# fgcallari/skeres

Hardware: AMD Instinct MI355X
Metric: LM iterations/sec (higher is better)
Workload: dtype f64

## Files before the change

skeres_amd/csrc/bal_kernels.hip:

```cpp
#include <hip/hip_runtime.h>

#include <algorithm>

#include "functors.hpp"
#include "bal_kernels.hpp"

namespace sk {

static constexpr int kBlock = 256;

__device__ __forceinline__ double wave_sum(double v) {
#pragma unroll
  for (int off = 32; off > 0; off >>= 1) v += __shfl_xor(v, off, 64);
  return v;
}

__device__ __forceinline__ int bal_part(const BalDev& d, int i) { return i >= d.cam_b ? 2 : ((i >= d.seg_lo && i < d.cam_a) ? 0 : 1); }
__device__ __forceinline__ int bal_pos(const BalDev& d, int i, int part) { return 9 * (i - (part == 0 ? d.seg_lo : (part == 1 ? d.cam_a : d.cam_b))); }
__device__ __forceinline__ double* bal_block(const BalDev& d, int i, int j, int* ld) {
  const int pj = bal_part(d, j), pi = bal_part(d, i);
  const BalDev::Front& f = d.front[pj];
  const int row = pi == pj ? bal_pos(d, i, pi) : f.border_row[i - d.cam_b];
  *ld = f.ld;
  return f.S + (size_t)row * f.ld + bal_pos(d, j, pj);
// ... 144 lines not shown
    double r0 = 0.0, r1 = 0.0, sqrt_rho1 = 1.0, alpha_sq_norm = 0.0;
    for (int first = 0; first < dim; first += W) {
      J out[2];
      out[1] = J(0.0);
      tape_run<J>(t, c, param, first, regs, out);
      if (first == 0) {
        r0 = out[0].a; r1 = out[1].a;
        if (kLoss) {
          const double sq = r0 * r0 + r1 * r1;
          double rho[3];
          bal_loss_eval(d, o, sq, rho);
          const LossCorrector lc(sq, rho);
          acc[0] += rho[0];
          sqrt_rho1 = lc.sqrt_rho1; alpha_sq_norm = lc.alpha_sq_norm;
          d.r[o] = r0 * lc.residual_scaling;
          d.r[(size_t)d.N + o] = r1 * lc.residual_scaling;
        } else {
          d.r[o] = r0;
          d.r[(size_t)d.N + o] = r1;
          acc[0] += r0 * r0 + r1 * r1;
        }
      }
#pragma unroll
      for (int w = 0; w < W; ++w) {
        const int k = first + w;
        if (k >= dim) continue;
        double j0 = out[0].v[w], j1 = out[1].v[w];
        if (kLoss) {
          const double rtj = alpha_sq_norm * (r0 * j0 + r1 * j1);
          const double a0 = sqrt_rho1 * (j0 - r0 * rtj), a1 = sqrt_rho1 * (j1 - r1 * rtj);
          j0 = a0; j1 = a1;
        }
        if (k < cs) {
          const double s = d.scale_c[9 * (size_t)ci + k];
          d.F[(size_t)k * d.N + o] = j0 * s;
          d.F[(size_t)(9 + k) * d.N + o] = j1 * s;
        } else {
          const double s = d.scale_p[3 * (size_t)pi + (k - cs)];
          d.E[(size_t)(k - cs) * d.N + o] = j0 * s;
          d.E[(size_t)(3 + k - cs) * d.N + o] = j1 * s;
        }
      }
    }
  }
  block_sum<1>(acc, d.partial, d.partial_stride);
}
template <bool kLoss>
__global__ __launch_bounds__(kBlock) void bal_eval_cost_tape_kernel(BalDev d, TapeDev t, int num_obs) {
  extern __shared__ __attribute__((aligned(16))) double tape_lds[];
  const TapeRegs<double> regs{tape_lds, kBlock, (int)threadIdx.x};
  double acc[2] = {0.0, 0.0};
  for (int o = blockIdx.x * kBlock + threadIdx.x; o < d.N; o += gridDim.x * kBlock) {
    if (d.is_host && d.is_host[o]) continue;
    const int ci = d.cam[o], pi = d.pt[o];
    double c[kTapeMaxObs], out[2];
    for (int k = 0; k < num_obs; ++k) c[k] = d.obs[(size_t)k * d.N + o];
    const int cs = d.cam_size;
    auto param = [&](int k) { return k < cs ? d.xc_new[9 * (size_t)ci + k] : d.xp_new[3 * (size_t)pi + (k - cs)]; };
    out[1] = 0.0;
    tape_run<double>(t, c, param, 0, regs, out);
    if (kLoss) {
      double rho[3];
      bal_loss_eval(d, o, out[0] * out[0] + out[1] * out[1], rho);
      acc[0] += rho[0];
    } else {
      acc[0] += out[0] * out[0] + out[1] * out[1];
    }
    double m0 = -d.u[3 * (size_t)d.N + o], m1 = -d.u[4 * (size_t)d.N + o];
#pragma unroll
    for (int k = 0; k < 3; ++k) {
      const double s = d.step_p[3 * (size_t)pi + k];
      m0 += d.E[(size_t)k * d.N + o] * s;
      m1 += d.E[(size_t)(3 + k) * d.N + o] * s;
    }
    acc[1] += m0 * (d.r[o] + m0 / 2.0) + m1 * (d.r[(size_t)d.N + o] + m1 / 2.0);
  }
  block_sum<2>(acc, d.partial, d.partial_stride);
}

template <bool kLoss>
__global__ __launch_bounds__(kBlock) void bal_host_jac_kernel(BalDev d, int partial_off) {
  double acc[1] = {0.0};
  for (int h = blockIdx.x * kBlock + threadIdx.x; h < d.num_host; h += gridDim.x * kBlock) {
    const int o = d.host_obs[h];
    const int ci = d.cam[o], pi = d.pt[o];
    const double* row = d.host_rows + (size_t)h * kHostRow;
    const double r0 = row[0], r1 = row[1];
    double j0[12], j1[12];
#pragma unroll
    for (int k = 0; k < 9; ++k) { j0[k] = row[2 + k]; j1[k] = row[11 + k]; }
#pragma unroll
    for (int k = 0; k < 3; ++k) { j0[9 + k] = row[20 + k]; j1[9 + k] = row[23 + k]; }
    if (kLoss) {
      const double sq = r0 * r0 + r1 * r1;
      double rho[3];
      bal_loss_eval(d, o, sq, rho);
      const LossCorrector lc(sq, rho);
      acc[0] += rho[0];
#pragma unroll
      for (int k = 0; k < 12; ++k) {
        const double a = j0[k], b = j1[k];
        const double rtj = lc.alpha_sq_norm * (r0 * a + r1 * b);
        j0[k] = lc.sqrt_rho1 * (a - r0 * rtj);
        j1[k] = lc.sqrt_rho1 * (b - r1 * rtj);
      }
      d.r[o] = r0 * lc.residual_scaling;
      d.r[(size_t)d.N + o] = r1 * lc.residual_scaling;
    } else {
      d.r[o] = r0;
      d.r[(size_t)d.N + o] = r1;
      acc[0] += r0 * r0 + r1 * r1;
    }
#pragma unroll
    for (int k = 0; k < 9; ++k) {
      const double s = d.scale_c[9 * (size_t)ci + k];
      d.F[(size_t)k * d.N + o] = j0[k] * s;
      d.F[(size_t)(9 + k) * d.N + o] = j1[k] * s;
    }
#pragma unroll
    for (int k = 0; k < 3; ++k) {
      const double s = d.scale_p[3 * (size_t)pi + k];
      d.E[(size_t)k * d.N + o] = j0[9 + k] * s;
      d.E[(size_t)(3 + k) * d.N + o] = j1[9 + k] * s;
    }
  }
  block_sum<1>(acc, d.partial + partial_off, d.partial_stride);
}

template <bool kLoss>
__global__ __launch_bounds__(kBlock) void bal_host_cost_kernel(BalDev d, int partial_off) {
  double acc[2] = {0.0, 0.0};
  for (int h = blockIdx.x * kBlock + threadIdx.x; h < d.num_host; h += gridDim.x * kBlock) {
    const int o = d.host_obs[h];
    const int ci = d.cam[o], pi = d.pt[o];
    const double n0 = d.host_rows[(size_t)h * kHostRow], n1 = d.host_rows[(size_t)h * kHostRow + 1];
    if (kLoss) {
      double rho[3];
      bal_loss_eval(d, o, n0 * n0 + n1 * n1, rho);
      acc[0] += rho[0];
    } else {
      acc[0] += n0 * n0 + n1 * n1;
    }
    double m0 = -d.u[3 * (size_t)d.N + o], m1 = -d.u[4 * (size_t)d.N + o];
#pragma unroll
    for (int k = 0; k < 3; ++k) {
      const double s = d.step_p[3 * (size_t)pi + k];
      m0 += d.E[(size_t)k * d.N + o] * s;
      m1 += d.E[(size_t)(3 + k) * d.N + o] * s;
    }
    acc[1] += m0 * (d.r[o] + m0 / 2.0) + m1 * (d.r[(size_t)d.N + o] + m1 / 2.0);
  }
  block_sum<2>(acc, d.partial + partial_off, d.partial_stride);
}

__global__ __launch_bounds__(kBlock) void bal_scale_jac_kernel(BalDev d) {
  for (int o = blockIdx.x * kBlock + threadIdx.x; o < d.N; o += gridDim.x * kBlock) {
    const int ci = d.cam[o], pi = d.pt[o];
#pragma unroll
    for (int k = 0; k < 9; ++k) {
      const double s = d.scale_c[9 * (size_t)ci + k];
      d.F[(size_t)k * d.N + o] *= s;
      d.F[(size_t)(9 + k) * d.N + o] *= s;
    }
#pragma unroll
    for (int k = 0; k < 3; ++k) {
      const double s = d.scale_p[3 * (size_t)pi + k];
      d.E[(size_t)k * d.N + o] *= s;
      d.E[(size_t)(3 + k) * d.N + o] *= s;
    }
  }
}

__global__ __launch_bounds__(kBlock) void bal_cam_records_kernel(BalDev d) {
  __shared__ __attribute__((aligned(16))) double stage[kBlock / 64][64 * kFcam];
  const int lane = threadIdx.x & 63, w = threadIdx.x >> 6;
  double* st = stage[w];
  const size_t N = d.N;
  for (long o0 = ((long)blockIdx.x * (kBlock / 64) + w) * 64; o0 < d.N; o0 += (long)gridDim.x * kBlock) {
    const long o = o0 + lane;
    const int my_slot = o < d.N ? d.obs_slot[o] : 0;
    if (o < d.N) {
#pragma unroll
      for (int k = 0; k < 18; ++k) st[lane * kFcam + k] = d.F[(size_t)k * N + o];
      st[lane * kFcam + 18] = d.r[o];
      st[lane * kFcam + 19] = d.r[N + o];
    }
    __builtin_amdgcn_wave_barrier();
    __builtin_amdgcn_s_waitcnt(0xC07F);
    __builtin_amdgcn_wave_barrier();
    const int nrec = (int)((d.N - o0) < 64 ? (d.N - o0) : 64);
#pragma unroll
    for (int i = 0; i < kFcam / 2; ++i) {
      const int e2 = i * 64 + lane, rr = e2 / (kFcam / 2), f2 = e2 - rr * (kFcam / 2);
      const int slot = __shfl(my_slot, rr, 64);
      if (rr < nrec) reinterpret_cast<double2*>(d.Fcam + (size_t)slot * kFcam)[f2] = reinterpret_cast<const double2*>(st)[e2];
    }
    __builtin_amdgcn_wave_barrier();
  }
}

__device__ __forceinline__ void bal_cam_reduce_body(const BalDev& d, int block) {
  const int wave = (block * kBlock + threadIdx.x) >> 6, lane = threadIdx.x & 63;
  if (wave >= d.C) return;
  double sq[9], g[9];
#pragma unroll
  for (int k = 0; k < 9; ++k) { sq[k] = 0.0; g[k] = 0.0; }
  for (int e = d.cam_start[wave] + lane; e < d.cam_start[wave + 1]; e += 64) {
    const double2* rec = reinterpret_cast<const double2*>(d.Fcam + (size_t)e * kFcam);
    double v[kFcam];
#pragma unroll
    for (int k = 0; k < kFcam / 2; ++k) { const double2 t = rec[k]; v[2 * k] = t.x; v[2 * k + 1] = t.y; }
    const double r0 = v[18], r1 = v[19];
#pragma unroll
    for (int k = 0; k < 9; ++k) {
      const double f0 = v[k], f1 = v[9 + k];
      sq[k] += f0 * f0 + f1 * f1;
      g[k] += f0 * r0 + f1 * r1;
    }
  }
#pragma unroll
  for (int k = 0; k < 9; ++k) { sq[k] = wave_sum(sq[k]); g[k] = wave_sum(g[k]); }
  if (lane == 0) {
#pragma unroll
    for (int k = 0; k < 9; ++k) { d.colsq_c[9 * (size_t)wave + k] = sq[k]; d.gs_c[9 * (size_t)wave + k] = g[k]; }
  }
}

__device__ __forceinline__ void bal_pt_reduce_body(const BalDev& d, int block) {
  const int gid = block * kBlock + threadIdx.x, sub = gid % kPointLanes;
  const int p = gid / kPointLanes;
  if (p >= d.P) return;
  double sq[3] = {0, 0, 0}, g[3] = {0, 0, 0};
  for (int o = d.pt_start[p] + sub; o < d.pt_start[p + 1]; o += kPointLanes) {
    const double r0 = d.r[o], r1 = d.r[(size_t)d.N + o];
#pragma unroll
    for (int k = 0; k < 3; ++k) {
      const double e0 = d.E[(size_t)k * d.N + o], e1 = d.E[(size_t)(3 + k) * d.N + o];
      sq[k] += e0 * e0 + e1 * e1;
      g[k] += e0 * r0 + e1 * r1;
    }
  }
#pragma unroll
  for (int k = 0; k < 3; ++k) { sq[k] = point_lanes_sum(sq[k]); g[k] = point_lanes_sum(g[k]); }
  if (sub == 0) {
#pragma unroll
    for (int k = 0; k < 3; ++k) { d.colsq_p[3 * (size_t)p + k] = sq[k]; d.gs_p[3 * (size_t)p + k] = g[k]; }
  }
}

__global__ __launch_bounds__(kBlock) void bal_reduce_kernel(BalDev d, int cam_blocks) {
  if ((int)blockIdx.x < cam_blocks) bal_cam_reduce_body(d, (int)blockIdx.x);
  else bal_pt_reduce_body(d, (int)blockIdx.x - cam_blocks);
}

__global__ void jacobi_scale_kernel(const double* colsq, double* scale, int n) {
  const int j = blockIdx.x * blockDim.x + threadIdx.x;
  if (j < n) scale[j] = scale[j] == 0.0 ? 0.0 : 1.0 / (1.0 + sqrt(colsq[j]));
}
__global__ void apply_scale_to_reductions_kernel(double* colsq, double* gs, const double* scale, int n) {
  const int j = blockIdx.x * blockDim.x + threadIdx.x;
  if (j < n) { const double s = scale[j]; colsq[j] = colsq[j] * s * s; gs[j] = gs[j] * s; }
}
__global__ void lm_diagonal_kernel(const double* colsq, double* D, int n, double lo, double hi, double radius) {
  const int j = blockIdx.x * blockDim.x + threadIdx.x;
  if (j < n) D[j] = sqrt(fmin(fmax(colsq[j], lo), hi) / radius);
}
__global__ __launch_bounds__(kBlock) void grad_max_xnorm_kernel(const double* gs, const double* scale, const double* x,
                                                                int n, double* partial, int stride) {
  double m = 0.0, s = 0.0;
  for (int j = blockIdx.x * kBlock + threadIdx.x; j < n; j += gridDim.x * kBlock) {
    if (scale[j] != 0.0 || gs[j] != 0.0) m = max_keep_nan(m, fabs(gs[j] / scale[j]));
    s += x[j] * x[j];
  }
  __shared__ double shm[kBlock / 64], shs[kBlock / 64];
#pragma unroll
  for (int off = 32; off > 0; off >>= 1) { m = max_keep_nan(m, __shfl_xor(m, off, 64)); s += __shfl_xor(s, off, 64); }
  if ((threadIdx.x & 63) == 0) { shm[threadIdx.x >> 6] = m; shs[threadIdx.x >> 6] = s; }
  __syncthreads();
  if (threadIdx.x == 0) {
    for (int i = 1; i < kBlock / 64; ++i) { m = max_keep_nan(m, shm[i]); s += shs[i]; }
    partial[blockIdx.x] = m;
    partial[stride + blockIdx.x] = s;
  }
}

__global__ __launch_bounds__(kBlock) void final_reduce_kernel(const double* partial, int stride, int count, int K, int maxmask, double* out) {
  __shared__ double sh[kBlock];
  const int k = blockIdx.x;
  const bool is_max = ((maxmask >> k) & 1) != 0;
  double a = 0.0;
  for (int i = threadIdx.x; i < count; i += kBlock) {
    const double v = partial[(size_t)k * stride + i];
    a = is_max ? max_keep_nan(a, v) : a + v;
  }
  sh[threadIdx.x] = a;
  __syncthreads();
  for (int w = kBlock / 2; w > 0; w >>= 1) {
    if ((int)threadIdx.x < w) sh[threadIdx.x] = is_max ? max_keep_nan(sh[threadIdx.x], sh[threadIdx.x + w]) : sh[threadIdx.x] + sh[threadIdx.x + w];
    __syncthreads();
  }
  if (threadIdx.x == 0) out[k] = sh[0];
}

__global__ __launch_bounds__(kBlock) void bal_point_block_kernel(BalDev d) {
  const int gid = blockIdx.x * kBlock + threadIdx.x, sub = gid % kPointLanes;
  const int p = gid / kPointLanes;
  if (p >= d.P) return;
  double t00 = 0, t10 = 0, t11 = 0, t20 = 0, t21 = 0, t22 = 0;
  for (int o = d.pt_start[p] + sub; o < d.pt_start[p + 1]; o += kPointLanes) {
    const double a0 = d.E[o], a1 = d.E[(size_t)d.N + o], a2 = d.E[2 * (size_t)d.N + o];
    const double b0 = d.E[3 * (size_t)d.N + o], b1 = d.E[4 * (size_t)d.N + o], b2 = d.E[5 * (size_t)d.N + o];
    t00 += a0 * a0 + b0 * b0; t10 += a1 * a0 + b1 * b0; t11 += a1 * a1 + b1 * b1;
    t20 += a2 * a0 + b2 * b0; t21 += a2 * a1 + b2 * b1; t22 += a2 * a2 + b2 * b2;
  }
  t00 = point_lanes_sum(t00); t10 = point_lanes_sum(t10); t11 = point_lanes_sum(t11);
  t20 = point_lanes_sum(t20); t21 = point_lanes_sum(t21); t22 = point_lanes_sum(t22);
  if (sub != 0) return;
  const double d0 = bal_lm_diag(d, d.colsq_p[3 * (size_t)p]), d1 = bal_lm_diag(d, d.colsq_p[3 * (size_t)p + 1]), d2 = bal_lm_diag(d, d.colsq_p[3 * (size_t)p + 2]);
  t00 += d0 * d0; t11 += d1 * d1; t22 += d2 * d2;
  const double l00 = sqrt(t00);
  const double l10 = t10 / l00, l20 = t20 / l00;
  const double l11 = sqrt(t11 - l10 * l10);
  const double l21 = (t21 - l20 * l10) / l11;
  const double l22 = sqrt(t22 - l20 * l20 - l21 * l21);
  const double m00 = 1.0 / l00, m11 = 1.0 / l11, m22 = 1.0 / l22;
  const double m10 = -(l10 * m00) / l11;
  const double m21 = -(l21 * m11) / l22;
  const double m20 = -(l20 * m00 + l21 * m10) / l22;
  const size_t P = d.P;
  d.M[p] = m00; d.M[P + p] = m10; d.M[2 * P + p] = m11; d.M[3 * P + p] = m20; d.M[4 * P + p] = m21; d.M[5 * P + p] = m22;
  const double g0 = d.gs_p[3 * (size_t)p], g1 = d.gs_p[3 * (size_t)p + 1], g2 = d.gs_p[3 * (size_t)p + 2];
  const double u0 = m00 * g0, u1 = m10 * g0 + m11 * g1, u2 = m20 * g0 + m21 * g1 + m22 * g2;
  d.q[p] = m00 * u0 + m10 * u1 + m20 * u2;
  d.q[P + p] = m11 * u1 + m21 * u2;
  d.q[2 * P + p] = m22 * u2;
  if (!(l00 > 0.0) || !(l11 > 0.0) || !(l22 > 0.0)) *d.fail_flag = 1;
}

__global__ __launch_bounds__(kBlock) void bal_kept_points_kernel(BalDev d, int obs_blocks) {
  const size_t N = d.N, P = d.P;
  if ((int)blockIdx.x < obs_blocks) {
    const int e = blockIdx.x * kBlock + threadIdx.x;
    if (e >= d.num_kept_obs) return;
    const int o = d.kept_obs[e], k = d.kept_obs_slot[e];
    const int ic = d.kept_cam[k] / 3, t3 = 3 * (d.kept_cam[k] % 3);
    const int c = d.cam[o];
    const bool below = ic > c;
    if (!d.front[bal_part(d, below ? c : ic)].S) return;
    double ea[3], eb[3];
#pragma unroll
    for (int a = 0; a < 3; ++a) { ea[a] = d.E[(size_t)a * N + o]; eb[a] = d.E[(size_t)(3 + a) * N + o]; }
    int ld;
    double* blk = below ? bal_block(d, ic, c, &ld) : bal_block(d, c, ic, &ld);
#pragma unroll
    for (int b = 0; b < 9; ++b) {
      const double f0 = d.F[(size_t)b * N + o], f1 = d.F[(size_t)(9 + b) * N + o];
#pragma unroll
      for (int a = 0; a < 3; ++a) {
        const double v = ea[a] * f0 + eb[a] * f1;
        if (below) blk[(size_t)(t3 + a) * ld + b] = v; else blk[(size_t)b * ld + t3 + a] = v;
      }
    }
    return;
  }
  const int k = (((int)blockIdx.x - obs_blocks) * kBlock + threadIdx.x) >> 6, lane = threadIdx.x & 63;
  if (k >= d.num_kept) return;
  const int p = d.kept_pt[k], ic = d.kept_cam[k] / 3, t3 = 3 * (d.kept_cam[k] % 3);
  double t00 = 0, t10 = 0, t11 = 0, t20 = 0, t21 = 0, t22 = 0;
  for (int o = d.pt_start[p] + lane; o < d.pt_start[p + 1]; o += 64) {
    const double a0 = d.E[o], a1 = d.E[N + o], a2 = d.E[2 * N + o];
    const double b0 = d.E[3 * N + o], b1 = d.E[4 * N + o], b2 = d.E[5 * N + o];
    t00 += a0 * a0 + b0 * b0; t10 += a1 * a0 + b1 * b0; t11 += a1 * a1 + b1 * b1;
    t20 += a2 * a0 + b2 * b0; t21 += a2 * a1 + b2 * b1; t22 += a2 * a2 + b2 * b2;
  }
  t00 = wave_sum(t00); t10 = wave_sum(t10); t11 = wave_sum(t11); t20 = wave_sum(t20); t21 = wave_sum(t21); t22 = wave_sum(t22);
  if (lane != 0) return;
  d.M[p] = 0.0; d.M[P + p] = 0.0; d.M[2 * P + p] = 0.0; d.M[3 * P + p] = 0.0; d.M[4 * P + p] = 0.0; d.M[5 * P + p] = 0.0;
  d.q[p] = 0.0; d.q[P + p] = 0.0; d.q[2 * P + p] = 0.0;
  if (!d.front[bal_part(d, ic)].S) return;
  const bool home = !d.kept_home || d.kept_home[k] != 0;
  const double d0 = home ? bal_lm_diag(d, d.colsq_p[3 * (size_t)p]) : 0.0, d1 = home ? bal_lm_diag(d, d.colsq_p[3 * (size_t)p + 1]) : 0.0,
               d2 = home ? bal_lm_diag(d, d.colsq_p[3 * (size_t)p + 2]) : 0.0;
  int ld;
  double* blk = bal_block(d, ic, ic, &ld) + (size_t)t3 * ld + t3;
  blk[0] = t00 + d0 * d0;
  blk[ld] = t10; blk[ld + 1] = t11 + d1 * d1;
  blk[2 * (size_t)ld] = t20; blk[2 * (size_t)ld + 1] = t21; blk[2 * (size_t)ld + 2] = t22 + d2 * d2;
  double* rhs = bal_rhs(d, ic) + t3;
  rhs[0] = home ? d.gs_p[3 * (size_t)p] : 0.0; rhs[1] = home ? d.gs_p[3 * (size_t)p + 1] : 0.0; rhs[2] = home ? d.gs_p[3 * (size_t)p + 2] : 0.0;
}

__global__ __launch_bounds__(kBlock) void bal_kept_sums_kernel(BalDev d, double* buf, int K, int gather) {
  const int t = blockIdx.x * kBlock + threadIdx.x;
  if (t >= 3 * d.num_kept) return;
  const int k = t / 3, a = t - 3 * k;
  const size_t p = (size_t)d.kept_pt[k], g = (size_t)(d.kept_global ? d.kept_global[k] : k);
  if (gather) { buf[3 * g + a] = d.colsq_p[3 * p + a]; buf[3 * (size_t)K + 3 * g + a] = d.gs_p[3 * p + a]; }
  else { d.colsq_p[3 * p + a] = buf[3 * g + a]; d.gs_p[3 * p + a] = buf[3 * (size_t)K + 3 * g + a]; }
}

__global__ __launch_bounds__(kBlock, 4) void bal_obs_precompute_kernel(BalDev d) {
  constexpr int kLs = kWs + 2;
  __shared__ __attribute__((aligned(16))) double stage[kBlock / 64][32 * kLs];
  const size_t N = d.N, P = d.P;
  const int lane = threadIdx.x & 63, wave = threadIdx.x >> 6;
  double* mine = &stage[wave][0];
  for (long base = (long)(blockIdx.x * kBlock + wave * 64); base < (long)d.N; base += (long)gridDim.x * kBlock) {
    const long o = base + lane;
    const int my_slot = o < (long)d.N ? d.obs_slot[o] : 0;
    double w[27], rt[2];
    if (o < (long)d.N) {
      const int p = d.pt[o];
      const double m00 = d.M[p], m10 = d.M[P + p], m11 = d.M[2 * P + p], m20 = d.M[3 * P + p], m21 = d.M[4 * P + p], m22 = d.M[5 * P + p];
      const double q0 = d.q[p], q1 = d.q[P + p], q2 = d.q[2 * P + p];
      double eh[2][3];
#pragma unroll
      for (int r = 0; r < 2; ++r) {
        const double e0 = d.E[(3 * r) * N + o], e1 = d.E[(3 * r + 1) * N + o], e2 = d.E[(3 * r + 2) * N + o];
        eh[r][0] = e0 * m00;
        eh[r][1] = e0 * m10 + e1 * m11;
        eh[r][2] = e0 * m20 + e1 * m21 + e2 * m22;
        rt[r] = d.r[r * N + o] - (e0 * q0 + e1 * q1 + e2 * q2);
      }
#pragma unroll
      for (int c = 0; c < 9; ++c) {
        const double f0 = d.F[c * N + o], f1 = d.F[(9 + c) * N + o];
#pragma unroll
        for (int a = 0; a < 3; ++a) w[3 * c + a] = f0 * eh[0][a] + f1 * eh[1][a];
      }
    }
    const int nrec = (int)(((long)d.N - base) < 64 ? ((long)d.N - base) : 64);
    const int sub = lane >> 4, chunk = lane & 15;
#pragma unroll
    for (int half = 0; half < 2; ++half) {
      if ((lane >> 5) == half && o < (long)d.N) {
        double* rec = mine + (lane & 31) * kLs;
#pragma unroll
        for (int k = 0; k < 27; ++k) rec[k] = w[k];
        rec[27] = rt[0]; rec[28] = rt[1];
        rec[29] = 0.0; rec[30] = 0.0; rec[31] = 0.0;
      }
      __builtin_amdgcn_wave_barrier();
#pragma unroll 4
      for (int it = 0; it < 8; ++it) {
        const int rl = 4 * it + sub, rec = 32 * half + rl;
        const int slot = __shfl(my_slot, rec, 64);
        if (rec < nrec) {
          const double2 v = *reinterpret_cast<const double2*>(&mine[rl * kLs + 2 * chunk]);
          *reinterpret_cast<double2*>(d.What + (size_t)slot * kWs + 2 * chunk) = v;
        }
      }
      __builtin_amdgcn_wave_barrier();
    }
  }
}

__global__ __launch_bounds__(kBlock) void bal_cam_diag_kernel(BalDev d) {
  const int i = (blockIdx.x * kBlock + threadIdx.x) >> 6, lane = threadIdx.x & 63;
  if (i >= d.C) return;
  if (d.pseudo && d.pseudo[i]) return;
  double acc[45], rh[9];
#pragma unroll
  for (int k = 0; k < 45; ++k) acc[k] = 0.0;
#pragma unroll
  for (int k = 0; k < 9; ++k) rh[k] = 0.0;
  for (int e = d.cam_start[i] + lane; e < d.cam_start[i + 1]; e += 64) {
    double f0[9], f1[9], w[28];
    {
      const double2* rec = reinterpret_cast<const double2*>(d.Fcam + (size_t)e * kFcam);
#pragma unroll
      for (int k = 0; k < 9; ++k) {
        const double2 t = rec[k];
        if (2 * k < 9) f0[2 * k] = t.x; else f1[2 * k - 9] = t.x;
        if (2 * k + 1 < 9) f0[2 * k + 1] = t.y; else f1[2 * k + 1 - 9] = t.y;
      }
    }
    const double2* wrec = reinterpret_cast<const double2*>(d.What + (size_t)e * kWs);
#pragma unroll
    for (int k = 0; k < 14; ++k) { const double2 t = wrec[k]; w[2 * k] = t.x; w[2 * k + 1] = t.y; }
    const double r0 = w[27], r1 = wrec[14].x;
    int k = 0;
#pragma unroll
    for (int c = 0; c < 9; ++c) {
      rh[c] += f0[c] * r0 + f1[c] * r1;
#pragma unroll
      for (int e2 = 0; e2 <= c; ++e2, ++k)
        acc[k] += (f0[c] * f0[e2] + f1[c] * f1[e2]) - (w[3 * c] * w[3 * e2] + w[3 * c + 1] * w[3 * e2 + 1] + w[3 * c + 2] * w[3 * e2 + 2]);
    }
  }
#pragma unroll
  for (int k = 0; k < 45; ++k) acc[k] = wave_sum(acc[k]);
#pragma unroll
  for (int k = 0; k < 9; ++k) rh[k] = wave_sum(rh[k]);
  if (lane == 0 && d.front[bal_part(d, i)].S) {
    int k = 0, ld;
    double* blk = bal_block(d, i, i, &ld);
    double* rhs = bal_rhs(d, i);
#pragma unroll
    for (int c = 0; c < 9; ++c) {
      rhs[c] = rh[c];
#pragma unroll
      for (int e2 = 0; e2 <= c; ++e2, ++k) blk[(size_t)c * ld + e2] = acc[k];
    }
  }
}

__global__ __launch_bounds__(64) void bal_dup_diag_kernel(BalDev d) {
  const int first = blockIdx.x;
  const int i = d.dup_cam[first];
  if (first > 0 && d.dup_cam[first - 1] == i) return;
  if (!d.front[bal_part(d, i)].S) return;
  const int t = threadIdx.x;
  if (t >= 45) return;
  int c = 0, rem = t;
  while (rem > c) { rem -= c + 1; ++c; }
  const int e2 = rem;
  double acc = 0.0;
  for (int k = first; k < d.num_dup && d.dup_cam[k] == i; ++k) {
    const double* wa = d.What + (size_t)d.dup_a[k] * kWs;
    const double* wb = d.What + (size_t)d.dup_b[k] * kWs;
    acc += (wa[3 * c] * wb[3 * e2] + wa[3 * c + 1] * wb[3 * e2 + 1] + wa[3 * c + 2] * wb[3 * e2 + 2]) +
           (wb[3 * c] * wa[3 * e2] + wb[3 * c + 1] * wa[3 * e2 + 1] + wb[3 * c + 2] * wa[3 * e2 + 2]);
  }
  int ld;
  double* blk = bal_block(d, i, i, &ld);
  blk[(size_t)c * ld + e2] -= acc;
}

constexpr int kPairSlot = 34;
__device__ __forceinline__ void pair_accumulate(const BalDev& d, int e_begin, int e_end, int stride, int c, double* slot, double (&acc)[9]) {
  if (e_begin >= e_end) return;
  const int last = e_begin + (e_end - 1 - e_begin) / stride * stride;
  const double* wr = d.What + (size_t)d.pair_row_obs[e_begin] * kWs + 3 * c;
  const double* wc = d.What + (size_t)d.pair_col_obs[e_begin] * kWs + 3 * c;
  double y0 = wr[0], y1 = wr[1], y2 = wr[2], v0 = wc[0], v1 = wc[1], v2 = wc[2];
  int e1 = e_begin + stride <= last ? e_begin + stride : last;
  int ob1 = d.pair_row_obs[e1], oa1 = d.pair_col_obs[e1];
  for (int e = e_begin; e < e_end; e += stride) {
    slot[3 * c] = v0; slot[3 * c + 1] = v1; slot[3 * c + 2] = v2;
    __builtin_amdgcn_wave_barrier();
    double w[kWu];
#pragma unroll
    for (int k = 0; k < kWu / 2; ++k) { const double2 t = reinterpret_cast<const double2*>(slot)[k]; w[2 * k] = t.x; w[2 * k + 1] = t.y; }
    __builtin_amdgcn_wave_barrier();
    const double* wrn = d.What + (size_t)ob1 * kWs + 3 * c;
    const double* wcn = d.What + (size_t)oa1 * kWs + 3 * c;
    const double yn0 = wrn[0], yn1 = wrn[1], yn2 = wrn[2], vn0 = wcn[0], vn1 = wcn[1], vn2 = wcn[2];
    const int e2 = e + 2 * stride <= last ? e + 2 * stride : last;
    const int ob2 = d.pair_row_obs[e2], oa2 = d.pair_col_obs[e2];
#pragma unroll
    for (int k = 0; k < 9; ++k) acc[k] += y0 * w[3 * k] + y1 * w[3 * k + 1] + y2 * w[3 * k + 2];
    y0 = yn0; y1 = yn1; y2 = yn2; v0 = vn0; v1 = vn1; v2 = vn2;
    ob1 = ob2; oa1 = oa2;
  }
}

__device__ __forceinline__ int xcd_grouped_block(int w, int group) {
  if (group <= 0) return w;
  const int x = w & 7, q = w >> 3;
  return ((q / group) * 8 + x) * group + q % group;
}

__global__ __launch_bounds__(kBlock) void bal_pair_kernel(BalDev d, int xcd_group) {
  const int lane = threadIdx.x & 63;
  const int wave = (xcd_grouped_block((int)blockIdx.x, xcd_group) * kBlock + threadIdx.x) >> 6;
  __shared__ __attribute__((aligned(16))) double share[kBlock / 64][7][kPairSlot];
  const int sub = lane / 9, c = lane - 9 * sub;
  const int slot = wave * 7 + sub;
  if (sub >= 7 || slot >= d.num_short_segments) return;
  const int seg = d.short_segments[slot];
  double acc[9];
#pragma unroll
  for (int k = 0; k < 9; ++k) acc[k] = 0.0;
  pair_accumulate(d, d.seg_start[seg], d.seg_start[seg + 1], 1, c, share[threadIdx.x >> 6][sub], acc);
  const int i = d.seg_row[seg], j = d.seg_col[seg];
  int ld;
  double* out = bal_block(d, i, j, &ld) + (size_t)c * ld;
#pragma unroll
  for (int k = 0; k < 9; ++k) out[k] = -acc[k];
}

__global__ __launch_bounds__(kBlock) void bal_pair_long_kernel(BalDev d, int xcd_group) {
  __shared__ double red[kBlock / 64][7][81];
  __shared__ __attribute__((aligned(16))) double share[kBlock / 64][7][kPairSlot];
  const int lane = threadIdx.x & 63, w = threadIdx.x >> 6;
  const int slot = (xcd_grouped_block((int)blockIdx.x, xcd_group) * kBlock + threadIdx.x) >> 6;
  if (slot >= d.num_long_segments) return;
  const int seg = d.long_segments[slot];
  const int sub = lane / 9, c = lane - 9 * sub;
  double acc[9];
#pragma unroll
  for (int k = 0; k < 9; ++k) acc[k] = 0.0;
  if (sub < 7) {
    pair_accumulate(d, d.seg_start[seg] + sub, d.seg_start[seg + 1], 7, c, share[w][sub], acc);
#pragma unroll
    for (int k = 0; k < 9; ++k) red[w][sub][9 * c + k] = acc[k];
  }
  __builtin_amdgcn_wave_barrier();
  __builtin_amdgcn_s_waitcnt(0xC07F);
  __builtin_amdgcn_wave_barrier();
  const int i = d.seg_row[seg], j = d.seg_col[seg];
  int ld;
  double* blk = bal_block(d, i, j, &ld);
  for (int e = lane; e < 81; e += 64) {
    double s = 0.0;
#pragma unroll
    for (int g = 0; g < 7; ++g) s += red[w][g][e];
    blk[(size_t)(e / 9) * ld + e % 9] = -s;
  }
}

__global__ void finish_normal_matrix_kernel(double* S, int ld, int n, int npad, int rhs_row, const double* D) {
  const int j = blockIdx.x * blockDim.x + threadIdx.x;
  if (j >= npad) return;
  if (j < n) S[(size_t)j * ld + j] += D[j] * D[j];
  else if (j == rhs_row) S[(size_t)j * ld + j] = 1e300;
  else S[(size_t)j * ld + j] = 1.0;
}
__global__ void bal_finish_S_kernel(BalDev d, int parts) {
  const int j = blockIdx.x * blockDim.x + threadIdx.x;
  if (j >= 9 * d.C) return;
  const int i = j / 9, c = j - 9 * i, part = bal_part(d, i);
  if (!((parts >> part) & 1) || !d.front[part].S) return;
  if (d.pseudo && d.pseudo[i]) return;
  int ld;
  double* blk = bal_block(d, i, i, &ld);
  const double D = bal_lm_diag(d, d.colsq_c[j]);
  blk[(size_t)c * ld + c] += D * D;
}
__global__ void set_diagonal_kernel(double* S, int ld, int from, int to, double value) {
  const int j = from + blockIdx.x * blockDim.x + threadIdx.x;
  if (j < to) S[(size_t)j * ld + j] = value;
}

__global__ __launch_bounds__(kBlock) void bal_obs_backsub_kernel(BalDev d) {
  const size_t N = d.N;
  for (int o = blockIdx.x * kBlock + threadIdx.x; o < d.N; o += gridDim.x * kBlock) {
    const double* yc = d.y_c + 9 * (size_t)d.cam[o];
    double f0 = 0.0, f1 = 0.0;
#pragma unroll
    for (int c = 0; c < 9; ++c) { f0 += d.F[c * N + o] * yc[c]; f1 += d.F[(9 + c) * N + o] * yc[c]; }
    d.u[o] = d.E[o] * f0 + d.E[3 * N + o] * f1;
    d.u[N + o] = d.E[N + o] * f0 + d.E[4 * N + o] * f1;
    d.u[2 * N + o] = d.E[2 * N + o] * f0 + d.E[5 * N + o] * f1;
    d.u[3 * N + o] = f0;
    d.u[4 * N + o] = f1;
  }
}

__global__ __launch_bounds__(kBlock) void bal_point_backsub_kernel(BalDev d) {
  const int gid = blockIdx.x * kBlock + threadIdx.x, sub = gid % kPointLanes;
  const int p = gid / kPointLanes;
  double acc[1] = {0.0};
  double w0 = 0.0, w1 = 0.0, w2 = 0.0;
  if (p < d.P) {
    for (int o = d.pt_start[p] + sub; o < d.pt_start[p + 1]; o += kPointLanes) {
      w0 += d.u[o];
      w1 += d.u[(size_t)d.N + o];
      w2 += d.u[2 * (size_t)d.N + o];
    }
  }
  w0 = point_lanes_sum(w0); w1 = point_lanes_sum(w1); w2 = point_lanes_sum(w2);
  if (p < d.P && sub == 0) {
    const size_t P = d.P;
    const double t0 = d.gs_p[3 * (size_t)p] - w0, t1 = d.gs_p[3 * (size_t)p + 1] - w1, t2 = d.gs_p[3 * (size_t)p + 2] - w2;
    const double m00 = d.M[p], m10 = d.M[P + p], m11 = d.M[2 * P + p], m20 = d.M[3 * P + p], m21 = d.M[4 * P + p], m22 = d.M[5 * P + p];
    const double u0 = m00 * t0, u1 = m10 * t0 + m11 * t1, u2 = m20 * t0 + m21 * t1 + m22 * t2;
    const double y[3] = {m00 * u0 + m10 * u1 + m20 * u2, m11 * u1 + m21 * u2, m22 * u2};
#pragma unroll
    for (int k = 0; k < 3; ++k) {
      const double st = -y[k];
      const double dl = st * d.scale_p[3 * (size_t)p + k];
      d.step_p[3 * (size_t)p + k] = st;
      const double xo = d.xp[3 * (size_t)p + k];
      const double xn = xo + dl;
      d.xp_new[3 * (size_t)p + k] = xn;
      const double df = xo - xn;
      acc[0] += df * df;
    }
  }
  block_sum<1>(acc, d.partial + d.partial_stride, d.partial_stride);
}

__global__ __launch_bounds__(kBlock) void bal_kept_step_kernel(BalDev d, int slot) {
  double acc[1] = {0.0};
  for (int k = threadIdx.x; k < d.num_kept; k += kBlock) {
    const int p = d.kept_pt[k], ic = d.kept_cam[k] / 3, t3 = 3 * (d.kept_cam[k] % 3);
    const bool home = !d.kept_home || d.kept_home[k] != 0;
#pragma unroll
    for (int a = 0; a < 3; ++a) {
      const double st = -d.y_c[9 * (size_t)ic + t3 + a];
      d.step_p[3 * (size_t)p + a] = st;
      const double xo = d.xp[3 * (size_t)p + a];
      const double xn = xo + st * d.scale_p[3 * (size_t)p + a];
      d.xp_new[3 * (size_t)p + a] = xn;
      const double df = xo - xn;
      if (home) acc[0] += df * df;
    }
  }
  block_sum<1>(acc, d.partial + d.partial_stride + slot, d.partial_stride);
}

__global__ __launch_bounds__(kBlock) void bal_cam_step_kernel(BalDev d, int norm_lo, int norm_hi, int norm_lo2, int norm_hi2) {
  double acc[1] = {0.0};
  const int n = 9 * d.C;
  const int j = blockIdx.x * kBlock + threadIdx.x;
  if (j < n) {
    const int i = j / 9, c = j - 9 * i, part = bal_part(d, i);
    const double y = d.front[part].S ? d.y_front[part][bal_pos(d, i, part) + c] : 0.0;
    d.y_c[j] = y;
    const double st = -y;
    d.step_c[j] = st;
    const double xo = d.xc[j];
    const double xn = xo + st * d.scale_c[j];
    d.xc_new[j] = xn;
    const double df = xo - xn;
    if ((j >= norm_lo && j < norm_hi) || (j >= norm_lo2 && j < norm_hi2)) acc[0] += df * df;
  }
  block_sum<1>(acc, d.partial, d.partial_stride);
}
__global__ __launch_bounds__(1024) void final_reduce_rows_kernel(const double* partial, int stride, ReduceRows rows) {
  __shared__ double sh[1024];
  const int k = blockIdx.x, count = rows.count[k];
  const bool is_max = rows.is_max[k] != 0;
  const double* src = partial + (size_t)rows.row[k] * stride;
  double a = 0.0;
  for (int i = threadIdx.x; i < count; i += 1024) a = is_max ? max_keep_nan(a, src[i]) : a + src[i];
  sh[threadIdx.x] = a;
  __syncthreads();
  for (int w = 512; w > 0; w >>= 1) {
    if ((int)threadIdx.x < w) sh[threadIdx.x] = is_max ? max_keep_nan(sh[threadIdx.x], sh[threadIdx.x + w]) : sh[threadIdx.x] + sh[threadIdx.x + w];
    __syncthreads();
  }
  if (threadIdx.x == 0) *rows.out[k] = sh[0];
}
void launch_final_reduce_rows(const double* partial, int stride, const ReduceRows& rows, hipStream_t s) {
  if (rows.n > 0) hipLaunchKernelGGL(final_reduce_rows_kernel, dim3(rows.n), dim3(1024), 0, s, partial, stride, rows);
}

__global__ __launch_bounds__(256) void tri_pack_kernel(double* S, int ld, double* packed, const int* __restrict__ col0, const long long* __restrict__ off,
                                                       int to_packed) {
  const int kb = blockIdx.y;
  const size_t c0 = (size_t)col0[kb] * 128, width = (size_t)(kb + 1) * 128 - c0;
  double* pk = packed + off[kb];
  const size_t n2 = 128 * width / 2;
  for (size_t i = (size_t)blockIdx.x * 256 + threadIdx.x; i < n2; i += (size_t)gridDim.x * 256) {
    const size_t e = 2 * i, r = e / width, c = e % width;
    double2* a = reinterpret_cast<double2*>(S + ((size_t)kb * 128 + r) * ld + c0 + c);
    double2* b = reinterpret_cast<double2*>(pk + e);
    if (to_packed) *b = *a; else *a = *b;
  }
}

static inline int grid_for(int n, int cap = 2048) {
  int g = (n + kBlock - 1) / kBlock;
  return g < 1 ? 1 : (g > cap ? cap : g);
}

__global__ __launch_bounds__(256) void zero_envelope_kernel(double* S, int ld, const int* col0) {
  const int kb = blockIdx.y;
  const size_t c0 = (size_t)col0[kb] * 128, width = (size_t)(kb + 1) * 128 - c0;
  const size_t n2 = 128 * width / 2;
  for (size_t i = (size_t)blockIdx.x * 256 + threadIdx.x; i < n2; i += (size_t)gridDim.x * 256) {
    const size_t e = 2 * i, r = e / width, c = e % width;
    *reinterpret_cast<double2*>(S + ((size_t)kb * 128 + r) * ld + c0 + c) = make_double2(0.0, 0.0);
  }
}
void launch_zero_envelope(double* S, int ld, const int* col0, int nblk, hipStream_t s) {
  if (nblk > 0) hipLaunchKernelGGL(zero_envelope_kernel, dim3(32, nblk), dim3(256), 0, s, S, ld, col0);
}

int bal_partial_blocks(int N) { return grid_for(N); }
size_t tri_packed_elems(int nblk) { return (size_t)128 * 128 * ((size_t)nblk * (nblk + 1) / 2); }
void launch_tri_pack(double* S, int ld, double* packed, int nblk, const int* col0, const long long* off, bool to_packed, hipStream_t s) {
  if (nblk > 0) hipLaunchKernelGGL(tri_pack_kernel, dim3(64, nblk), dim3(256), 0, s, S, ld, packed, col0, off, to_packed ? 1 : 0);
}

void launch_bal_eval_jac(const BalDev& d, hipStream_t s) {
  if (d.loss_root >= 0) hipLaunchKernelGGL(bal_eval_jac_kernel<true>, dim3(grid_for(d.N)), dim3(kBlock), 0, s, d);
  else hipLaunchKernelGGL(bal_eval_jac_kernel<false>, dim3(grid_for(d.N)), dim3(kBlock), 0, s, d);
}
void launch_bal_eval_cost(const BalDev& d, hipStream_t s) {
  if (d.loss_root >= 0) hipLaunchKernelGGL(bal_eval_cost_kernel<true>, dim3(grid_for(d.N)), dim3(kBlock), 0, s, d);
  else hipLaunchKernelGGL(bal_eval_cost_kernel<false>, dim3(grid_for(d.N)), dim3(kBlock), 0, s, d);
}
int bal_tape_width(const Tape& t) { return t.num_obs_consts > kTapeMaxObs ? 0 : tape_pick_width(t, kBlock); }
template <class K> static void bal_tape_allow_lds(K kernel, size_t bytes) {
  if (bytes > 48 * 1024) (void)hipFuncSetAttribute(reinterpret_cast<const void*>(kernel), hipFuncAttributeMaxDynamicSharedMemorySize, (int)bytes);
}
void launch_bal_eval_jac_tape(const BalDev& d, const TapeDevBuffers& tb, hipStream_t s) {
  const int W = bal_tape_width(tb.host), nobs = tb.host.num_obs_consts;
  const size_t lds = tape_lds_bytes(tb.host, W, kBlock);
  const dim3 g(grid_for(d.N)), b(kBlock);
#define SK_TAPE_JAC(LOSS, WW) { bal_tape_allow_lds(bal_eval_jac_tape_kernel<LOSS, WW>, lds); hipLaunchKernelGGL((bal_eval_jac_tape_kernel<LOSS, WW>), g, b, lds, s, d, tb.view, nobs); }
  if (d.loss_root >= 0) { if (W == 3) SK_TAPE_JAC(true, 3) else if (W == 2) SK_TAPE_JAC(true, 2) else SK_TAPE_JAC(true, 1) }
  else { if (W == 3) SK_TAPE_JAC(false, 3) else if (W == 2) SK_TAPE_JAC(false, 2) else SK_TAPE_JAC(false, 1) }
#undef SK_TAPE_JAC
}
void launch_bal_eval_cost_tape(const BalDev& d, const TapeDevBuffers& tb, hipStream_t s) {
  const size_t lds = tape_lds_bytes(tb.host, 0, kBlock);
  const int nobs = tb.host.num_obs_consts;
  if (d.loss_root >= 0) { bal_tape_allow_lds(bal_eval_cost_tape_kernel<true>, lds); hipLaunchKernelGGL(bal_eval_cost_tape_kernel<true>, dim3(grid_for(d.N)), dim3(kBlock), lds, s, d, tb.view, nobs); }
  else { bal_tape_allow_lds(bal_eval_cost_tape_kernel<false>, lds); hipLaunchKernelGGL(bal_eval_cost_tape_kernel<false>, dim3(grid_for(d.N)), dim3(kBlock), lds, s, d, tb.view, nobs); }
}
int launch_bal_host_jac(const BalDev& d, int partial_off, hipStream_t s) {
  if (d.num_host <= 0) return 0;
  const int g = grid_for(d.num_host);
  if (d.loss_root >= 0) hipLaunchKernelGGL(bal_host_jac_kernel<true>, dim3(g), dim3(kBlock), 0, s, d, partial_off);
  else hipLaunchKernelGGL(bal_host_jac_kernel<false>, dim3(g), dim3(kBlock), 0, s, d, partial_off);
  return g;
}
int launch_bal_host_cost(const BalDev& d, int partial_off, hipStream_t s) {
  if (d.num_host <= 0) return 0;
  const int g = grid_for(d.num_host);
  if (d.loss_root >= 0) hipLaunchKernelGGL(bal_host_cost_kernel<true>, dim3(g), dim3(kBlock), 0, s, d, partial_off);
  else hipLaunchKernelGGL(bal_host_cost_kernel<false>, dim3(g), dim3(kBlock), 0, s, d, partial_off);
  return g;
}
void launch_bal_scale_jac(const BalDev& d, hipStream_t s) { hipLaunchKernelGGL(bal_scale_jac_kernel, dim3(grid_for(d.N)), dim3(kBlock), 0, s, d); }
void launch_bal_cam_records(const BalDev& d, hipStream_t s) { hipLaunchKernelGGL(bal_cam_records_kernel, dim3(grid_for((d.N + 63) / 64 * 64)), dim3(kBlock), 0, s, d); }
void launch_bal_reduce(const BalDev& d, hipStream_t s) {
  const int cam_blocks = (d.C * 64 + kBlock - 1) / kBlock, pt_blocks = d.P > 0 ? (int)(((long)d.P * kPointLanes + kBlock - 1) / kBlock) : 0;
  hipLaunchKernelGGL(bal_reduce_kernel, dim3(cam_blocks + pt_blocks), dim3(kBlock), 0, s, d, cam_blocks);
}
static int point_grid(int P) { return (int)(((long)P * kPointLanes + kBlock - 1) / kBlock); }
int bal_point_blocks(int P) { return P > 0 ? point_grid(P) : 1; }
void launch_jacobi_scale(const double* colsq, double* scale, int n, hipStream_t s) { if (n > 0) hipLaunchKernelGGL(jacobi_scale_kernel, dim3((n + 255) / 256), dim3(256), 0, s, colsq, scale, n); }
void launch_apply_scale_to_reductions(double* colsq, double* gs, const double* scale, int n, hipStream_t s) { if (n > 0) hipLaunchKernelGGL(apply_scale_to_reductions_kernel, dim3((n + 255) / 256), dim3(256), 0, s, colsq, gs, scale, n); }
void launch_lm_diagonal(const double* colsq, double* D, int n, double lo, double hi, double radius, hipStream_t s) { if (n > 0) hipLaunchKernelGGL(lm_diagonal_kernel, dim3((n + 255) / 256), dim3(256), 0, s, colsq, D, n, lo, hi, radius); }
int launch_grad_max_xnorm(const double* gs, const double* scale, const double* x, int n, double* partial, int stride, hipStream_t s) {
  const int g = grid_for(n, 256);
  hipLaunchKernelGGL(grad_max_xnorm_kernel, dim3(g), dim3(kBlock), 0, s, gs, scale, x, n, partial, stride);
  return g;
}
__global__ void bal_pack_rank_scalars_kernel(const double* __restrict__ scal, double* __restrict__ table, int rank, int world, int mode, int segmented) {
  const int K = mode == 0 ? 3 : 4;
  for (int i = threadIdx.x; i < world * K; i += blockDim.x) table[i] = 0.0;
  __syncthreads();
  if (threadIdx.x != 0) return;
  double* t = table + (size_t)rank * K;
  if (mode == 0) {
    t[0] = scal[4];
    t[1] = segmented ? fmax(scal[2], scal[0]) : scal[2];
    t[2] = scal[3] + (segmented ? scal[1] : 0.0);
  } else {
    const int fail = *reinterpret_cast<const int*>(scal + 14), info = *reinterpret_cast<const int*>(scal + 15);
    t[0] = scal[0]; t[1] = scal[1];
    t[2] = scal[9] + (segmented ? scal[8] : 0.0);
    t[3] = (double)(fail | info);
  }
}
void launch_bal_pack_rank_scalars(const double* scal, double* table, int rank, int world, int mode, bool segmented, hipStream_t s) {
  hipLaunchKernelGGL(bal_pack_rank_scalars_kernel, dim3(1), dim3(64), 0, s, scal, table, rank, world, mode, segmented ? 1 : 0);
}
void launch_final_reduce(const double* partial, int stride, int count, int K, int maxmask, double* out, hipStream_t s) { hipLaunchKernelGGL(final_reduce_kernel, dim3(K), dim3(kBlock), 0, s, partial, stride, count, K, maxmask, out); }
void launch_bal_point_block(const BalDev& d, hipStream_t s) { if (d.P > 0) hipLaunchKernelGGL(bal_point_block_kernel, dim3(point_grid(d.P)), dim3(kBlock), 0, s, d); }
void launch_bal_kept_points(const BalDev& d, hipStream_t s) {
  if (d.num_kept <= 0) return;
  const int obs_blocks = (d.num_kept_obs + kBlock - 1) / kBlock;
  hipLaunchKernelGGL(bal_kept_points_kernel, dim3(obs_blocks + (d.num_kept * 64 + kBlock - 1) / kBlock), dim3(kBlock), 0, s, d, obs_blocks);
}
void launch_bal_obs_precompute(const BalDev& d, hipStream_t s) { hipLaunchKernelGGL(bal_obs_precompute_kernel, dim3(grid_for(d.N)), dim3(kBlock), 0, s, d); }
void launch_bal_kept_sums(const BalDev& d, double* buf, int K, bool gather, hipStream_t s) {
  if (d.num_kept > 0) hipLaunchKernelGGL(bal_kept_sums_kernel, dim3((3 * d.num_kept + kBlock - 1) / kBlock), dim3(kBlock), 0, s, d, buf, K, gather ? 1 : 0);
}
void launch_bal_cam_diag(const BalDev& d, hipStream_t s) {
  hipLaunchKernelGGL(bal_cam_diag_kernel, dim3((d.C * 64 + kBlock - 1) / kBlock), dim3(kBlock), 0, s, d);
  if (d.num_dup > 0) hipLaunchKernelGGL(bal_dup_diag_kernel, dim3(d.num_dup), dim3(64), 0, s, d);
}
void launch_bal_pair(const BalDev& d, hipStream_t s) {
  const int group_long = dev_knobs().schedule_plain ? 0 : 8, group_short = group_long;
  auto grid = [](int blocks, int group) { return group > 0 ? (blocks + 8 * group - 1) / (8 * group) * (8 * group) : blocks; };
  if (d.num_long_segments > 0)
    hipLaunchKernelGGL(bal_pair_long_kernel, dim3(grid((d.num_long_segments * 64 + kBlock - 1) / kBlock, group_long)), dim3(kBlock), 0, s, d, group_long);
  if (d.num_short_segments > 0) {
    const int waves = (d.num_short_segments + 6) / 7;
    hipLaunchKernelGGL(bal_pair_kernel, dim3(grid((waves * 64 + kBlock - 1) / kBlock, group_short)), dim3(kBlock), 0, s, d, group_short);
  }
}
void launch_finish_normal_matrix(double* S, int ld, int n, int npad, int rhs_row, const double* D, hipStream_t s) { hipLaunchKernelGGL(finish_normal_matrix_kernel, dim3((npad + 255) / 256), dim3(256), 0, s, S, ld, n, npad, rhs_row, D); }
__global__ void bal_finish_all_kernel(BalDev d, BalFinishRanges r, int jmax) {
  const int j = blockIdx.x * blockDim.x + threadIdx.x;
  if (j >= jmax) return;
  if (j < 9 * d.C) {
    const int i = j / 9, c = j - 9 * i, part = bal_part(d, i);
    if (d.front[part].S && !(d.pseudo && d.pseudo[i])) {
      int ld;
      double* blk = bal_block(d, i, i, &ld);
      const double D = bal_lm_diag(d, d.colsq_c[j]);
      blk[(size_t)c * ld + c] += D * D;
    }
  }
#pragma unroll
  for (int k = 0; k < 4; ++k)
    if (r.S[k] && j >= r.from[k] && j < r.to[k]) r.S[k][(size_t)j * r.ld[k] + j] = r.value[k];
}
void launch_bal_finish_all(const BalDev& d, const BalFinishRanges& r, hipStream_t s) {
  int jmax = 9 * d.C;
  for (int k = 0; k < 4; ++k) if (r.S[k] && r.to[k] > jmax) jmax = r.to[k];
  hipLaunchKernelGGL(bal_finish_all_kernel, dim3((jmax + 255) / 256), dim3(256), 0, s, d, r, jmax);
}
void launch_bal_finish_S(const BalDev& d, int parts, hipStream_t s) { hipLaunchKernelGGL(bal_finish_S_kernel, dim3((9 * d.C + 255) / 256), dim3(256), 0, s, d, parts); }
void launch_set_diagonal(double* S, int ld, int from, int to, double value, hipStream_t s) {
  if (to > from) hipLaunchKernelGGL(set_diagonal_kernel, dim3((to - from + 255) / 256), dim3(256), 0, s, S, ld, from, to, value);
}
void launch_bal_backsub(const BalDev& d, double* out, int norm_lo, int norm_hi, int norm_lo2, int norm_hi2, hipStream_t s) {
  const int gc = (9 * d.C + kBlock - 1) / kBlock, gp = bal_point_blocks(d.P);
  hipLaunchKernelGGL(bal_cam_step_kernel, dim3(gc), dim3(kBlock), 0, s, d, norm_lo, norm_hi, norm_lo2, norm_hi2);
  hipLaunchKernelGGL(bal_obs_backsub_kernel, dim3(grid_for(d.N)), dim3(kBlock), 0, s, d);
  hipLaunchKernelGGL(bal_point_backsub_kernel, dim3(gp), dim3(kBlock), 0, s, d);
  if (d.num_kept > 0) hipLaunchKernelGGL(bal_kept_step_kernel, dim3(1), dim3(kBlock), 0, s, d, gp);
  ReduceRows rows;
  rows.n = 2;
  rows.row[0] = 0; rows.count[0] = gc; rows.out[0] = out;
  rows.row[1] = 1; rows.count[1] = d.P > 0 ? gp + (d.num_kept > 0 ? 1 : 0) : 0; rows.out[1] = out + 1;
  launch_final_reduce_rows(d.partial, d.partial_stride, rows, s);
}

__global__ __launch_bounds__(kBlock) void dogleg_vector_norms_kernel(BalDev d, DoglegDev q) {
  double acc[3] = {0.0, 0.0, 0.0};
  const int nc = 9 * d.C, n = nc + 3 * d.P;
  for (int j = blockIdx.x * kBlock + threadIdx.x; j < n; j += gridDim.x * kBlock) {
    double sj = 0.0, gj = 0.0;
    if (!(j < nc && d.pseudo && d.pseudo[j / 9])) {
      const double diag = sqrt(fmin(fmax(d.colsq_c[j], d.lm_lo), d.lm_hi));
      const double gh = d.gs_c[j] / diag;
      gj = d.step_c[j];
      const double p = diag * gj;
      sj = -gh / diag;
      acc[0] += gh * gh; acc[1] += gh * p; acc[2] += p * p;
    }
    q.s[j] = sj; q.g[j] = gj;
  }
  block_sum<3>(acc, q.partial + 5 * (size_t)q.stride, q.stride);
}

__global__ __launch_bounds__(kBlock) void bal_dogleg_products_kernel(BalDev d, DoglegDev q) {
  double acc[5] = {0.0, 0.0, 0.0, 0.0, 0.0};
  const size_t N = d.N;
  const double* sp = q.s + 9 * (size_t)d.C;
  const double* gp = q.g + 9 * (size_t)d.C;
  for (int o = blockIdx.x * kBlock + threadIdx.x; o < d.N; o += gridDim.x * kBlock) {
    const size_t ci = 9 * (size_t)d.cam[o], pi = 3 * (size_t)d.pt[o];
    double w0 = 0.0, w1 = 0.0, m0 = 0.0, m1 = 0.0;
#pragma unroll
    for (int k = 0; k < 9; ++k) {
      const double f0 = d.F[k * N + o], f1 = d.F[(9 + k) * N + o], sk_ = q.s[ci + k], gk = q.g[ci + k];
      w0 += f0 * sk_; w1 += f1 * sk_; m0 += f0 * gk; m1 += f1 * gk;
    }
#pragma unroll
    for (int k = 0; k < 3; ++k) {
      const double e0 = d.E[k * N + o], e1 = d.E[(3 + k) * N + o], sk_ = sp[pi + k], gk = gp[pi + k];
      w0 += e0 * sk_; w1 += e1 * sk_; m0 += e0 * gk; m1 += e1 * gk;
    }
    const double r0 = d.r[o], r1 = d.r[N + o];
    acc[0] += w0 * r0 + w1 * r1; acc[1] += m0 * r0 + m1 * r1;
    acc[2] += w0 * w0 + w1 * w1; acc[3] += w0 * m0 + w1 * m1; acc[4] += m0 * m0 + m1 * m1;
  }
  block_sum<5>(acc, q.partial, q.stride);
}

__global__ __launch_bounds__(kBlock) void bal_dogleg_combine_kernel(BalDev d, DoglegDev q, double a, double b) {
  double acc[1] = {0.0};
  const int n = 9 * d.C + 3 * d.P;
  for (int j = blockIdx.x * kBlock + threadIdx.x; j < n; j += gridDim.x * kBlock) {
    const double st = a * q.s[j] + b * q.g[j];
    d.step_c[j] = st;
    const double xo = d.xc[j];
    const double xn = xo + st * d.scale_c[j];
    d.xc_new[j] = xn;
    const double df = xo - xn;
    acc[0] += df * df;
  }
  block_sum<1>(acc, q.partial + 8 * (size_t)q.stride, q.stride);
}

int dogleg_partial_stride(const BalDev& d) { return std::max(grid_for(d.N), grid_for(9 * d.C + 3 * d.P)); }
void launch_dogleg_vector_norms(const BalDev& d, const DoglegDev& q, hipStream_t s) {
  hipLaunchKernelGGL(dogleg_vector_norms_kernel, dim3(grid_for(9 * d.C + 3 * d.P)), dim3(kBlock), 0, s, d, q);
}
void launch_bal_dogleg_products(const BalDev& d, const DoglegDev& q, hipStream_t s) {
  hipLaunchKernelGGL(bal_dogleg_products_kernel, dim3(grid_for(d.N)), dim3(kBlock), 0, s, d, q);
}
void launch_dogleg_reduce_scalars(const DoglegDev& q, hipStream_t s) { launch_final_reduce(q.partial, q.stride, q.stride, 8, 0, q.scal, s); }
void launch_bal_dogleg_combine(const BalDev& d, const DoglegDev& q, double a, double b, hipStream_t s) {
  const int g = grid_for(9 * d.C + 3 * d.P);
  hipLaunchKernelGGL(bal_dogleg_combine_kernel, dim3(g), dim3(kBlock), 0, s, d, q, a, b);
  launch_final_reduce(q.partial + 8 * (size_t)q.stride, q.stride, g, 1, 0, q.scal + 8, s);
}

__global__ void box_project_kernel(double* x, const double* __restrict__ lo, const double* __restrict__ hi, int n) {
  const int j = blockIdx.x * blockDim.x + threadIdx.x;
  if (j < n) x[j] = fmin(fmax(x[j], lo[j]), hi[j]);
}

__global__ __launch_bounds__(kBlock) void bounded_grad_max_xnorm_kernel(const double* __restrict__ gs, const double* __restrict__ scale, const double* __restrict__ x,
                                                                        int n, BoundsDev q) {
  double m = 0.0;
  double acc[2] = {0.0, 0.0};
  for (int j = blockIdx.x * kBlock + threadIdx.x; j < n; j += gridDim.x * kBlock) {
    const double xj = x[j], lo = q.lo[j], hi = q.hi[j];
    if (scale[j] != 0.0) m = fmax(m, fabs(xj - fmin(fmax(xj - gs[j] / scale[j], lo), hi)));
    acc[0] += xj * xj;
    acc[1] += (xj == lo || xj == hi) ? 1.0 : 0.0;
  }
  __shared__ double shm[kBlock / 64];
#pragma unroll
  for (int off = 32; off > 0; off >>= 1) m = fmax(m, __shfl_xor(m, off, 64));
  if ((threadIdx.x & 63) == 0) shm[threadIdx.x >> 6] = m;
  __syncthreads();
  if (threadIdx.x == 0) {
    for (int i = 1; i < kBlock / 64; ++i) m = fmax(m, shm[i]);
    q.partial[3 * (size_t)q.stride + blockIdx.x] = m;
  }
  block_sum<2>(acc, q.partial + 4 * (size_t)q.stride, q.stride);
}

__global__ __launch_bounds__(kBlock) void bal_directional_derivative_kernel(BalDev d, BoundsDev q) {
  double m = 0.0;
  double acc[1] = {0.0};
  const int nc = 9 * d.C, n = nc + 3 * d.P;
  for (int j = blockIdx.x * kBlock + threadIdx.x; j < n; j += gridDim.x * kBlock) {
    if (j < nc && d.pseudo && d.pseudo[j / 9]) continue;
    const double st = d.step_c[j];
    acc[0] += d.gs_c[j] * st;
    m = fmax(m, fabs(st * d.scale_c[j]));
  }
  __shared__ double shm[kBlock / 64];
#pragma unroll
  for (int off = 32; off > 0; off >>= 1) m = fmax(m, __shfl_xor(m, off, 64));
  if ((threadIdx.x & 63) == 0) shm[threadIdx.x >> 6] = m;
  __syncthreads();
  if (threadIdx.x == 0) {
    for (int i = 1; i < kBlock / 64; ++i) m = fmax(m, shm[i]);
    q.partial[2 * (size_t)q.stride + blockIdx.x] = m;
  }
  block_sum<1>(acc, q.partial + q.stride, q.stride);
}

__global__ __launch_bounds__(kBlock) void bal_bounded_candidate_kernel(BalDev d, BoundsDev q, double alpha) {
  double acc[1] = {0.0};
  const int nc = 9 * d.C, n = nc + 3 * d.P;
  for (int j = blockIdx.x * kBlock + threadIdx.x; j < n; j += gridDim.x * kBlock) {
    const double xo = d.xc[j];
    double xn = xo;
    if (!(j < nc && d.pseudo && d.pseudo[j / 9])) xn = fmin(fmax(xo + (alpha * d.step_c[j]) * d.scale_c[j], q.lo[j]), q.hi[j]);
    d.xc_new[j] = xn;
    const double df = xo - xn;
    acc[0] += df * df;
  }
  block_sum<1>(acc, q.partial, q.stride);
}

int bounds_partial_stride(int n) { return grid_for(n); }
void launch_box_project(double* x, const double* lo, const double* hi, int n, hipStream_t s) {
  if (n > 0) hipLaunchKernelGGL(box_project_kernel, dim3((n + 255) / 256), dim3(256), 0, s, x, lo, hi, n);
}
void launch_bounded_grad_max_xnorm(const double* gs, const double* scale, const double* x, int n, const BoundsDev& q, hipStream_t s) {
  const int g = grid_for(n);
  hipLaunchKernelGGL(bounded_grad_max_xnorm_kernel, dim3(g), dim3(kBlock), 0, s, gs, scale, x, n, q);
  launch_final_reduce(q.partial + 3 * (size_t)q.stride, q.stride, g, 3, 1, q.scal + 3, s);
}
void launch_bal_directional_derivative(const BalDev& d, const BoundsDev& q, hipStream_t s) {
  const int g = grid_for(9 * d.C + 3 * d.P);
  hipLaunchKernelGGL(bal_directional_derivative_kernel, dim3(g), dim3(kBlock), 0, s, d, q);
  launch_final_reduce(q.partial + q.stride, q.stride, g, 2, 2, q.scal + 1, s);
}
void launch_bal_bounded_candidate(const BalDev& d, const BoundsDev& q, double alpha, hipStream_t s) {
  const int g = grid_for(9 * d.C + 3 * d.P);
  hipLaunchKernelGGL(bal_bounded_candidate_kernel, dim3(g), dim3(kBlock), 0, s, d, q, alpha);
  launch_final_reduce(q.partial, q.stride, g, 1, 0, q.scal, s);
}

}
```

skeres_amd/csrc/bal_kernels.hpp:

```cpp
#pragma once
#include <hip/hip_runtime.h>

#include "common.hpp"
#include "loss.hpp"

namespace sk {

constexpr int kLongSegment = 32;
constexpr int kWs = 32;
constexpr int kWu = 28;
struct BalDev {
  int C, P, N;
  int res_size, cam_size, pt_size;
  const int* cam;
  const int* pt;
  const double* obs;
  const int* pt_start;
  const int* cam_start;
  const int* cam_obs;
  int num_segments;
  const int* seg_start;
  const int* seg_row;
  const int* seg_col;
  int num_short_segments, num_long_segments;
  const int* short_segments;
  const int* long_segments;
  const int* pair_row_obs;
  const int* pair_col_obs;
  int num_kept;
  const int* kept_pt;  const int* kept_cam;
  int num_kept_obs;  const int* kept_obs;  const int* kept_obs_slot;
  const unsigned char* pseudo;
  const int* kept_home;  const int* kept_global;
  int num_dup;  const int* dup_a;  const int* dup_b;  const int* dup_cam;
  double* xc;  double* xp;
  double* xc_new;  double* xp_new;
  double* scale_c;  double* scale_p;
  double* colsq_c;  double* colsq_p;
  double* gs_c;  double* gs_p;
  double lm_lo, lm_hi, lm_radius;  const double* lm_radius_dev;
  double* step_c;  double* step_p;
  double* y_c;
  double* r;  double* F;  double* E;  double* What;  double* u;
  double* Fcam;  const int* obs_slot;
  double* M;  double* q;
  struct Front { double* S; int ld; int interior; int rhs_row; const int* border_row; };
  Front front[3];
  int seg_lo, cam_a, cam_b;
  const double* y_front[3];
  double* S;  int ld;  int rhs_row;
  double* partial;  int partial_stride;
  int* fail_flag;
  const LossNode* loss_nodes;  int loss_root;  const int* loss_of_obs;
  const unsigned char* is_host;
  int num_host;
  const int* host_obs;
  const double* host_rows;
};
constexpr int kHostRow = 26;
constexpr int kFcam = 20;

int bal_partial_blocks(int N);
int bal_point_blocks(int P);
void launch_zero_envelope(double* S, int ld, const int* col0, int nblk, hipStream_t s);
size_t tri_packed_elems(int nblk);
void launch_tri_pack(double* S, int ld, double* packed, int nblk, const int* col0, const long long* off, bool to_packed, hipStream_t s);
void launch_bal_eval_jac(const BalDev& d, hipStream_t s);
void launch_bal_eval_cost(const BalDev& d, hipStream_t s);
void launch_bal_eval_jac_tape(const BalDev& d, const TapeDevBuffers& tb, hipStream_t s);
void launch_bal_eval_cost_tape(const BalDev& d, const TapeDevBuffers& tb, hipStream_t s);
int launch_bal_host_jac(const BalDev& d, int partial_off, hipStream_t s);
int launch_bal_host_cost(const BalDev& d, int partial_off, hipStream_t s);
void launch_bal_scale_jac(const BalDev& d, hipStream_t s);
void launch_bal_cam_records(const BalDev& d, hipStream_t s);
void launch_bal_reduce(const BalDev& d, hipStream_t s);
void launch_jacobi_scale(const double* colsq, double* scale, int n, hipStream_t s);
void launch_apply_scale_to_reductions(double* colsq, double* gs, const double* scale, int n, hipStream_t s);
void launch_lm_diagonal(const double* colsq, double* D, int n, double lo, double hi, double radius, hipStream_t s);
int launch_grad_max_xnorm(const double* gs, const double* scale, const double* x, int n, double* partial, int stride, hipStream_t s);
void launch_final_reduce(const double* partial, int stride, int count, int K, int maxmask, double* out, hipStream_t s);
void launch_bal_pack_rank_scalars(const double* scal, double* table, int rank, int world, int mode, bool segmented, hipStream_t s);
struct ReduceRows { int n = 0; int row[4] = {0, 0, 0, 0}, count[4] = {0, 0, 0, 0}, is_max[4] = {0, 0, 0, 0}; double* out[4] = {nullptr, nullptr, nullptr, nullptr}; };
void launch_final_reduce_rows(const double* partial, int stride, const ReduceRows& rows, hipStream_t s);
void launch_bal_point_block(const BalDev& d, hipStream_t s);
void launch_bal_kept_points(const BalDev& d, hipStream_t s);
void launch_bal_kept_sums(const BalDev& d, double* buf, int K, bool gather, hipStream_t s);
void launch_bal_obs_precompute(const BalDev& d, hipStream_t s);
void launch_bal_cam_diag(const BalDev& d, hipStream_t s);
void launch_bal_pair(const BalDev& d, hipStream_t s);
void launch_finish_normal_matrix(double* S, int ld, int n, int npad, int rhs_row, const double* D, hipStream_t s);
void launch_bal_finish_S(const BalDev& d, int parts, hipStream_t s);
struct BalFinishRanges { double* S[4] = {nullptr, nullptr, nullptr, nullptr}; int ld[4] = {0, 0, 0, 0}, from[4] = {0, 0, 0, 0}, to[4] = {0, 0, 0, 0}; double value[4] = {0, 0, 0, 0}; };
void launch_bal_finish_all(const BalDev& d, const BalFinishRanges& r, hipStream_t s);
void launch_set_diagonal(double* S, int ld, int from, int to, double value, hipStream_t s);
void launch_bal_backsub(const BalDev& d, double* out, int norm_lo, int norm_hi, int norm_lo2, int norm_hi2, hipStream_t s);

struct DoglegDev { double* s; double* g; double* partial; int stride; double* scal; };
int dogleg_partial_stride(const BalDev& d);
void launch_dogleg_vector_norms(const BalDev& d, const DoglegDev& q, hipStream_t s);
void launch_bal_dogleg_products(const BalDev& d, const DoglegDev& q, hipStream_t s);
void launch_dogleg_reduce_scalars(const DoglegDev& q, hipStream_t s);
void launch_bal_dogleg_combine(const BalDev& d, const DoglegDev& q, double a, double b, hipStream_t s);

struct BoundsDev { const double* lo; const double* hi; double* partial; int stride; double* scal; };
int bounds_partial_stride(int n);
void launch_box_project(double* x, const double* lo, const double* hi, int n, hipStream_t s);
void launch_bounded_grad_max_xnorm(const double* gs, const double* scale, const double* x, int n, const BoundsDev& q, hipStream_t s);
void launch_bal_directional_derivative(const BalDev& d, const BoundsDev& q, hipStream_t s);
void launch_bal_bounded_candidate(const BalDev& d, const BoundsDev& q, double alpha, hipStream_t s);

}
```

skeres_amd/csrc/bal_solver.hip:

```cpp
#include <algorithm>
#include <cmath>
#include <limits>

#include "bal_kernels.hpp"
#include "bal_plan.hpp"
#include "solver.hpp"

namespace sk {

namespace {

struct CaptureGuard {
  hipStream_t s; bool active; bool* graph_mode;
  CaptureGuard(hipStream_t st, bool on, bool* gm) : s(st), active(on), graph_mode(gm) {}
  void release() { active = false; }
  ~CaptureGuard() {
    if (!active) return;
    hipGraph_t g = nullptr;
    (void)hipStreamEndCapture(s, &g);
    if (g) (void)hipGraphDestroy(g);
    (void)hipGetLastError();
    *graph_mode = false;
  }
};

class BalSolver : public SolverBase {
 public:
  BalSolver(const Options& o, Problem* p) : SolverBase(o, p) {}
  double syrk_flops_per_solve() const override {
    double f = 0.0;
    for (int k = 0; k < 3; ++k) if (fr_[k].nblk > 0) f += cholesky_syrk_flops((int)fr_[k].dim, group_, fr_[k].env(), chain_ok() && (k != 1 || tail_chain()), nullptr, fr_[k].ncols, fr_[k].tail_rows, fr_[k].tl());
    return f;
  }
  double syrk_c_bytes_per_solve() const override {
    double tiles = 0.0;
    for (int k = 0; k < 3; ++k) {
      double t = 0.0;
      if (fr_[k].nblk > 0) (void)cholesky_syrk_flops((int)fr_[k].dim, group_, fr_[k].env(), chain_ok() && (k != 1 || tail_chain()), &t, fr_[k].ncols, fr_[k].tail_rows, fr_[k].tl());
      tiles += t;
    }
    return tiles * 2.0 * 128.0 * 128.0 * sizeof(double);
  }
  void set_kernel_timing(int on) override {
    SolverBase::set_kernel_timing(on);
    kt_b_.only(on == 2 ? "gemm_syrk" : ""); kt_b_.enable(on != 0);
  }
  KernelTimer::Stat kernel_stat(const std::string& name) override {
    KernelTimer::Stat a = kt_.get_stat(name), b = kt_b_.get_stat(name);
    a.seconds += b.seconds; a.launches += b.launches;
    return a;
  }
  bool stat(const std::string& name, double* value) const override {
    const int nblk = npad_ / 128;
    if (name == "envelope_fill") {
      double in = 0.0;
      for (int k = 0; k < 3; ++k) in += fr_[k].envelope().blocks();
      *value = in / (0.5 * nblk * (nblk + 1.0));
      return true;
    }
    if (name == "reduced_system_blocks") { *value = nblk; return true; }
    if (name == "camera_order") { *value = camera_order_; return true; }
    if (name == "cholesky_flops_full") { const double n = 9.0 * C_; *value = n * n * n / 3.0; return true; }
    if (name == "cholesky_flops_plan") {
      double f = 0.0;
      for (int k = 0; k < 3; ++k) if (fr_[k].nblk > 0) f += cholesky_plan_flops(fr_[k].nblk, fr_[k].env(), fr_[k].ncols, fr_[k].tail_rows, fr_[k].tl());
      *value = f;
      return true;
    }
    if (name == "cholesky_columns_resident") {
      int r = 0;
      for (int k = 0; k < 3; ++k) {
        if (fr_[k].nblk == 0) continue;
        const CholeskyPlan plan = cholesky_plan(fr_[k].nblk, group_, fr_[k].env(), chain_live() && (k != 1 || tail_chain()), fr_[k].ncols, fr_[k].tail_rows, fr_[k].tl());
        for (char c : plan.resident) r += c ? 1 : 0;
      }
      *value = r;
      return true;
    }
    if (name == "chain_steps") {
      *value = (dissected_ ? std::max(fr_[0].ncols, fr_[1].ncols) : 0) + fr_[2].ncols;
      return true;
    }
    if (name == "allreduce_bytes") { *value = (double)packed_elems_ * sizeof(double); return true; }
    if (name == "allreduce_bytes_full_triangle") { *value = (double)tri_packed_elems(nblk) * sizeof(double); return true; }
    if (name == "dissected") { *value = dissected_ ? 1.0 : 0.0; return true; }
    if (name == "pair_segments_short") { *value = d_.num_short_segments; return true; }
    if (name == "pair_segments_long") { *value = d_.num_long_segments; return true; }
    if (name == "graph_replay") { *value = graph_mode_ ? 1.0 : 0.0; return true; }
    if (name == "host_callback_blocks" || name == "tape_blocks") {
      const bool host = name == "host_callback_blocks";
      size_t c = 0;
      for (size_t b = 0; b < problem_->rb_functor.size(); ++b)
        c += host ? problem_->rb_functor[b] == SK_FUNCTOR_HOST_CALLBACK : problem_->tape_of_block(b) != nullptr;
      *value = (double)c;
      return true;
    }
    if (name == "tape_width") { *value = tape_mode_ ? bal_tape_width(tape_dev_.host) : 0; return true; }
    if (name == "tape_lds_bytes") { *value = tape_mode_ ? (double)tape_lds_bytes(tape_dev_.host, bal_tape_width(tape_dev_.host), 256) : 0.0; return true; }
    if (name == "retained_points") { *value = (double)retained_pts_.size(); return true; }
    if (name == "retained_model_us") { *value = retained_model_us_; return true; }
    if (name == "retained_model_us_without") { *value = retained_without_us_; return true; }
    if (name == "border_cameras") { *value = border_cams_; return true; }
    if (name == "border_gap") { *value = border_gap_; return true; }
    if (name == "border_model_us") { *value = border_model_us_; return true; }
    if (name == "border_model_us_plain") { *value = border_plain_us_; return true; }
    if (name == "segments") { *value = segmented_ ? segments_ : (dissected_ ? 2 : 1); return true; }
    if (name == "segment_cameras") { *value = segmented_ ? my_hi_ - my_lo_ : C_; return true; }
    if (name.rfind("model_us_segments_", 0) == 0) { const int k = atoi(name.c_str() + 18); if (k < 1 || k > 8) return false; *value = cut_model_.model_us[k]; return true; }
    if (name == "dissection_head_cameras") { *value = cam_a_; return true; }
    if (name == "dissection_tail_cameras") { *value = cam_b_ - cam_a_; return true; }
    if (name == "dissection_separator_cameras") { *value = dissected_ ? C_ - cam_b_ : 0; return true; }
    if (name == "dissection_model_us_plain") { *value = cut_model_.t_plain; return true; }
    if (name == "dissection_model_us") { *value = cut_model_.t_model; return true; }
    if (name == "model_us_two_segments_with_members") { *value = cut_model_.two_segments_members_us; return true; }
    return strategy_stat(name, value);
  }
  bool chain_ok() const { return opt_.cholesky_group == 0 && opt_.lookahead && chol_ctx_.server != nullptr; }
  bool chain_live() const { return chain_ok() && cholesky_chain_enabled(&chol_ctx_); }
  bool tail_chain() const { return chol_ctx_b_.server != nullptr; }
  int distribution(double* allreduce_s, double* saved_s) const override {
    if (allreduce_s) *allreduce_s = est_allreduce_s_;
    if (saved_s) *saved_s = est_saved_s_;
    return distribution_;
  }

 protected:
  int setup() override;
  int evaluate_with_jacobian(bool first) override;
  int linear_solve(double radius, LinearSolve* out) override;
  int dogleg_trial(double a, double b, double* cost, double* step_norm) override;
  int bounded_trial(double alpha, double* cost, double* step_norm) override;
  bool supports_dogleg() const override { return true; }
  int solve_once(double radius, LinearSolve* out, bool* chain_lost);
  struct Backsolve { int resident; bool zero_after; };
  int enqueue_schur_assembly(const Backsolve& bs, bool graph);
  int enqueue_factor_backsolve(const Backsolve& bs, bool graph);
  int enqueue_point_backsub(bool graph);
  int enqueue_candidate_cost(int rows, bool* failed);
  int trial_cost(const double* step_sq_dev, int step_sq_slot, double* cost, double* step_norm);
  const char* refuses_bounds() const override {
    for (int f : problem_->rb_functor)
      if (f == SK_FUNCTOR_HOST_CALLBACK) return "parameter bounds with host-evaluated (director) residual blocks under DENSE_SCHUR are not supported";
    return nullptr;
  }
  int upload_bounds();
  BoundsDev bd_{};
  DevBuf<double> b_bd_box_, b_bd_partial_, b_bd_scal_;
  DoglegDev dl_{};
  DevBuf<double> b_dl_vec_, b_dl_partial_, b_dl_scal_;
  void accept_candidate() override { std::swap(d_.xc, d_.xc_new); std::swap(d_.xp, d_.xp_new); parity_ ^= 1; }
  int write_back() override;
  void describe(Summary* s) override {
    s->num_parameter_blocks = (int)problem_->block_size.size();
    s->num_parameters = problem_->num_parameters();
    s->num_residual_blocks = (int)problem_->rb_functor.size();
    s->num_residuals = problem_->num_residuals;
    s->num_e_blocks = P_total_; s->num_f_blocks = C_ - pseudo_cams_;
  }

 private:
  int gather_rank_scalars(double* vals, int K, const int* ops);
  int host_callbacks(const double* x_dev, bool jac, bool* failed);
  std::vector<int> host_obs_;
  std::vector<const CostFunction*> host_cf_;
  std::vector<double> host_x_, host_rows_h_;
  DevBuf<unsigned char> b_is_host_;
  DevBuf<int> b_host_obs_;
  DevBuf<double> b_host_rows_;
  std::vector<int> h_cam_, h_pt_;
  int gather_rank_scalars_signed(double* vals, int K);
  bool rank_table_on_device(int K) const;
  int enqueue_rank_table(int mode, int K);
  int fold_rank_table(const double* table, double* vals, int K, const int* ops);
  int exchange_rank_table(const double* vals, int K, std::vector<double>* table);

  int C_ = 0, P_total_ = 0, P_ = 0, N_ = 0;
  int res_size_ = 2, cam_size_ = 9, pt_size_ = 3;
  int n_ = 0, npad_ = 0, rhs_row_ = 0;
  std::vector<int> cam_block_, pt_block_;
  std::vector<int> local_pt_;
  BalDev d_{};
  DevBuf<LossNode> b_loss_nodes_;
  DevBuf<int> b_loss_of_obs_;
  DevBuf<int> b_cam_, b_pt_, b_pt_start_, b_cam_start_, b_cam_obs_, b_obs_slot_, b_seg_start_, b_seg_row_, b_seg_col_, b_pair_row_, b_pair_col_, b_short_segs_, b_long_segs_;
  int *fail_p_ = nullptr, *info_p_ = nullptr;
  DevBuf<double> b_obs_, b_xc_, b_xp_, b_xc_new_, b_xp_new_, b_scale_, b_colsq_, b_gs_, b_step_, b_y_,
      b_r_, b_F_, b_Fcam_, b_E_, b_W_, b_rt_, b_M_, b_q_, b_S_, b_Linv_, b_partial_, b_scal_, b_small_;
  std::vector<int> env_last_;
  std::vector<int> env_tail_;
  std::vector<int> retained_pts_, retained_cam_;
  int pseudo_cams_ = 0;
  int border_members_ = 0;
  double retained_model_us_ = 0.0, retained_without_us_ = 0.0;
  std::vector<int> struct_ocam_, struct_opt_;
  int struct_P_ = 0;
  DevBuf<int> b_kept_pt_, b_kept_cam_, b_kept_obs_, b_kept_obs_slot_;
  int P_own_ = 0;
  DevBuf<int> b_kept_home_, b_kept_global_;
  DevBuf<int> b_dup_a_, b_dup_b_, b_dup_cam_;
  int num_dup_ = 0;
  int num_kept_obs_ = 0;
  DevBuf<unsigned char> b_pseudo_;
  int border_cams_ = 0, border_gap_ = 0;
  double border_model_us_ = 0.0, border_plain_us_ = 0.0;
  FrontHost fr_[3];
  bool dissected_ = false;
  bool segmented_ = false;
  int segments_ = 0, role_ = 0, my_lo_ = 0, my_hi_ = 0;
  bool replica_ = false;
  int fold_world_ = 0;
  int cam_a_ = 0, cam_b_ = 0, border_blocks_ = 0;
  std::vector<int> seg_off_;
  std::vector<int> sep_first_;
  std::vector<int> root_last_, root_tail_;
  FrontView leaf_;
  DevBuf<int> b_border_row_[2], b_leaf_map_, b_leaf_gmap_;
  CutModel cut_model_;
  DissectedSystem ds_;
  CholeskyContext chol_ctx_b_;
  KernelTimer kt_b_;
  bool tape_mode_ = false;
  TapeDevBuffers tape_dev_;
  bool graph_mode_ = false;
  int parity_ = 0;
  hipGraphExec_t g_step_[2] = {nullptr, nullptr}, g_eval_[2] = {nullptr, nullptr};
  bool graph_ok() const { return graph_mode_ && !kt_.enabled(); }
  int finish_capture(hipStream_t s, hipGraphExec_t* exec);
  DevBuf<int> b_zero_col0_f_[3], b_mapB_;
  bool mapB_involution_ = false;
  DevBuf<double> b_yf_, b_wf_, b_ybB_;
  double order_hash_ = 0.0;
  int camera_order_ = 0;
  int group_ = 3;
  DevBuf<double> b_pack_;
  size_t packed_elems_ = 0;
  std::vector<int> pack_col0_h_;
  std::vector<long long> pack_off_h_;
  DevBuf<int> b_pack_col0_;
  DevBuf<long long> b_pack_off_;
  int distribution_ = SK_DISTRIBUTION_SHARDED;
  double est_allreduce_s_ = 0.0, est_saved_s_ = 0.0;
  int choose_distribution(const std::vector<int>& opt);
  struct Structure {
    std::vector<int> ocam, opt;
    std::vector<int> band_ocam, band_opt;
    std::vector<int> env_for_model;
    int Creal = 0;
  };
  int init_queues();
  int plan_layout(Structure* st);
  void plan_pack();
  int prepare_pack();
  int shard_or_replicate(const std::vector<int>& opt);
  int cut_camera_sequence(Structure* st);
  void adopt_cuts(const CutPlan& cuts, int Cband, bool multi, Structure* st);
  int upload_structure(const LocalStructure& ls);
  int allocate_fronts(const FrontLayout& lay);
  int bind_device_view(const LocalStructure& ls);
  int agree_with_ranks();
  bool distribution_decided_ = false;
  std::chrono::steady_clock::time_point setup_t0_, stage_last_;
  void stage(const char* what) {
    if (!dev_knobs().debug_setup) return;
    const auto now = std::chrono::steady_clock::now();
    std::fprintf(stderr, "[skeres_amd] set-up: %-40s %8.1f ms (at %.1f ms)\n", what, std::chrono::duration<double, std::milli>(now - stage_last_).count(),
                 std::chrono::duration<double, std::milli>(now - setup_t0_).count());
    stage_last_ = now;
  }
  CholeskyContext chol_ctx_;
  enum Slot {
    kGradMaxCam = 0, kXSqCam, kGradMaxPt, kXSqPt, kSumSq,
    kEvalFirst = kGradMaxCam, kEvalLast = kSumSq,
    kCandSumSq = 0, kModel,
    kStepSqCam = 8, kStepSqPt,
    kRadiusDev = 12,
    kFail = 14, kInfo,
    kStepFirst = kCandSumSq, kStepLast = kInfo,
    kDevSlots = kStepLast + 1,
    kRadius = kDevSlots,
    kDogleg,
    kBounds = kDogleg + kDlScalCount,
    kRankTable = kBounds + kBdScalCount,
    kRankTableSlots = 24,
    kHostSlots = kRankTable + kRankTableSlots
  };
  static_assert(kEvalLast < kStepSqCam && kModel < kStepSqCam && kStepSqPt < kRadiusDev && kRadiusDev < kFail, "b_scal_'s slots are distinct");
  static_assert(kStepLast < kRadius && kRadius < kDogleg && kDogleg + kDlScalCount <= kBounds && kBounds + kBdScalCount <= kRankTable, "h_scal_'s regions do not overlap");
  double* h_scal_ = nullptr;
  int host_flag(int slot) const { int v = 0; std::memcpy(&v, h_scal_ + slot, sizeof(int)); return v; }
  double* rank_table_dev() const { return b_small_.p + 2 * 9 * (size_t)C_ + 6 * retained_pts_.size() + 64; }
  int partial_stride_ = 0;
  bool zero_by_backsolve_ = false;
  bool need_full_zero_ = false;
  DevBuf<int> b_zero_min_f_[3];
  bool pair_claimed_ = false;
 public:
  ~BalSolver() override {
    if (pair_claimed_) cholesky_release_pair_servers(&chol_ctx_);
    for (hipGraphExec_t g : {g_step_[0], g_step_[1], g_eval_[0], g_eval_[1]}) if (g) (void)hipGraphExecDestroy(g);
    if (h_scal_) (void)hipHostFree(h_scal_);
  }
};

int BalSolver::choose_distribution(const std::vector<int>& opt) {
  const int W = opt_.world;
  distribution_ = SK_DISTRIBUTION_SHARDED;
  if (W <= 1 || opt_.distribution_mode == SK_DISTRIBUTION_SHARDED) return SK_OK;
  if (opt_.distribution_mode != SK_DISTRIBUTION_REPLICATED) {
    const double per_iter = chain_model::shardable_work_s(chain_model::pair_entries(opt, P_total_), (double)opt.size());
    est_saved_s_ = per_iter * (1.0 - 1.0 / W);
    int rc = allreduce(b_pack_.p, packed_elems_);
    if (rc) return rc;
    SK_HIP_TRY(hipStreamSynchronize(stream_));
    const auto t0 = std::chrono::steady_clock::now();
    for (int rep = 0; rep < 2; ++rep) { rc = allreduce(b_pack_.p, packed_elems_); if (rc) return rc; }
    SK_HIP_TRY(hipStreamSynchronize(stream_));
    double mine = std::chrono::duration<double>(std::chrono::steady_clock::now() - t0).count() / 2.0;
    double vals[1] = {mine};
    const int ops[1] = {0};
    SK_HIP_TRY(b_small_.alloc(2 * 9 * (size_t)C_ + 6 * retained_pts_.size() + 64 + 16 * (size_t)W));
    rc = gather_rank_scalars(vals, 1, ops);
    if (rc) return rc;
    est_allreduce_s_ = vals[0] / W;
    collect_allreduce_time(true);
    phase_[5] = 0.0;
    if (est_allreduce_s_ <= est_saved_s_) return SK_OK;
  }
  distribution_ = SK_DISTRIBUTION_REPLICATED;
  opt_.allreduce = nullptr; opt_.world = 1; opt_.rank = 0;
  b_pack_.release();
  return SK_OK;
}

int BalSolver::setup() {
  setup_t0_ = stage_last_ = std::chrono::steady_clock::now();
  std::string why;
  if (!problem_is_bal_shaped(*problem_, &why)) { set_error("%s", why.c_str()); return SK_ERR_UNSUPPORTED; }
  const Problem& p = *problem_;
  int rc = SK_OK;
  Structure st;
  (void)bal_block_shape(p, &res_size_, &cam_size_, &pt_size_);
  bal_index_problem(p, &cam_block_, &pt_block_, &st.ocam, &st.opt);
  C_ = (int)cam_block_.size(); P_total_ = (int)pt_block_.size();
  st.Creal = C_;
  n_ = 9 * C_; rhs_row_ = n_; npad_ = ((n_ + 1 + 127) / 128) * 128;
  if ((rc = init_queues())) return rc;
  if ((rc = plan_layout(&st))) return rc;
  stage("camera order applied");
  plan_pack();
  if ((rc = cut_camera_sequence(&st))) return rc;
  if (opt_.allreduce && !distribution_decided_) {
    if ((rc = prepare_pack())) return rc;
    if (!segmented_ && (rc = choose_distribution(st.opt))) return rc;
  }
  const LocalInputs li{&st.ocam, &st.opt, C_, P_total_, opt_.world, opt_.rank, segmented_, segments_, role_, &seg_off_, &retained_pts_, &retained_cam_};
  LocalStructure ls = index_local_structure(p, li);
  if (!ls.error.empty()) { set_error("%s", ls.error.c_str()); return SK_ERR_UNSUPPORTED; }
  local_pt_ = ls.local_pt; P_ = ls.P; P_own_ = ls.P_own; N_ = ls.N;
  host_obs_ = ls.host_obs; host_cf_ = ls.host_cf;
  stage("dissection, local observations, camera lists");
  add_pair_lists(&ls, C_, kLongSegment);
  if (!ls.error.empty()) { set_error("%s", ls.error.c_str()); return SK_ERR_UNSUPPORTED; }
  if ((rc = upload_structure(ls))) return rc;
  stage("pair lists, uploads");
  const bool with_pseudo = !struct_ocam_.empty();
  const FrontInputs fi{with_pseudo ? &struct_ocam_ : &st.ocam, with_pseudo ? &struct_opt_ : &st.opt, with_pseudo ? struct_P_ : P_total_, C_, npad_, rhs_row_,
                       &env_last_, &env_tail_, dissected_, segmented_, segments_, role_, &seg_off_, &sep_first_, cam_b_, border_members_, &root_last_, &root_tail_};
  if ((rc = allocate_fronts(layout_fronts(fi)))) return rc;
  stage("fronts, zero pass, tables");
  if ((rc = bind_device_view(ls))) return rc;
  if (bounded_ && (rc = upload_bounds())) return rc;
  if ((rc = agree_with_ranks())) return rc;
  stage("device view, the ranks' agreement");
  return SK_OK;
}

int BalSolver::init_queues() {
  const Problem& p = *problem_;
  SK_HIP_TRY(cholesky_init());
  {
    bool host_or_tape = false;
    for (size_t b = 0; b < p.rb_functor.size() && !host_or_tape; ++b) host_or_tape = p.rb_functor[b] == SK_FUNCTOR_HOST_CALLBACK || p.tape_of_block(b) != nullptr;
    if (dogleg() && host_or_tape) {
      for (size_t b = 0; b < p.rb_functor.size(); ++b)
        if (p.rb_functor[b] == SK_FUNCTOR_HOST_CALLBACK) { set_error("DOGLEG with host-evaluated (director) residual blocks under DENSE_SCHUR is not supported"); return SK_ERR_UNSUPPORTED; }
    }
    graph_mode_ = npad_ / 128 <= 8 && !opt_.allreduce && !host_or_tape && opt_.dissection != SK_DISSECTION_ON && dev_knobs().dissect_at < 0 && opt_.graph_replay && !dogleg() && !bounded_;
    if (graph_mode_) opt_.lookahead = false;
  }
  chol_ctx_.resident = chol_ctx_b_.resident = opt_.resident_kernels;
  if (opt_.lookahead && chol_ctx_.init() != hipSuccess) {
    (void)hipGetLastError();
    opt_.lookahead = false;
  }
  if (opt_.lookahead) cholesky_prepare(&chol_ctx_, stream_);
  if (opt_.allreduce && opt_.world > 1) {
    SK_HIP_TRY(b_small_.alloc(2 * 9 * ((size_t)C_ + (size_t)(std::max(1536, opt_.retained_max) + 12) / 3) + 6 * (size_t)(std::max(1536, opt_.retained_max) + 12) + 64 + 16 * (size_t)opt_.world));
    double off[1] = {opt_.lookahead ? 0.0 : 1.0};
    int rc = gather_rank_scalars_signed(off, 1);
    if (rc) return rc;
    if (off[0] > 0.0) opt_.lookahead = false;
  }
  return SK_OK;
}

int BalSolver::plan_layout(Structure* st) {
  const Problem& p = *problem_;
  const int Creal = st->Creal;
  RetainedGraphs rgraphs;
  const bool many_segments = opt_.allreduce && opt_.world > 1 && opt_.distribution_mode == SK_DISTRIBUTION_SEGMENTED && opt_.max_segments != 2;
  const bool border_ok = opt_.envelope && opt_.border != SK_BORDER_OFF && opt_.dissection != SK_DISSECTION_ON && dev_knobs().dissect_at < 0 && !many_segments;
  const bool retained_ok = opt_.retained != SK_RETAINED_OFF && opt_.dissection != SK_DISSECTION_ON && dev_knobs().dissect_at < 0 && !graph_mode_;
  CameraOrderPlan plan;
  auto pick = [&](bool with_memory_order) {
    ReducedSystemPlan rp = plan_reduced_system(p, cam_block_, st->ocam, st->opt, Creal, P_total_, with_memory_order, border_ok, opt_.border,
                                               retained_ok ? opt_.retained : SK_RETAINED_OFF, opt_.retained_max);
    plan = std::move(rp.order);
    retained_pts_ = rp.retained; rgraphs = std::move(rp.graphs);
    retained_without_us_ = rp.without_us; retained_model_us_ = retained_pts_.empty() ? 0.0 : plan.model_us;
    unsigned long long h = 1469598103934665603ull;
    for (int v : retained_pts_) { h ^= (unsigned)v; h *= 1099511628211ull; }
    for (int v : plan.id) { h ^= (unsigned)v; h *= 1099511628211ull; }
    for (int v : plan.last) { h ^= (unsigned)v; h *= 1099511628211ull; }
    for (int v : plan.tail) { h ^= (unsigned)v; h *= 1099511628211ull; }
    order_hash_ = (double)(h >> 12);
  };
  stage("structure, queue trial");
  pick(true);
  stage("plan of the reduced system");
  if (opt_.allreduce && opt_.world > 1) {
    double v[2] = {order_hash_, -order_hash_};
    int rc = gather_rank_scalars_signed(v, 2);
    if (rc) return rc;
    if (v[0] != order_hash_ || v[1] != -order_hash_) pick(false);
  }
  const std::vector<int>& id = plan.id;
  camera_order_ = plan.candidate;
  if (!retained_pts_.empty()) {
    pseudo_cams_ = rgraphs.Cx - Creal;
    C_ = rgraphs.Cx;
    n_ = 9 * C_; rhs_row_ = n_; npad_ = ((n_ + 1 + 127) / 128) * 128;
    struct_ocam_ = rgraphs.ocam_x; struct_opt_ = rgraphs.opt_x; struct_P_ = rgraphs.Px;
    for (int& c : struct_ocam_) c = id[c];
    st->band_ocam = rgraphs.ocam_g; st->band_opt = rgraphs.opt_g;
    for (int& c : st->band_ocam) c = id[c];
    retained_cam_.resize(retained_pts_.size());
    for (size_t k = 0; k < retained_pts_.size(); ++k) retained_cam_[k] = id[Creal + (int)k / 3];
  }
  std::vector<int> cb(C_, -1);
  for (int c = 0; c < Creal; ++c) cb[id[c]] = cam_block_[c];
  cam_block_.swap(cb);
  for (int& c : st->ocam) c = id[c];
  const int nblk = npad_ / 128;
  const double best = plan.flops, full = cholesky_syrk_flops(npad_, 1, nullptr);
  border_plain_us_ = plan.border.plain_us;
  if (plan.bordered) {
    env_tail_ = plan.tail;
    border_cams_ = plan.border.border_cams; border_gap_ = plan.border.gap;
    border_model_us_ = plan.border.model_us;
  }
  group_ = opt_.group_or(opt_.envelope && best < 0.5 * full ? 1 : 3);
  st->env_for_model = plan.last;
  if (opt_.envelope) env_last_ = plan.last;
  else env_tail_.clear();
  if (dev_knobs().debug_envelope && opt_.envelope) {
    long h = 0;
    for (int c = 0; c < nblk; ++c) h += env_last_[c] - c;
    std::fprintf(stderr, "[skeres_amd] camera order %d (0 first appearance, 1 memory, 2 RCM); envelope: %d block columns, mean height %.1f; "
                 "trailing-update flops %.3e (full %.3e)\n", camera_order_, nblk, (double)h / nblk, best, full);
    if (border_cams_ > 0)
      std::fprintf(stderr, "[skeres_amd] loop closures: %d cameras in a trailing border (visits split at jumps of more than %d cameras): chain model %.0f us against %.0f\n",
                   border_cams_, border_gap_, border_model_us_, border_plain_us_);
  }
  return SK_OK;
}

static void pack_rows(int nblk, const std::vector<int>& last, const std::vector<int>& tail, std::vector<int>* col0, std::vector<long long>* off) {
  col0->assign(nblk, 0);
  off->assign(nblk + 1, 0);
  if (!last.empty()) *col0 = cholesky_row_first_cols(nblk, last.data(), tail.empty() ? nullptr : tail.data());
  for (int kb = 0; kb < nblk; ++kb) (*off)[kb + 1] = (*off)[kb] + (long long)128 * 128 * (kb + 1 - (*col0)[kb]);
}
void BalSolver::plan_pack() {
  pack_rows(npad_ / 128, env_last_, env_tail_, &pack_col0_h_, &pack_off_h_);
  packed_elems_ = (size_t)pack_off_h_.back();
}
int BalSolver::prepare_pack() {
  if (opt_.reduce_buffer) {
    if (opt_.reduce_buffer_bytes < packed_elems_ * sizeof(double)) { set_error("reduce buffer too small: need %zu bytes", packed_elems_ * sizeof(double)); return SK_ERR_INVALID_ARGUMENT; }
    b_pack_.adopt(static_cast<double*>(opt_.reduce_buffer), packed_elems_);
  } else {
    SK_HIP_TRY(b_pack_.alloc(packed_elems_));
  }
  SK_HIP_TRY(b_pack_.zero(stream_));
  return SK_OK;
}
int BalSolver::shard_or_replicate(const std::vector<int>& opt) {
  int rc = prepare_pack();
  if (rc) return rc;
  rc = choose_distribution(opt);
  if (rc) return rc;
  distribution_decided_ = true;
  return SK_OK;
}

int BalSolver::cut_camera_sequence(Structure* st) {
  const bool seg_modes = opt_.distribution_mode == SK_DISTRIBUTION_AUTO || opt_.distribution_mode == SK_DISTRIBUTION_SEGMENTED;
  if (opt_.allreduce && opt_.world > 1 && pseudo_cams_ > 0 && !seg_modes) {
    int rc = shard_or_replicate(st->opt);
    if (rc) return rc;
  }
  for (int pass = 0; pass < 2; ++pass) {
    const bool multi = opt_.allreduce != nullptr && opt_.world >= 2;
    border_members_ = env_tail_.empty() ? 0 : border_cams_ + pseudo_cams_;
    const BandStructure band{&st->ocam, &st->opt, C_, P_total_, &st->band_ocam, &st->band_opt, &struct_ocam_, &struct_opt_, struct_P_,
                             &st->env_for_model, &env_tail_, npad_ / 128, pseudo_cams_, border_members_};
    const bool band_chain_bound = band_is_chain_bound(band);
    const bool two_seg_try = multi && pseudo_cams_ > 0 && seg_modes && !distribution_decided_;
    const bool pseudo_border = border_members_ > 0 && (!multi || two_seg_try) && (pseudo_cams_ > 0 || band_chain_bound);
    const int Cband = C_ - (pseudo_border ? border_members_ : 0);
    const bool plan_ok = opt_.dissection != SK_DISSECTION_OFF && opt_.envelope && opt_.lookahead && opt_.cholesky_group == 0 && (env_tail_.empty() || pseudo_border);
    bool may_dissect = plan_ok && (multi ? ((pseudo_cams_ == 0 || two_seg_try) && seg_modes)
                                         : (!opt_.allreduce && chol_ctx_b_.init_secondary(chol_ctx_) == hipSuccess));
    if (!may_dissect) (void)hipGetLastError();
    if (!plan_ok && opt_.distribution_mode == SK_DISTRIBUTION_SEGMENTED) {
      set_error("the segmented distribution needs the library's own factorisation plan (envelope, look-ahead, no explicit group); not supported with these options");
      return SK_ERR_UNSUPPORTED;
    }
    CutPlan cuts;
    if (may_dissect) {
      const bool lockstep_cut = !multi && opt_.dissection == SK_DISSECTION_AUTO && opt_.resident_kernels && cholesky_chain_enabled(&chol_ctx_);
      const CutFlags flags{multi, two_seg_try, lockstep_cut, pseudo_border, opt_.dissection, opt_.distribution_mode, opt_.max_segments, opt_.world, dev_knobs().dissect_at};
      cuts = plan_cuts(band, flags, &cut_model_);
      if (cuts.needs_pair_claim) {
        if (!pair_claimed_) pair_claimed_ = cholesky_claim_pair_servers(&chol_ctx_);
        if (!pair_claimed_ && cuts.drop_without_claim) { cuts.a.clear(); cuts.b.clear(); }
      }
    }
    if (two_seg_try && cuts.a.empty() && opt_.distribution_mode != SK_DISTRIBUTION_SEGMENTED) {
      int rc = shard_or_replicate(st->opt);
      if (rc) return rc;
      continue;
    }
    if (multi && opt_.distribution_mode == SK_DISTRIBUTION_SEGMENTED && cuts.a.empty()) {
      set_error("the segmented distribution needs a separator in the camera sequence (no point seen from both ends); not supported for this problem");
      return SK_ERR_UNSUPPORTED;
    }
    if (!cuts.a.empty()) adopt_cuts(cuts, Cband, multi, st);
    break;
  }
  return SK_OK;
}

void BalSolver::adopt_cuts(const CutPlan& cuts, int Cband, bool multi, Structure* st) {
  dissected_ = true;
  segmented_ = multi;
  const CutNumbering num = apply_cuts(cuts, Cband, C_);
  seg_off_ = num.seg_off; sep_first_ = num.sep_first;
  const std::vector<int>& fin = num.fin;
  segments_ = (int)cuts.a.size() + 1;
  cam_b_ = seg_off_[segments_];
  std::vector<int> cb2(C_);
  for (int c = 0; c < C_; ++c) cb2[fin[c]] = cam_block_[c];
  cam_block_.swap(cb2);
  for (int& c : st->ocam) c = fin[c];
  for (int& c : struct_ocam_) c = fin[c];
  for (int& c : retained_cam_) c = fin[c];
  env_tail_.clear();
  cam_a_ = seg_off_[1];
  if (!segmented_) return;
  distribution_ = SK_DISTRIBUTION_SEGMENTED;
  role_ = opt_.rank % segments_;
  replica_ = opt_.rank >= segments_;
  fold_world_ = segments_;
  my_lo_ = seg_off_[role_]; my_hi_ = seg_off_[role_ + 1];
  std::vector<int> sep_off;
  for (int f : sep_first_) sep_off.push_back(9 * (std::min(f, C_ - border_members_) - cam_b_));
  root_tail_.clear();
  root_last_ = root_envelope(sep_off, 9 * border_members_, &root_tail_);
  pack_rows((9 * (C_ - cam_b_) + 1 + 127) / 128, root_last_, root_tail_, &pack_col0_h_, &pack_off_h_);
  packed_elems_ = (size_t)pack_off_h_.back();
}

int BalSolver::upload_structure(const LocalStructure& ls) {
  const Problem& p = *problem_;
  hipStream_t s = stream_;
  SK_HIP_TRY(b_cam_.upload(ls.cam, s)); SK_HIP_TRY(b_pt_.upload(ls.pt, s)); SK_HIP_TRY(b_obs_.upload(ls.obs, s));
  if (ls.tape) { tape_mode_ = true; SK_HIP_TRY(tape_dev_.upload(*ls.tape, s)); }
  SK_HIP_TRY(b_pt_start_.upload(ls.pt_start, s)); SK_HIP_TRY(b_cam_start_.upload(ls.cam_start, s)); SK_HIP_TRY(b_cam_obs_.upload(ls.cam_obs, s));
  SK_HIP_TRY(b_obs_slot_.upload(ls.slot, s));
  if (!ls.dup_cam.empty()) { SK_HIP_TRY(b_dup_a_.upload(ls.dup_a, s)); SK_HIP_TRY(b_dup_b_.upload(ls.dup_b, s)); SK_HIP_TRY(b_dup_cam_.upload(ls.dup_cam, s)); }
  num_dup_ = (int)ls.dup_cam.size();
  SK_HIP_TRY(b_seg_start_.upload(ls.seg_start, s)); SK_HIP_TRY(b_seg_row_.upload(ls.seg_row, s)); SK_HIP_TRY(b_seg_col_.upload(ls.seg_col, s));
  SK_HIP_TRY(b_pair_row_.upload(ls.pair_row, s)); SK_HIP_TRY(b_pair_col_.upload(ls.pair_col, s));
  SK_HIP_TRY(b_short_segs_.upload(ls.short_segs, s)); SK_HIP_TRY(b_long_segs_.upload(ls.long_segs, s));
  d_.num_short_segments = (int)ls.short_segs.size(); d_.num_long_segments = (int)ls.long_segs.size();
  const size_t nc = 9 * (size_t)C_, np = 3 * (size_t)P_, nx = nc + np;
  std::vector<double> x(nx, 0.0);
  for (int i = 0; i < C_; ++i) if (cam_block_[i] >= 0) std::memcpy(&x[9 * (size_t)i], p.block_ptr[cam_block_[i]], cam_size_ * sizeof(double));
  for (int q = 0; q < P_; ++q) std::memcpy(&x[nc + 3 * (size_t)q], p.block_ptr[pt_block_[local_pt_[q]]], pt_size_ * sizeof(double));
  SK_HIP_TRY(b_xc_.upload(x, s)); SK_HIP_TRY(b_xc_new_.alloc(nx));
  SK_HIP_TRY(b_scale_.alloc(nx)); SK_HIP_TRY(b_colsq_.alloc(nx)); SK_HIP_TRY(b_gs_.alloc(nx)); SK_HIP_TRY(b_step_.alloc(nx));
  {
    std::vector<double> free_mask(nx, 1.0);
    auto mask_block = [&](int block, size_t off, int size, int padded) {
      for (int k = size; k < padded; ++k) free_mask[off + k] = 0.0;
      if ((size_t)block < p.block_constant.size() && p.block_constant[block]) { for (int k = 0; k < size; ++k) free_mask[off + k] = 0.0; return; }
      const int pi = (size_t)block < p.block_param.size() ? p.block_param[block] : -1;
      if (pi < 0) return;
      const LocalParameterization& lp = p.params[pi];
      if (lp.type == kParamSubset) for (int k = 0; k < size; ++k) if ((lp.constant_mask >> k) & 1u) free_mask[off + k] = 0.0;
    };
    for (int i = 0; i < C_; ++i) {
      if (cam_block_[i] >= 0) mask_block(cam_block_[i], 9 * (size_t)i, cam_size_, 9);
      else for (int k = 0; k < 9; ++k) free_mask[9 * (size_t)i + k] = 0.0;
    }
    for (int q = 0; q < P_; ++q) mask_block(pt_block_[local_pt_[q]], nc + 3 * (size_t)q, pt_size_, 3);
    SK_HIP_TRY(hipMemcpyAsync(b_scale_.p, free_mask.data(), nx * sizeof(double), hipMemcpyHostToDevice, s));
    SK_HIP_TRY(hipStreamSynchronize(s));
  }
  SK_HIP_TRY(b_y_.alloc(npad_ + 128));
  SK_HIP_TRY(b_r_.alloc(2 * (size_t)N_)); SK_HIP_TRY(b_F_.alloc(18 * (size_t)N_)); SK_HIP_TRY(b_Fcam_.alloc(kFcam * (size_t)N_)); SK_HIP_TRY(b_E_.alloc(6 * (size_t)N_));
  SK_HIP_TRY(b_W_.alloc(kWs * (size_t)N_)); SK_HIP_TRY(b_rt_.alloc(5 * (size_t)N_));
  if (res_size_ < 2 || cam_size_ < 9 || pt_size_ < 3) {
    SK_HIP_TRY(b_r_.zero(s)); SK_HIP_TRY(b_F_.zero(s)); SK_HIP_TRY(b_E_.zero(s));
  }
  SK_HIP_TRY(b_M_.alloc(6 * (size_t)P_)); SK_HIP_TRY(b_q_.alloc(3 * (size_t)P_));
  if (pseudo_cams_ > 0) {
    std::vector<unsigned char> pseudo(C_, 0);
    for (int i = 0; i < C_; ++i) pseudo[i] = cam_block_[i] < 0 ? 1 : 0;
    SK_HIP_TRY(b_pseudo_.upload(pseudo, s));
    SK_HIP_TRY(b_kept_pt_.upload(ls.kept_pt, s)); SK_HIP_TRY(b_kept_cam_.upload(ls.kept_cam, s));
    if (segmented_) { SK_HIP_TRY(b_kept_home_.upload(ls.kept_home, s)); SK_HIP_TRY(b_kept_global_.upload(ls.kept_global, s)); }
    SK_HIP_TRY(b_kept_obs_.upload(ls.kept_obs, s)); SK_HIP_TRY(b_kept_obs_slot_.upload(ls.kept_obs_slot, s));
    num_kept_obs_ = (int)ls.kept_obs.size();
  }
  return SK_OK;
}

int BalSolver::allocate_fronts(const FrontLayout& lay) {
  hipStream_t s = stream_;
  for (int f = 0; f < 3; ++f) fr_[f] = lay.fr[f];
  border_blocks_ = lay.border_blocks;
  {
    const FrontHost& e = fr_[2];
    SK_HIP_TRY(b_S_.alloc(e.s_off + e.dim * e.dim));
    SK_HIP_TRY(b_Linv_.alloc(e.linv_off + (size_t)e.ncols * 128 * 128)); SK_HIP_TRY(b_Linv_.zero(s));
    const size_t y_end = e.y_off + e.dim;
    SK_HIP_TRY(b_yf_.alloc(y_end)); SK_HIP_TRY(b_yf_.zero(s)); SK_HIP_TRY(b_wf_.alloc(y_end)); SK_HIP_TRY(b_ybB_.alloc((size_t)std::max(1, border_blocks_) * 128));
  }
  if (opt_.allreduce) { SK_HIP_TRY(b_pack_col0_.upload(pack_col0_h_, s)); SK_HIP_TRY(b_pack_off_.upload(pack_off_h_, s)); }
  cholesky_prepare(&chol_ctx_, s);
  if (dissected_ && !segmented_) SK_HIP_TRY(chol_ctx_b_.init_secondary(chol_ctx_));
  SK_HIP_TRY(b_S_.zero(s));
  for (int f = 0; f < 3; ++f) {
    const FrontHost& F = fr_[f];
    if (F.nblk == 0) continue;
    std::vector<int> col0(F.nblk, 0);
    const bool chain_here = chain_ok() && (f != 1 || tail_chain());
    const int widen = F.last.empty() ? 1 : std::max(group_, cholesky_plan_max_group(cholesky_plan(F.nblk, group_, F.last.data(), chain_here, F.ncols, F.tail_rows, F.tl())));
    if (!F.last.empty()) {
      const std::vector<int> first = cholesky_row_first_cols(F.nblk, F.last.data(), F.tl(), F.tail_rows);
      for (int i = 0; i < F.nblk; ++i) col0[i] = std::max(0, first[i] - (widen - 1));
    }
    SK_HIP_TRY(b_zero_col0_f_[f].upload(col0, s));
    std::vector<int> col_min(F.nblk);
    for (int i = 0; i < F.nblk; ++i) col_min[i] = i < F.ncols ? i : F.ncols;
    SK_HIP_TRY(b_zero_min_f_[f].upload(col_min, s));
  }
  for (int f = 0; f < 2; ++f) if (!lay.border_row_h[f].empty()) SK_HIP_TRY(b_border_row_[f].upload(lay.border_row_h[f], s));
  if (segmented_) { SK_HIP_TRY(b_leaf_map_.upload(lay.leaf_map_h, s)); SK_HIP_TRY(b_leaf_gmap_.upload(lay.leaf_gmap_h, s)); }
  if (dissected_ && !segmented_) { SK_HIP_TRY(b_mapB_.upload(lay.mapB, s)); mapB_involution_ = lay.mapB_involution; }
  partial_stride_ = std::max(std::max(std::max(bal_partial_blocks(N_), bal_point_blocks(P_) + 1), (9 * C_ + 255) / 256), 256) + bal_partial_blocks((int)host_obs_.size());
  SK_HIP_TRY(b_partial_.alloc(4 * (size_t)partial_stride_));
  SK_HIP_TRY(b_scal_.alloc(kDevSlots)); SK_HIP_TRY(b_scal_.zero(s)); SK_HIP_TRY(b_small_.alloc(2 * 9 * (size_t)C_ + 6 * retained_pts_.size() + 64 + 16 * (size_t)opt_.world));
  fail_p_ = reinterpret_cast<int*>(b_scal_.p + kFail); info_p_ = reinterpret_cast<int*>(b_scal_.p + kInfo);
  SK_HIP_TRY(hipHostMalloc(reinterpret_cast<void**>(&h_scal_), kHostSlots * sizeof(double), hipHostMallocDefault));
  if (dogleg()) {
    BalDev shape{}; shape.C = C_; shape.P = P_; shape.N = N_;
    const size_t nx = 9 * (size_t)C_ + 3 * (size_t)P_;
    dl_.stride = dogleg_partial_stride(shape);
    SK_HIP_TRY(b_dl_vec_.alloc(2 * nx)); SK_HIP_TRY(b_dl_vec_.zero(s));
    SK_HIP_TRY(b_dl_partial_.alloc(9 * (size_t)dl_.stride)); SK_HIP_TRY(b_dl_partial_.zero(s));
    SK_HIP_TRY(b_dl_scal_.alloc(16)); SK_HIP_TRY(b_dl_scal_.zero(s));
    dl_.s = b_dl_vec_.p; dl_.g = b_dl_vec_.p + nx; dl_.partial = b_dl_partial_.p; dl_.scal = b_dl_scal_.p;
  }
  return SK_OK;
}

int BalSolver::bind_device_view(const LocalStructure& ls) {
  const Problem& p = *problem_;
  hipStream_t s = stream_;
  const size_t nc = 9 * (size_t)C_, nx = nc + 3 * (size_t)P_;
  d_.C = C_; d_.P = P_; d_.N = N_;
  d_.pseudo = pseudo_cams_ > 0 ? b_pseudo_.p : nullptr; d_.num_kept = pseudo_cams_ > 0 ? (int)ls.kept_pt.size() : 0; d_.kept_pt = b_kept_pt_.p; d_.kept_cam = b_kept_cam_.p;
  d_.num_kept_obs = pseudo_cams_ > 0 ? num_kept_obs_ : 0; d_.kept_obs = b_kept_obs_.p; d_.kept_obs_slot = b_kept_obs_slot_.p;
  d_.kept_home = segmented_ && pseudo_cams_ > 0 ? b_kept_home_.p : nullptr; d_.kept_global = segmented_ && pseudo_cams_ > 0 ? b_kept_global_.p : nullptr;
  d_.num_dup = num_dup_; d_.dup_a = b_dup_a_.p; d_.dup_b = b_dup_b_.p; d_.dup_cam = b_dup_cam_.p;
  d_.res_size = res_size_; d_.cam_size = cam_size_; d_.pt_size = pt_size_;
  d_.cam = b_cam_.p; d_.pt = b_pt_.p; d_.obs = b_obs_.p; d_.pt_start = b_pt_start_.p; d_.cam_start = b_cam_start_.p; d_.cam_obs = b_cam_obs_.p; d_.obs_slot = b_obs_slot_.p;
  d_.num_segments = (int)ls.seg_row.size(); d_.seg_start = b_seg_start_.p; d_.seg_row = b_seg_row_.p; d_.seg_col = b_seg_col_.p;
  d_.short_segments = b_short_segs_.p; d_.long_segments = b_long_segs_.p;
  d_.pair_row_obs = b_pair_row_.p; d_.pair_col_obs = b_pair_col_.p;
  d_.xc = b_xc_.p; d_.xp = b_xc_.p + nc; d_.xc_new = b_xc_new_.p; d_.xp_new = b_xc_new_.p + nc;
  d_.scale_c = b_scale_.p; d_.scale_p = b_scale_.p + nc; d_.colsq_c = b_colsq_.p; d_.colsq_p = b_colsq_.p + nc;
  d_.gs_c = b_gs_.p; d_.gs_p = b_gs_.p + nc; d_.step_c = b_step_.p; d_.step_p = b_step_.p + nc;
  d_.y_c = b_y_.p; d_.r = b_r_.p; d_.F = b_F_.p; d_.Fcam = b_Fcam_.p; d_.E = b_E_.p; d_.What = b_W_.p; d_.u = b_rt_.p; d_.M = b_M_.p; d_.q = b_q_.p;
  for (int f = 0; f < 3; ++f) {
    d_.front[f].S = fr_[f].nblk > 0 ? b_S_.p + fr_[f].s_off : nullptr; d_.front[f].ld = (int)fr_[f].dim; d_.front[f].interior = fr_[f].ncols * 128;
    d_.front[f].rhs_row = fr_[f].rhs_row; d_.front[f].border_row = f < 2 ? b_border_row_[f].p : nullptr;
    d_.y_front[f] = b_yf_.p + fr_[f].y_off;
  }
  d_.seg_lo = segmented_ ? my_lo_ : 0; d_.cam_a = segmented_ ? my_hi_ : cam_a_; d_.cam_b = cam_b_;
  d_.S = d_.front[2].S; d_.ld = d_.front[2].ld; d_.rhs_row = fr_[2].rhs_row;
  if (segmented_) {
    const FrontHost& F = fr_[0];
    leaf_.S = d_.front[0].S; leaf_.ld = (long)F.dim; leaf_.nblk = F.nblk; leaf_.ncols = F.ncols; leaf_.last = F.env();
    leaf_.Linv = b_Linv_.p + F.linv_off; leaf_.rhs_row = F.rhs_row; leaf_.tail_rows = F.tail_rows; leaf_.spike = role_ > 0 && role_ + 1 < segments_;
    leaf_.tail = F.tl();
  }
  if (dissected_ && !segmented_) {
    auto view = [&](int f) {
      FrontView v;
      v.S = d_.front[f].S; v.ld = (long)fr_[f].dim; v.nblk = fr_[f].nblk; v.ncols = fr_[f].ncols; v.last = fr_[f].env();
      v.Linv = b_Linv_.p + fr_[f].linv_off; v.rhs_row = fr_[f].rhs_row; v.tail = fr_[f].tl();
      return v;
    };
    ds_.A = view(0); ds_.B = view(1); ds_.R = view(2); ds_.border_blocks = border_blocks_; ds_.mapB = b_mapB_.p; ds_.mapB_involution = mapB_involution_;
  }
  d_.partial = b_partial_.p; d_.partial_stride = partial_stride_; d_.fail_flag = fail_p_;
  d_.loss_nodes = nullptr; d_.loss_root = p.rb_loss.empty() ? -1 : p.rb_loss[0]; d_.loss_of_obs = nullptr;
  {
    bool mixed = false;
    int any_root = -1;
    for (size_t b = 0; b < p.rb_loss.size(); ++b) { mixed = mixed || p.rb_loss[b] != p.rb_loss[0]; any_root = std::max(any_root, p.rb_loss[b]); }
    if (mixed) {
      std::vector<int> roots(N_);
      for (int o = 0; o < N_; ++o) roots[o] = p.rb_loss[ls.order[o]];
      SK_HIP_TRY(b_loss_of_obs_.upload(roots, s));
      d_.loss_of_obs = b_loss_of_obs_.p; d_.loss_root = any_root;
    }
  }
  if (d_.loss_root >= 0) { SK_HIP_TRY(b_loss_nodes_.upload(p.loss_nodes, s)); d_.loss_nodes = b_loss_nodes_.p; }
  d_.is_host = nullptr; d_.num_host = (int)host_obs_.size(); d_.host_obs = nullptr; d_.host_rows = nullptr;
  if (!host_obs_.empty()) {
    std::vector<unsigned char> flag(N_, 0);
    for (int o : host_obs_) flag[o] = 1;
    SK_HIP_TRY(b_is_host_.upload(flag, s)); SK_HIP_TRY(b_host_obs_.upload(host_obs_, s));
    SK_HIP_TRY(b_host_rows_.alloc(host_obs_.size() * (size_t)kHostRow));
    d_.is_host = b_is_host_.p; d_.host_obs = b_host_obs_.p; d_.host_rows = b_host_rows_.p;
    h_cam_ = ls.cam; h_pt_ = ls.pt;
    host_x_.resize(nx); host_rows_h_.resize(host_obs_.size() * (size_t)kHostRow);
  }
  graph_mode_ = graph_mode_ && host_obs_.empty() && !dissected_ && !tape_mode_;
  zero_by_backsolve_ = !graph_mode_ && !dev_knobs().schedule_plain && opt_.resident_kernels;
  for (int f = 0; f < 3; ++f) if (fr_[f].nblk > 0 && !cholesky_backsolve_resident(fr_[f].nblk)) zero_by_backsolve_ = false;
  SK_HIP_TRY(hipStreamSynchronize(s));
  return SK_OK;
}

int BalSolver::upload_bounds() {
  const Problem& p = *problem_;
  hipStream_t s = stream_;
  const size_t nc = 9 * (size_t)C_, nx = nc + 3 * (size_t)P_;
  const double inf = std::numeric_limits<double>::infinity();
  std::vector<double> box(2 * nx);
  std::fill(box.begin(), box.begin() + (long)nx, -inf); std::fill(box.begin() + (long)nx, box.end(), inf);
  auto fill = [&](int block, size_t off, int size) {
    for (int k = 0; k < size; ++k) { box[off + k] = p.lower_bound((size_t)block, k); box[nx + off + k] = p.upper_bound((size_t)block, k); }
  };
  for (int i = 0; i < C_; ++i) if (cam_block_[i] >= 0) fill(cam_block_[i], 9 * (size_t)i, cam_size_);
  for (int q = 0; q < P_; ++q) fill(pt_block_[local_pt_[q]], nc + 3 * (size_t)q, pt_size_);
  SK_HIP_TRY(b_bd_box_.upload(box, s));
  bd_.stride = bounds_partial_stride((int)nx);
  SK_HIP_TRY(b_bd_partial_.alloc(6 * (size_t)bd_.stride)); SK_HIP_TRY(b_bd_partial_.zero(s));
  SK_HIP_TRY(b_bd_scal_.alloc(8)); SK_HIP_TRY(b_bd_scal_.zero(s));
  bd_.lo = b_bd_box_.p; bd_.hi = b_bd_box_.p + nx; bd_.partial = b_bd_partial_.p; bd_.scal = b_bd_scal_.p;
  launch_box_project(d_.xc, bd_.lo, bd_.hi, (int)nx, s);
  SK_HIP_TRY(hipStreamSynchronize(s));
  return SK_OK;
}

int BalSolver::agree_with_ranks() {
  if (!opt_.allreduce) return SK_OK;
  double v[2] = {order_hash_, -order_hash_};
  int rc = gather_rank_scalars_signed(v, 2);
  if (rc) return rc;
  if (v[0] != order_hash_ || v[1] != -order_hash_) {
    set_error("the ranks derived different camera orders for the reduced system (are the residual blocks added in the same order on every rank?)");
    return SK_ERR_COMM;
  }
  double off[1] = {chain_ok() && !chain_live() ? 1.0 : 0.0};
  rc = gather_rank_scalars_signed(off, 1);
  if (rc) return rc;
  if (off[0] > 0.0) cholesky_disable_chain(&chol_ctx_);
  return SK_OK;
}
bool BalSolver::rank_table_on_device(int K) const { return opt_.allreduce != nullptr && opt_.world > 1 && opt_.world * K <= kRankTableSlots; }
int BalSolver::enqueue_rank_table(int mode, int K) {
  double* dev = rank_table_dev();
  launch_bal_pack_rank_scalars(b_scal_.p, dev, opt_.rank, opt_.world, mode, segmented_, stream_);
  int rc = allreduce(dev, (size_t)opt_.world * K);
  if (rc) return rc;
  SK_HIP_TRY(hipMemcpyAsync(h_scal_ + kRankTable, dev, (size_t)opt_.world * K * sizeof(double), hipMemcpyDeviceToHost, stream_));
  return SK_OK;
}
int BalSolver::fold_rank_table(const double* table, double* vals, int K, const int* ops) {
  const int W = opt_.world;
  const int fold = fold_world_ > 0 ? std::min(fold_world_, W) : W;
  for (int k = 0; k < K; ++k) {
    double a = 0.0;
    for (int r = 0; r < fold; ++r) a = ops[k] ? std::max(a, table[(size_t)r * K + k]) : a + table[(size_t)r * K + k];
    vals[k] = a;
  }
  return SK_OK;
}
int BalSolver::exchange_rank_table(const double* vals, int K, std::vector<double>* table) {
  table->assign((size_t)opt_.world * K, 0.0);
  for (int k = 0; k < K; ++k) (*table)[(size_t)opt_.rank * K + k] = vals[k];
  double* dev = rank_table_dev();
  SK_HIP_TRY(hipMemcpyAsync(dev, table->data(), table->size() * sizeof(double), hipMemcpyHostToDevice, stream_));
  int rc = allreduce(dev, table->size());
  if (rc) return rc;
  SK_HIP_TRY(hipMemcpyAsync(table->data(), dev, table->size() * sizeof(double), hipMemcpyDeviceToHost, stream_));
  SK_HIP_TRY(hipStreamSynchronize(stream_));
  return SK_OK;
}
int BalSolver::gather_rank_scalars_signed(double* vals, int K) {
  std::vector<double> table;
  int rc = exchange_rank_table(vals, K, &table);
  if (rc) return rc;
  for (int k = 0; k < K; ++k) {
    double a = table[k];
    for (int r = 1; r < opt_.world; ++r) a = std::max(a, table[(size_t)r * K + k]);
    vals[k] = a;
  }
  return SK_OK;
}
int BalSolver::gather_rank_scalars(double* vals, int K, const int* ops) {
  if (!opt_.allreduce) return SK_OK;
  std::vector<double> table;
  int rc = exchange_rank_table(vals, K, &table);
  return rc ? rc : fold_rank_table(table.data(), vals, K, ops);
}

int BalSolver::evaluate_with_jacobian(bool first) {
  hipStream_t s = stream_;
  const size_t nc = 9 * (size_t)C_, np = 3 * (size_t)P_;
  SK_HIP_TRY(hipEventRecord(ev_[kEvBegin], s));
  const bool graph = graph_ok() && !first;
  const bool replay = graph && g_eval_[parity_] != nullptr;
  if (graph && !replay && hipStreamBeginCapture(s, hipStreamCaptureModeThreadLocal) != hipSuccess) { (void)hipGetLastError(); graph_mode_ = false; return evaluate_with_jacobian(first); }
  CaptureGuard capture(s, graph && !replay, &graph_mode_);
  if (!replay) {
  kt_.begin("bal_eval_jac", s);
  if (tape_mode_) launch_bal_eval_jac_tape(d_, tape_dev_, s); else launch_bal_eval_jac(d_, s);
  kt_.end("bal_eval_jac", s);
  int nb = bal_partial_blocks(N_);
  if (d_.num_host > 0) {
    bool failed = false;
    int rc = host_callbacks(d_.xc, true, &failed);
    if (rc) return rc;
    if (failed) return SK_ERR_EVALUATION_FAILED;
    nb += launch_bal_host_jac(d_, nb, s);
  }
  kt_.begin("bal_cam_records", s); launch_bal_cam_records(d_, s); kt_.end("bal_cam_records", s);
  kt_.begin("bal_reduce", s); launch_bal_reduce(d_, s); kt_.end("bal_reduce", s);
  if (opt_.allreduce) {
    double* buf = b_small_.p;
    const size_t nk = segmented_ && pseudo_cams_ > 0 ? 6 * retained_pts_.size() : 0;
    if (nk) SK_HIP_TRY(hipMemsetAsync(buf + 2 * nc, 0, nk * sizeof(double), s));
    if (replica_) {
      SK_HIP_TRY(hipMemsetAsync(buf, 0, 2 * nc * sizeof(double), s));
    } else {
      SK_HIP_TRY(hipMemcpyAsync(buf, d_.colsq_c, nc * sizeof(double), hipMemcpyDeviceToDevice, s));
      SK_HIP_TRY(hipMemcpyAsync(buf + nc, d_.gs_c, nc * sizeof(double), hipMemcpyDeviceToDevice, s));
      if (nk) launch_bal_kept_sums(d_, buf + 2 * nc, (int)retained_pts_.size(), true, s);
    }
    int rc = allreduce(buf, 2 * nc + nk);
    if (rc) return rc;
    SK_HIP_TRY(hipMemcpyAsync(d_.colsq_c, buf, nc * sizeof(double), hipMemcpyDeviceToDevice, s));
    SK_HIP_TRY(hipMemcpyAsync(d_.gs_c, buf + nc, nc * sizeof(double), hipMemcpyDeviceToDevice, s));
    if (nk) launch_bal_kept_sums(d_, buf + 2 * nc, (int)retained_pts_.size(), false, s);
  }
  if (first && opt_.jacobi_scaling) {
    launch_jacobi_scale(b_colsq_.p, b_scale_.p, (int)(nc + np), s);
    launch_bal_scale_jac(d_, s);
    launch_bal_cam_records(d_, s);
    launch_apply_scale_to_reductions(b_colsq_.p, b_gs_.p, b_scale_.p, (int)(nc + np), s);
  }
  if (!opt_.allreduce) {
    const int g = launch_grad_max_xnorm(b_gs_.p, b_scale_.p, d_.xc, (int)(nc + np), b_partial_.p + (size_t)partial_stride_, partial_stride_, s);
    ReduceRows rows;
    rows.n = 3;
    rows.row[0] = 0; rows.count[0] = nb; rows.out[0] = b_scal_.p + kSumSq;
    rows.row[1] = 1; rows.count[1] = g; rows.is_max[1] = 1; rows.out[1] = b_scal_.p + kGradMaxCam;
    rows.row[2] = 2; rows.count[2] = g; rows.out[2] = b_scal_.p + kXSqCam;
    launch_final_reduce_rows(b_partial_.p, partial_stride_, rows, s);
  } else {
  launch_final_reduce(b_partial_.p, partial_stride_, nb, 1, 0, b_scal_.p + kSumSq, s);
  int c_lo = 0, c_n = (int)nc;
  if (segmented_) { c_lo = 9 * my_lo_; c_n = 9 * (my_hi_ - my_lo_); }
  int gc = launch_grad_max_xnorm(d_.gs_c + c_lo, d_.scale_c + c_lo, d_.xc + c_lo, c_n, b_partial_.p, partial_stride_, s);
  if (segmented_ && role_ == 0) {
    const int lo2 = 9 * cam_b_, n2 = (int)nc - lo2;
    gc += launch_grad_max_xnorm(d_.gs_c + lo2, d_.scale_c + lo2, d_.xc + lo2, n2, b_partial_.p + gc, partial_stride_, s);
  }
  launch_final_reduce(b_partial_.p, partial_stride_, gc, 2, 1, b_scal_.p + kGradMaxCam, s);
  const int np_own = 3 * P_own_;
  const int gp = launch_grad_max_xnorm(d_.gs_p, d_.scale_p, d_.xp, np_own, b_partial_.p + 2 * (size_t)partial_stride_, partial_stride_, s);
  launch_final_reduce(b_partial_.p + 2 * (size_t)partial_stride_, partial_stride_, np_own ? gp : 0, 2, 1, b_scal_.p + kGradMaxPt, s);
  }
  SK_HIP_TRY(hipMemcpyAsync(h_scal_ + kEvalFirst, b_scal_.p + kEvalFirst, (kEvalLast + 1 - kEvalFirst) * sizeof(double), hipMemcpyDeviceToHost, s));
  if (bounded_) {
    kt_.begin("bounded_grad_max_xnorm", s); launch_bounded_grad_max_xnorm(b_gs_.p, b_scale_.p, d_.xc, (int)(nc + np), bd_, s); kt_.end("bounded_grad_max_xnorm", s);
    SK_HIP_TRY(hipMemcpyAsync(h_scal_ + kBounds + kBdGradMax, bd_.scal + kBdGradMax, (kBdActive + 1 - kBdGradMax) * sizeof(double), hipMemcpyDeviceToHost, s));
  }
  }
  if (graph) {
    if (!replay) { capture.release(); int rc = finish_capture(s, &g_eval_[parity_]); if (rc) return rc; if (!graph_mode_) return evaluate_with_jacobian(first); }
    SK_HIP_TRY(hipGraphLaunch(g_eval_[parity_], s));
  }
  SK_HIP_TRY(hipEventRecord(ev_[kEvJac], s));
  const bool dev_gather = rank_table_on_device(3) && !graph;
  if (dev_gather) { int rc = enqueue_rank_table(0, 3); if (rc) return rc; }
  SK_HIP_TRY(hipStreamSynchronize(s));
  const double sumsq = h_scal_[kSumSq];
  const double gmax_c = h_scal_[kGradMaxCam], x2_c = h_scal_[kXSqCam];
  double loc[3] = {sumsq, segmented_ ? std::max(h_scal_[kGradMaxPt], gmax_c) : h_scal_[kGradMaxPt], h_scal_[kXSqPt] + (segmented_ ? x2_c : 0.0)};
  const int ops3[3] = {0, 1, 0};
  int rc = dev_gather ? fold_rank_table(h_scal_ + kRankTable, loc, 3, ops3) : gather_rank_scalars(loc, 3, ops3);
  if (rc) return rc;
  add_phases(0, 0);
  cost_ = 0.5 * loc[0];
  gmax_ = segmented_ ? loc[1] : std::max(gmax_c, loc[1]);
  xnorm_ = std::sqrt((segmented_ ? 0.0 : x2_c) + loc[2]);
  if (bounded_) { gmax_ = h_scal_[kBounds + kBdGradMax]; active_bounds_ = (long)h_scal_[kBounds + kBdActive]; }
  if (!std::isfinite(cost_) || (!opt_.allreduce && (!std::isfinite(gmax_c) || !std::isfinite(loc[1])))) return SK_ERR_EVALUATION_FAILED;
  return SK_OK;
}

int BalSolver::linear_solve(double radius, LinearSolve* out) {
  bool chain_lost = false;
  int rc = solve_once(radius, out, &chain_lost);
  if (rc == SK_OK && chain_lost) rc = solve_once(radius, out, &chain_lost);
  return rc;
}

int BalSolver::solve_once(double radius, LinearSolve* out, bool* chain_lost) {
  hipStream_t s = stream_;
  *chain_lost = false;
  *out = LinearSolve();
  ++n_linear_solves_;
  SK_HIP_TRY(hipEventRecord(ev_[kEvBegin], s));
  const bool graph = graph_ok();
  const bool replay = graph && g_step_[parity_] != nullptr;
  bool candidate_failed = false;
  if (graph) {
    h_scal_[kRadius] = radius;
    if (!replay && hipStreamBeginCapture(s, hipStreamCaptureModeThreadLocal) != hipSuccess) { (void)hipGetLastError(); graph_mode_ = false; return solve_once(radius, out, chain_lost); }
  }
  CaptureGuard capture(s, graph && !replay, &graph_mode_);
  if (!replay) {
    d_.lm_lo = opt_.min_lm_diagonal; d_.lm_hi = opt_.max_lm_diagonal; d_.lm_radius = radius; d_.lm_radius_dev = nullptr;
    if (graph) {
      SK_HIP_TRY(hipMemcpyAsync(b_scal_.p + kRadiusDev, h_scal_ + kRadius, sizeof(double), hipMemcpyHostToDevice, s));
      d_.lm_radius_dev = b_scal_.p + kRadiusDev;
    }
    Backsolve bs;
    bs.resident = opt_.resident_kernels && cholesky_backsolve_resident(npad_ / 128) ? 1 : 0;
    bs.zero_after = zero_by_backsolve_ && bs.resident;
    int rc = enqueue_schur_assembly(bs, graph);
    if (rc == SK_OK) rc = enqueue_factor_backsolve(bs, graph);
    if (rc == SK_OK) rc = enqueue_point_backsub(graph);
    if (rc == SK_OK && !dogleg()) rc = enqueue_candidate_cost(2, &candidate_failed);
    if (rc) return rc;
    if (!graph) SK_HIP_TRY(hipEventRecord(ev_[kEvCost], s));
    SK_HIP_TRY(hipMemcpyAsync(h_scal_ + kStepFirst, b_scal_.p + kStepFirst, (kStepLast + 1 - kStepFirst) * sizeof(double), hipMemcpyDeviceToHost, s));
  }
  const bool dev_gather = rank_table_on_device(4) && !graph;
  if (dev_gather) { int rc = enqueue_rank_table(1, 4); if (rc) return rc; }
  if (graph) {
    if (!replay) { capture.release(); int rc = finish_capture(s, &g_step_[parity_]); if (rc) return rc; if (!graph_mode_) return solve_once(radius, out, chain_lost); }
    SK_HIP_TRY(hipGraphLaunch(g_step_[parity_], s));
    SK_HIP_TRY(hipEventRecord(ev_[kEvCost], s));
  }
  SK_HIP_TRY(hipStreamSynchronize(s));
  if (graph) {
    add_phase(2, ev_[kEvBegin], ev_[kEvCost]);
  } else {
    add_phases(1, 4);
  }
  const int fail = host_flag(kFail), info = host_flag(kInfo);
  if (info != 0) need_full_zero_ = true;
  if (cholesky_note_info(opt_.lookahead ? &chol_ctx_ : nullptr, info) && !opt_.allreduce) {
    if (graph_mode_) {
      for (hipGraphExec_t* g : {&g_step_[0], &g_step_[1], &g_eval_[0], &g_eval_[1]}) if (*g) { (void)hipGraphExecDestroy(*g); *g = nullptr; }
      graph_mode_ = false;
    }
    *chain_lost = true;
    return SK_OK;
  }
  if (dogleg()) {
    out->valid = (fail | info) == 0;
    out->dl = dogleg::Scalars::from(h_scal_ + kDogleg + kDlScalars);
    return SK_OK;
  }
  double loc[4] = {h_scal_[kCandSumSq], h_scal_[kModel], h_scal_[kStepSqPt] + (segmented_ ? h_scal_[kStepSqCam] : 0.0), (double)(fail | info)};
  const int ops4[4] = {0, 0, 0, 1};
  int rc = dev_gather ? fold_rank_table(h_scal_ + kRankTable, loc, 4, ops4) : gather_rank_scalars(loc, 4, ops4);
  if (rc) return rc;
  if (opt_.allreduce && loc[3] >= 2.0) cholesky_disable_chain(&chol_ctx_);
  const double step_sq = (segmented_ ? 0.0 : h_scal_[kStepSqCam]) + loc[2];
  if (loc[3] != 0.0 || !std::isfinite(step_sq) || !std::isfinite(loc[1])) return SK_OK;
  out->valid = true;
  out->model_cost_change = -loc[1];
  out->cost = candidate_failed ? std::numeric_limits<double>::max() : 0.5 * loc[0];
  out->step_norm = std::sqrt(bounded_ ? h_scal_[kBounds + kBdStepSq] : step_sq);
  out->g_delta = h_scal_[kBounds + kBdGDelta]; out->max_delta = h_scal_[kBounds + kBdMaxDelta];
  return SK_OK;
}

int BalSolver::enqueue_schur_assembly(const Backsolve& bs, bool graph) {
  hipStream_t s = stream_;
  kt_.begin("memset_S", s);
  for (int f = 0; f < 3; ++f)
    if (fr_[f].nblk > 0) launch_zero_envelope(d_.front[f].S, (int)fr_[f].dim, (zero_by_backsolve_ && !need_full_zero_) ? b_zero_min_f_[f].p : b_zero_col0_f_[f].p, fr_[f].nblk, s);
  kt_.end("memset_S", s);
  need_full_zero_ = !bs.zero_after;
  SK_HIP_TRY(hipMemsetAsync(b_scal_.p + kFail, 0, (kInfo + 1 - kFail) * sizeof(double), s));
  launch_bal_point_block(d_, s);
  launch_bal_kept_points(d_, s);
  launch_bal_obs_precompute(d_, s);
  kt_.begin("bal_cam_diag", s); launch_bal_cam_diag(d_, s); kt_.end("bal_cam_diag", s);
  kt_.begin("bal_pair", s); launch_bal_pair(d_, s); kt_.end("bal_pair", s);
  if (opt_.allreduce && !segmented_) {
    launch_tri_pack(d_.S, npad_, b_pack_.p, npad_ / 128, b_pack_col0_.p, b_pack_off_.p, true, s);
    int rc = allreduce(b_pack_.p, packed_elems_);
    if (rc) return rc;
    launch_tri_pack(d_.S, npad_, b_pack_.p, npad_ / 128, b_pack_col0_.p, b_pack_off_.p, false, s);
  }
  if (!segmented_) {
    BalFinishRanges r;
    int k = 0;
    for (int f = 0; f < 2; ++f)
      if (fr_[f].nblk > 0 && fr_[f].ncols * 128 > 9 * fr_[f].cams) { r.S[k] = d_.front[f].S; r.ld[k] = (int)fr_[f].dim; r.from[k] = 9 * fr_[f].cams; r.to[k] = fr_[f].ncols * 128; r.value[k] = 1.0; ++k; }
    r.S[k] = d_.front[2].S; r.ld[k] = (int)fr_[2].dim; r.from[k] = fr_[2].rhs_row; r.to[k] = fr_[2].rhs_row + 1; r.value[k] = 1e300; ++k;
    if ((int)fr_[2].dim > fr_[2].rhs_row + 1) { r.S[k] = d_.front[2].S; r.ld[k] = (int)fr_[2].dim; r.from[k] = fr_[2].rhs_row + 1; r.to[k] = (int)fr_[2].dim; r.value[k] = 1.0; ++k; }
    launch_bal_finish_all(d_, r, s);
  } else {
    launch_bal_finish_S(d_, 3, s);
    for (int f = 0; f < 2; ++f)
      if (fr_[f].nblk > 0) launch_set_diagonal(d_.front[f].S, (int)fr_[f].dim, 9 * fr_[f].cams, fr_[f].ncols * 128, 1.0, s);
  }
  if (!graph) SK_HIP_TRY(hipEventRecord(ev_[kEvAssemble], s));
  return SK_OK;
}

int BalSolver::enqueue_factor_backsolve(const Backsolve& bs, bool graph) {
  hipStream_t s = stream_;
  CholeskyContext* ctx = opt_.lookahead ? &chol_ctx_ : nullptr;
  int* bs_info = bs.resident ? info_p_ : nullptr;
  double* yf[3] = {b_yf_.p + fr_[0].y_off, b_yf_.p + fr_[1].y_off, b_yf_.p + fr_[2].y_off};
  double* wf[3] = {b_wf_.p + fr_[0].y_off, b_wf_.p + fr_[1].y_off, b_wf_.p + fr_[2].y_off};
  const bool prefilled = bs.resident != 0;
  if (prefilled) SK_HIP_TRY(hipMemsetAsync(b_yf_.p, 0xff, (fr_[0].dim + fr_[1].dim + fr_[2].dim) * sizeof(double), s));
  if (segmented_) {
    const FrontView& L = leaf_;
    const FrontHost& R = fr_[2];
    double* Rs = d_.front[2].S;
    double* RLinv = b_Linv_.p + R.linv_off;
    if (L.ncols > 0) {
      cholesky_factor(L.S, L.ld, L.nblk * 128, L.Linv, info_p_, group_, s, ctx, &kt_, L.last, chain_ok(), L.ncols, L.tail_rows, nullptr, L.tail);
      cholesky_border_add(Rs, (long)R.dim, L.S, L.ld, L.ncols, L.nblk - L.ncols, b_leaf_map_.p, s);
    }
    if (replica_) SK_HIP_TRY(hipMemsetAsync(b_pack_.p, 0, packed_elems_ * sizeof(double), s));
    else launch_tri_pack(Rs, (int)R.dim, b_pack_.p, R.nblk, b_pack_col0_.p, b_pack_off_.p, true, s);
    int rc = allreduce(b_pack_.p, packed_elems_);
    if (rc) return rc;
    launch_tri_pack(Rs, (int)R.dim, b_pack_.p, R.nblk, b_pack_col0_.p, b_pack_off_.p, false, s);
    launch_bal_finish_S(d_, 4, s);
    launch_set_diagonal(Rs, (int)R.dim, R.rhs_row, R.rhs_row + 1, 1e300, s);
    launch_set_diagonal(Rs, (int)R.dim, R.rhs_row + 1, (int)R.dim, 1.0, s);
    cholesky_factor(Rs, (long)R.dim, (int)R.dim, RLinv, info_p_, group_, s, ctx, &kt_, R.env(), chain_ok(), -1, 1, nullptr, R.tl());
    cholesky_backsolve(Rs, (long)R.dim, 9 * R.cams, (int)R.dim, R.rhs_row, RLinv, wf[2], yf[2], s, &kt_, R.env(), bs_info, R.tl(), bs.zero_after, bs.resident, prefilled);
    if (L.ncols > 0) {
      cholesky_gather_map(yf[2], b_leaf_gmap_.p, b_ybB_.p, (L.nblk - L.ncols) * 128, s);
      cholesky_backsolve_front(L.S, L.ld, L.nblk, L.ncols, L.rhs_row, L.Linv, b_ybB_.p, wf[0], yf[0], s, L.last, L.spike, L.tail_rows, bs_info, bs.zero_after, L.tail, nullptr, bs.resident, prefilled);
    }
  } else if (dissected_) {
    cholesky_dissected_factor(ds_, info_p_, group_, s, ctx, &chol_ctx_b_, &kt_, &kt_b_, chain_ok());
    cholesky_dissected_backsolve(ds_, 9 * fr_[2].cams, wf[2], yf[2], wf[0], yf[0], wf[1], yf[1], b_ybB_.p, s, &chol_ctx_b_, &kt_, bs_info, bs.zero_after, bs.resident, prefilled);
  } else {
    const FrontHost& R = fr_[2];
    cholesky_factor(d_.front[2].S, (long)R.dim, (int)R.dim, b_Linv_.p, info_p_, group_, s, ctx, &kt_, R.env(), chain_ok(), -1, 1, nullptr, R.tl());
    cholesky_backsolve(d_.front[2].S, (long)R.dim, n_, (int)R.dim, R.rhs_row, b_Linv_.p, wf[2], yf[2], s, &kt_, R.env(), bs_info, R.tl(), bs.zero_after, bs.resident, prefilled);
  }
  if (!graph) SK_HIP_TRY(hipEventRecord(ev_[kEvChol], s));
  return SK_OK;
}

int BalSolver::enqueue_point_backsub(bool graph) {
  hipStream_t s = stream_;
  int lo = 0, hi = 9 * C_, lo2 = 0, hi2 = 0;
  if (segmented_) {
    lo = 9 * my_lo_; hi = 9 * my_hi_;
    if (role_ == 0) { lo2 = 9 * cam_b_; hi2 = 9 * C_; }
  }
  launch_bal_backsub(d_, b_scal_.p + kStepSqCam, lo, hi, lo2, hi2, s);
  if (dogleg()) {
    kt_.begin("dogleg_vector_norms", s); launch_dogleg_vector_norms(d_, dl_, s); kt_.end("dogleg_vector_norms", s);
    kt_.begin("bal_dogleg_products", s); launch_bal_dogleg_products(d_, dl_, s); kt_.end("bal_dogleg_products", s);
    launch_dogleg_reduce_scalars(dl_, s);
    SK_HIP_TRY(hipMemcpyAsync(h_scal_ + kDogleg + kDlScalars, dl_.scal + kDlScalars, (kDlStepSq - kDlScalars) * sizeof(double), hipMemcpyDeviceToHost, s));
  }
  if (bounded_) {
    kt_.begin("bal_directional_derivative", s); launch_bal_directional_derivative(d_, bd_, s); kt_.end("bal_directional_derivative", s);
    kt_.begin("bal_bounded_candidate", s); launch_bal_bounded_candidate(d_, bd_, 1.0, s); kt_.end("bal_bounded_candidate", s);
    SK_HIP_TRY(hipMemcpyAsync(h_scal_ + kBounds + kBdStepSq, bd_.scal + kBdStepSq, (kBdMaxDelta + 1 - kBdStepSq) * sizeof(double), hipMemcpyDeviceToHost, s));
  }
  if (!graph) SK_HIP_TRY(hipEventRecord(ev_[kEvBacksub], s));
  return SK_OK;
}

int BalSolver::enqueue_candidate_cost(int rows, bool* failed) {
  hipStream_t s = stream_;
  kt_.begin("bal_eval_cost", s);
  if (tape_mode_) launch_bal_eval_cost_tape(d_, tape_dev_, s); else launch_bal_eval_cost(d_, s);
  kt_.end("bal_eval_cost", s);
  int nb_cost = bal_partial_blocks(N_);
  if (d_.num_host > 0) {
    int rc = host_callbacks(d_.xc_new, false, failed);
    if (rc) return rc;
    nb_cost += launch_bal_host_cost(d_, nb_cost, s);
  }
  launch_final_reduce(b_partial_.p, partial_stride_, nb_cost, rows, 0, b_scal_.p + kCandSumSq, s);
  return SK_OK;
}

int BalSolver::trial_cost(const double* step_sq_dev, int step_sq_slot, double* cost, double* step_norm) {
  hipStream_t s = stream_;
  SK_HIP_TRY(hipEventRecord(ev_[kEvBacksub], s));
  bool failed = false;
  int rc = enqueue_candidate_cost(1, &failed);
  if (rc) return rc;
  SK_HIP_TRY(hipEventRecord(ev_[kEvCost], s));
  SK_HIP_TRY(hipMemcpyAsync(h_scal_ + kCandSumSq, b_scal_.p + kCandSumSq, sizeof(double), hipMemcpyDeviceToHost, s));
  SK_HIP_TRY(hipMemcpyAsync(h_scal_ + step_sq_slot, step_sq_dev, sizeof(double), hipMemcpyDeviceToHost, s));
  SK_HIP_TRY(hipStreamSynchronize(s));
  add_phases(3, 4);
  *cost = failed ? std::numeric_limits<double>::max() : 0.5 * h_scal_[kCandSumSq];
  *step_norm = std::sqrt(h_scal_[step_sq_slot]);
  return SK_OK;
}

int BalSolver::bounded_trial(double alpha, double* cost, double* step_norm) {
  SK_HIP_TRY(hipEventRecord(ev_[kEvBegin], stream_));
  kt_.begin("bal_bounded_candidate", stream_); launch_bal_bounded_candidate(d_, bd_, alpha, stream_); kt_.end("bal_bounded_candidate", stream_);
  return trial_cost(bd_.scal + kBdStepSq, kBounds + kBdStepSq, cost, step_norm);
}

int BalSolver::dogleg_trial(double a, double b, double* cost, double* step_norm) {
  SK_HIP_TRY(hipEventRecord(ev_[kEvBegin], stream_));
  kt_.begin("bal_dogleg_combine", stream_); launch_bal_dogleg_combine(d_, dl_, a, b, stream_); kt_.end("bal_dogleg_combine", stream_);
  return trial_cost(dl_.scal + kDlStepSq, kDogleg + kDlStepSq, cost, step_norm);
}

int BalSolver::finish_capture(hipStream_t s, hipGraphExec_t* exec) {
  hipGraph_t g = nullptr;
  hipError_t e = hipStreamEndCapture(s, &g);
  if (e == hipSuccess && g) e = hipGraphInstantiate(exec, g, nullptr, nullptr, 0);
  if (g) (void)hipGraphDestroy(g);
  if (e != hipSuccess || !*exec) {
    (void)hipGetLastError();
    *exec = nullptr;
    graph_mode_ = false;
    std::fprintf(stderr, "[skeres_amd] hipGraph capture of the iteration failed (%s): launches are enqueued one by one\n", hipGetErrorString(e));
  }
  return SK_OK;
}

int BalSolver::host_callbacks(const double* x_dev, bool jac, bool* failed) {
  *failed = false;
  const size_t nc = 9 * (size_t)C_, np = 3 * (size_t)P_;
  SK_HIP_TRY(hipMemcpyAsync(host_x_.data(), x_dev, (nc + np) * sizeof(double), hipMemcpyDeviceToHost, stream_));
  SK_HIP_TRY(hipStreamSynchronize(stream_));
  for (size_t h = 0; h < host_obs_.size(); ++h) {
    const int o = host_obs_[h];
    const CostFunction* cf = host_cf_[h];
    const double* params[2] = {&host_x_[9 * (size_t)h_cam_[o]], &host_x_[nc + 3 * (size_t)h_pt_[o]]};
    double* row = &host_rows_h_[h * (size_t)kHostRow];
    for (int k = 0; k < kHostRow; ++k) row[k] = 0.0;
    if (res_size_ == 2 && cam_size_ == 9 && pt_size_ == 3) {
      double* jptr[2] = {row + 2, row + 20};
      if (!cf->callback(cf->user, params, row, jac ? jptr : nullptr)) { *failed = true; return SK_OK; }
    } else {
      double res[2] = {0.0, 0.0}, jc[2 * 9], jq[2 * 3];
      double* jptr[2] = {jc, jq};
      if (!cf->callback(cf->user, params, res, jac ? jptr : nullptr)) { *failed = true; return SK_OK; }
      for (int r = 0; r < res_size_; ++r) {
        row[r] = res[r];
        if (jac) {
          for (int k = 0; k < cam_size_; ++k) row[2 + 9 * r + k] = jc[r * cam_size_ + k];
          for (int k = 0; k < pt_size_; ++k) row[20 + 3 * r + k] = jq[r * pt_size_ + k];
        }
      }
    }
  }
  SK_HIP_TRY(hipMemcpyAsync(b_host_rows_.p, host_rows_h_.data(), host_rows_h_.size() * sizeof(double), hipMemcpyHostToDevice, stream_));
  SK_HIP_TRY(hipStreamSynchronize(stream_));
  return SK_OK;
}

int BalSolver::write_back() {
  const size_t nc = 9 * (size_t)C_, np = 3 * (size_t)P_;
  std::vector<double> x(nc + np);
  SK_HIP_TRY(hipMemcpyAsync(x.data(), d_.xc, (nc + np) * sizeof(double), hipMemcpyDeviceToHost, stream_));
  SK_HIP_TRY(hipStreamSynchronize(stream_));
  if (segmented_) {
    std::vector<double> cams(nc, 0.0);
    if (!replica_) {
      const size_t lo = 9 * (size_t)my_lo_, hi = 9 * (size_t)my_hi_;
      std::memcpy(&cams[lo], &x[lo], (hi - lo) * sizeof(double));
      if (role_ == 0) std::memcpy(&cams[9 * (size_t)cam_b_], &x[9 * (size_t)cam_b_], (nc - 9 * (size_t)cam_b_) * sizeof(double));
    }
    DevBuf<double> tmpc;
    SK_HIP_TRY(tmpc.upload(cams, stream_));
    int rc = allreduce(tmpc.p, cams.size());
    if (rc) return rc;
    SK_HIP_TRY(hipMemcpyAsync(x.data(), tmpc.p, nc * sizeof(double), hipMemcpyDeviceToHost, stream_));
    SK_HIP_TRY(hipStreamSynchronize(stream_));
  }
  for (int i = 0; i < C_; ++i) if (cam_block_[i] >= 0) std::memcpy(problem_->block_ptr[cam_block_[i]], &x[9 * (size_t)i], cam_size_ * sizeof(double));
  if (!opt_.allreduce) {
    for (int q = 0; q < P_; ++q) std::memcpy(problem_->block_ptr[pt_block_[local_pt_[q]]], &x[nc + 3 * (size_t)q], pt_size_ * sizeof(double));
    return SK_OK;
  }
  std::vector<double> all(3 * (size_t)P_total_, 0.0);
  if (!replica_)
    for (int q = 0; q < P_own_; ++q) std::memcpy(&all[3 * (size_t)local_pt_[q]], &x[nc + 3 * (size_t)q], 3 * sizeof(double));
  DevBuf<double> tmp;
  SK_HIP_TRY(tmp.upload(all, stream_));
  int rc = allreduce(tmp.p, all.size());
  if (rc) return rc;
  SK_HIP_TRY(hipMemcpyAsync(all.data(), tmp.p, all.size() * sizeof(double), hipMemcpyDeviceToHost, stream_));
  SK_HIP_TRY(hipStreamSynchronize(stream_));
  for (int q = 0; q < P_total_; ++q) std::memcpy(problem_->block_ptr[pt_block_[q]], &all[3 * (size_t)q], pt_size_ * sizeof(double));
  return SK_OK;
}

}

std::unique_ptr<SolverBase> make_bal_solver(const Options& o, Problem* p) { return std::unique_ptr<SolverBase>(new BalSolver(o, p)); }

}
```

skeres_amd/csrc/capi.hip:

```cpp
#include <cmath>
#include <cstdlib>
#include <new>

#include "bal_kernels.hpp"
#include "chol_solve.hpp"
#include "dense_kernels.hpp"
#include "dense_rows_kernels.hpp"
#include "evaluate_kernels.hpp"
#include "cgnr_plan.hpp"
#include "inner_plan.hpp"
#include "covariance.hpp"
#include "covariance_plan.hpp"
#include "evaluate_plan.hpp"
#include "solver.hpp"

using namespace sk;

struct sk_ptrvec { std::vector<double*> v; };
struct sk_loss_function { LossFunction l; };
struct sk_cost_function { CostFunction c; };
struct sk_problem { Problem p; };
struct sk_local_parameterization { LocalParameterization p; };
struct sk_options { Options o; };
struct sk_summary { Summary s; };
struct sk_solver { std::unique_ptr<SolverBase> impl; };
struct sk_covariance_options { CovarianceOptions o; };
struct sk_covariance { Covariance c; explicit sk_covariance(const CovarianceOptions& o) : c(o) {} };
struct sk_evaluate_options { EvaluateOptions o; bool launch_timing = false; double launch_seconds[kEvaluatePhases] = {0, 0, 0, 0, 0, 0}; };

static std::string g_program_name;

#define SK_GUARD_BEGIN try {
#define SK_GUARD_END(ret)                                                   \
  } catch (const std::bad_alloc&) { set_error("out of host memory"); return ret; } \
  catch (const std::exception& e) { set_error("internal error: %s", e.what()); return ret; } \
  catch (...) { set_error("internal error"); return ret; }

namespace sk {
int Problem::intern_loss(const LossFunction* l) {
  if (!l || l->nodes.empty()) return -1;
  std::string key(reinterpret_cast<const char*>(l->nodes.data()), l->nodes.size() * sizeof(LossNode));
  auto it = loss_root_of.find(key);
  if (it != loss_root_of.end()) return it->second;
  const int base = (int)loss_nodes.size();
  for (LossNode n : l->nodes) {
    if (n.f >= 0) n.f += base;
    if (n.g >= 0) n.g += base;
    loss_nodes.push_back(n);
  }
  const int root = (int)loss_nodes.size() - 1;
  loss_root_of.emplace(std::move(key), root);
  has_loss = true;
  return root;
}
}

namespace sk { int rotation_apply(int op, int row_major, int jet_dim, const double* in, int n, double* out); }

namespace sk {
const DevKnobs& dev_knobs() {
  static const DevKnobs knobs = [] {
    DevKnobs k;
    auto num = [](const char* name, int def) { const char* e = getenv(name); return e ? atoi(e) : def; };
    k.chain_server = num("SK_CHOL_CHAIN_SERVER", 1);
    k.bs_resident = num("SK_BS_RESIDENT", 1);
    k.chain_stamps = getenv("SK_CHAIN_STAMPS");
    k.bs_stamps = getenv("SK_BS_STAMPS");
    if (const char* e = getenv("SK_DEBUG")) {
      const std::string topics = std::string(",") + e + ",";
      k.debug_queues = topics.find(",queues,") != std::string::npos;
      k.debug_envelope = topics.find(",envelope,") != std::string::npos;
      k.debug_segments = topics.find(",segments,") != std::string::npos;
      k.debug_setup = topics.find(",setup,") != std::string::npos;
      k.debug_chain_abort = topics.find(",chain_abort,") != std::string::npos;
    }
    k.queue_shift = num("SK_QUEUE_SHIFT", 0);
    k.chain_queues = num("SK_CHAIN_QUEUES", -1);
    k.pair_max_trailing = num("SK_CHAIN_PAIR_MAX_TRAILING", 0);
    k.dissect_at = num("SK_DISSECT_AT", -1);
    k.schedule_plain = num("SK_SCHEDULE_PLAIN", 0);
    k.cgnr_batch = num("SK_CGNR_BATCH", 0);
    k.inner_batch = num("SK_INNER_BATCH", 0);
    k.chain_xcd_local = num("SK_CHAIN_XCD_LOCAL", 0);
    if (const char* e = getenv("SK_BS_PAIR")) k.bs_pair = atoi(e);
    if (const char* e = getenv("SK_BS_SPREAD")) k.bs_spread = atoi(e);
    if (const char* e = getenv("SK_CHAIN_EARLY_SERVER")) k.chain_early_server = atoi(e);
    if (const char* e = getenv("SK_BULK_RESERVE")) {
      k.bulk_reserve = atoi(e);
      const char* c = strchr(e, ',');
      k.bulk_reserve_early = c ? atoi(c + 1) : k.bulk_reserve;
    }
    return k;
  }();
  return knobs;
}
}

extern "C" {

const char* sk_version(void) { return "skeres_amd 0.1 (gfx950)"; }
const char* sk_last_error(void) { return get_error(); }
void sk_init_logging(const char* name) { g_program_name = name ? name : ""; }
int sk_device_count(void) { int n = 0; if (hipGetDeviceCount(&n) != hipSuccess) return 0; return n; }

double* sk_array_new(int n) { if (n < 0) return nullptr; return static_cast<double*>(std::calloc((size_t)(n > 0 ? n : 1), sizeof(double))); }
void sk_array_free(double* a) { std::free(a); }
double sk_array_getitem(const double* a, int i) { return a[i]; }
void sk_array_setitem(double* a, int i, double v) { a[i] = v; }
double* sk_array_slice(double* buffer, int start) { return &buffer[start]; }
void sk_array_copy_in(double* dst, const double* src, int n) { if (n > 0) std::memcpy(dst, src, (size_t)n * sizeof(double)); }
void sk_array_copy_out(const double* src, double* dst, int n) { if (n > 0) std::memcpy(dst, src, (size_t)n * sizeof(double)); }

int sk_matrix_is_null(double* const* m) { return m == nullptr; }
double* sk_matrix_row(double* const* m, int i) { return m[i]; }

sk_ptrvec* sk_ptrvec_new(void) { return new (std::nothrow) sk_ptrvec(); }
void sk_ptrvec_free(sk_ptrvec* v) { delete v; }
void sk_ptrvec_add(sk_ptrvec* v, double* p) { v->v.push_back(p); }
int sk_ptrvec_size(const sk_ptrvec* v) { return (int)v->v.size(); }
double* sk_ptrvec_get(const sk_ptrvec* v, int i) { return v->v[i]; }
void sk_ptrvec_set(sk_ptrvec* v, int i, double* p) { v->v[i] = p; }
double** sk_ptrvec_to_pointer_pointer(sk_ptrvec* v) { return v->v.empty() ? nullptr : v->v.data(); }

int sk_rotation_apply(int op, int row_major, int jet_dim, const double* in, int n, double* out) {
  SK_GUARD_BEGIN
  return sk::rotation_apply(op, row_major, jet_dim, in, n, out);
  SK_GUARD_END(SK_ERR_INVALID_ARGUMENT)
}

sk_loss_function* sk_loss_trivial(void) { return new (std::nothrow) sk_loss_function(); }
void sk_loss_free(sk_loss_function* l) { delete l; }

static sk_loss_function* loss_leaf_new(int type, double a, double b) {
  if (!(a > 0.0) || (type == kLossTolerant && !(b > 0.0))) { set_error("loss function parameters must be positive"); return nullptr; }
  sk_loss_function* l = new (std::nothrow) sk_loss_function();
  if (!l) { set_error("out of host memory"); return nullptr; }
  LossNode n; n.type = type; n.f = n.g = -1; n.depth = 0; n.a = a; n.b = b;
  l->l.nodes.push_back(n);
  return l;
}
sk_loss_function* sk_loss_huber(double a) { return loss_leaf_new(kLossHuber, a, 0.0); }
sk_loss_function* sk_loss_soft_l_one(double a) { return loss_leaf_new(kLossSoftLOne, a, 0.0); }
sk_loss_function* sk_loss_cauchy(double a) { return loss_leaf_new(kLossCauchy, a, 0.0); }
sk_loss_function* sk_loss_tukey(double a) { return loss_leaf_new(kLossTukey, a, 0.0); }
sk_loss_function* sk_loss_tolerant(double a, double b) { return loss_leaf_new(kLossTolerant, a, b); }

static int loss_append(std::vector<LossNode>* dst, const sk_loss_function* child, int* depth) {
  *depth = -1;
  if (!child || child->l.nodes.empty()) return -1;
  const int base = (int)dst->size();
  for (LossNode n : child->l.nodes) {
    if (n.f >= 0) n.f += base;
    if (n.g >= 0) n.g += base;
    dst->push_back(n);
  }
  *depth = dst->back().depth;
  return (int)dst->size() - 1;
}
sk_loss_function* sk_loss_composed(const sk_loss_function* f, const sk_loss_function* g) {
  SK_GUARD_BEGIN
  sk_loss_function* l = new sk_loss_function();
  int df = -1, dg = -1;
  LossNode n; n.type = kLossComposed; n.a = n.b = 0.0;
  n.g = loss_append(&l->l.nodes, g, &dg);
  n.f = loss_append(&l->l.nodes, f, &df);
  n.depth = 1 + (df > dg ? df : dg);
  if (n.depth < 1) n.depth = 1;
  if (n.depth > kLossMaxDepth) { delete l; set_error("loss functions nested deeper than %d", kLossMaxDepth); return nullptr; }
  l->l.nodes.push_back(n);
  return l;
  SK_GUARD_END(nullptr)
}
sk_loss_function* sk_loss_scaled(const sk_loss_function* rho, double a) {
  SK_GUARD_BEGIN
  sk_loss_function* l = new sk_loss_function();
  int d = -1;
  LossNode n; n.type = kLossScaled; n.a = a; n.b = 0.0; n.g = -1;
  n.f = loss_append(&l->l.nodes, rho, &d);
  n.depth = 1 + (d > 0 ? d : 0);
  if (n.depth > kLossMaxDepth) { delete l; set_error("loss functions nested deeper than %d", kLossMaxDepth); return nullptr; }
  l->l.nodes.push_back(n);
  return l;
  SK_GUARD_END(nullptr)
}

__global__ void loss_evaluate_kernel(const LossNode* nodes, int root, const double* s, int n, double* rho) {
  const int i = blockIdx.x * blockDim.x + threadIdx.x;
  if (i >= n) return;
  double r[3];
  loss_evaluate(nodes, root, s[i], r);
  rho[3 * i] = r[0]; rho[3 * i + 1] = r[1]; rho[3 * i + 2] = r[2];
}
int sk_loss_evaluate(const sk_loss_function* loss, const double* sq_norm, int n, double* rho) {
  SK_GUARD_BEGIN
  if (n < 0 || (n > 0 && (!sq_norm || !rho))) { set_error("sk_loss_evaluate: bad arguments"); return SK_ERR_INVALID_ARGUMENT; }
  if (n == 0) return SK_OK;
  if (sk_device_count() <= 0) { set_error("no HIP device available: libskeres_amd has no CPU fallback"); return SK_ERR_NO_DEVICE; }
  DevBuf<LossNode> dn; DevBuf<double> ds, dr;
  std::vector<LossNode> nodes;
  if (loss) nodes = loss->l.nodes;
  const int root = nodes.empty() ? -1 : (int)nodes.size() - 1;
  nodes = loss_nodes_or_trivial(std::move(nodes));
  SK_HIP_TRY(dn.upload(nodes, nullptr));
  SK_HIP_TRY(ds.upload(std::vector<double>(sq_norm, sq_norm + n), nullptr));
  SK_HIP_TRY(dr.alloc(3 * (size_t)n));
  hipLaunchKernelGGL(loss_evaluate_kernel, dim3((n + 127) / 128), dim3(128), 0, nullptr, dn.p, root, ds.p, n, dr.p);
  SK_HIP_TRY(hipGetLastError());
  SK_HIP_TRY(hipMemcpy(rho, dr.p, 3 * (size_t)n * sizeof(double), hipMemcpyDeviceToHost));
  return SK_OK;
  SK_GUARD_END(SK_ERR_INVALID_ARGUMENT)
}

static sk_local_parameterization* param_new(int type, int global_size, int local_size, unsigned mask) {
  if (global_size < 1 || global_size > kParamMaxSize) { set_error("local parameterization: size %d outside 1..%d", global_size, kParamMaxSize); return nullptr; }
  sk_local_parameterization* h = new (std::nothrow) sk_local_parameterization();
  if (!h) { set_error("out of host memory"); return nullptr; }
  h->p.type = type; h->p.global_size = global_size; h->p.local_size = local_size; h->p.constant_mask = mask;
  return h;
}
sk_local_parameterization* sk_local_parameterization_identity(int size) { return param_new(kParamIdentity, size, size, 0u); }
sk_local_parameterization* sk_local_parameterization_subset(int size, const int* constant_parameters, int num_constant) {
  if (num_constant < 0 || (num_constant > 0 && !constant_parameters)) { set_error("subset parameterization: bad arguments"); return nullptr; }
  unsigned mask = 0;
  for (int i = 0; i < num_constant; ++i) {
    const int c = constant_parameters[i];
    if (c < 0 || c >= size) { set_error("subset parameterization: constant index %d outside [0, %d)", c, size); return nullptr; }
    if ((mask >> c) & 1u) { set_error("subset parameterization: the set of constant parameters cannot contain duplicates"); return nullptr; }
    mask |= 1u << c;
  }
  return param_new(kParamSubset, size, size - num_constant, mask);
}
sk_local_parameterization* sk_local_parameterization_quaternion(void) { return param_new(kParamQuaternion, 4, 3, 0u); }
sk_local_parameterization* sk_local_parameterization_homogeneous_vector(int size) {
  if (size < 2) { set_error("homogeneous vector parameterization: the size of the homogeneous vector needs to be greater than 1"); return nullptr; }
  return param_new(kParamHomogeneousVector, size, size - 1, 0u);
}
void sk_local_parameterization_free(sk_local_parameterization* p) { delete p; }
int sk_local_parameterization_global_size(const sk_local_parameterization* p) { return p ? p->p.global_size : -1; }
int sk_local_parameterization_local_size(const sk_local_parameterization* p) { return p ? p->p.local_size : -1; }

__global__ void param_apply_kernel(ParamBlock pb, const double* x, const double* delta, int n, double* x_plus, double* jac) {
  const int i = blockIdx.x * blockDim.x + threadIdx.x;
  if (i >= n) return;
  if (x_plus) param_plus(pb, x + (size_t)i * pb.global_size, delta + (size_t)i * (pb.local_size > 0 ? pb.local_size : 1), x_plus + (size_t)i * pb.global_size);
  if (jac) param_jacobian(pb, x + (size_t)i * pb.global_size, jac + (size_t)i * pb.global_size * pb.local_size);
}
static ParamBlock param_block_of(const LocalParameterization& lp) {
  ParamBlock pb; pb.type = lp.type; pb.global_size = lp.global_size; pb.local_size = lp.local_size; pb.constant_mask = lp.constant_mask;
  pb.global_off = pb.local_off = 0;
  return pb;
}
int sk_local_parameterization_plus(const sk_local_parameterization* p, const double* x, const double* delta, int n, double* x_plus) {
  SK_GUARD_BEGIN
  if (!p || n < 0 || (n > 0 && (!x || !delta || !x_plus))) { set_error("sk_local_parameterization_plus: bad arguments"); return SK_ERR_INVALID_ARGUMENT; }
  if (n == 0) return SK_OK;
  if (sk_device_count() <= 0) { set_error("no HIP device available: libskeres_amd has no CPU fallback"); return SK_ERR_NO_DEVICE; }
  const int gs = p->p.global_size, ls = std::max(p->p.local_size, 1);
  DevBuf<double> dx, dd, dout;
  SK_HIP_TRY(dx.upload(std::vector<double>(x, x + (size_t)n * gs), nullptr));
  SK_HIP_TRY(dd.upload(std::vector<double>(delta, delta + (size_t)n * ls), nullptr));
  SK_HIP_TRY(dout.alloc((size_t)n * gs));
  hipLaunchKernelGGL(param_apply_kernel, dim3((n + 127) / 128), dim3(128), 0, nullptr, param_block_of(p->p), (const double*)dx.p, (const double*)dd.p, n, dout.p, (double*)nullptr);
  SK_HIP_TRY(hipGetLastError());
  SK_HIP_TRY(hipMemcpy(x_plus, dout.p, (size_t)n * gs * sizeof(double), hipMemcpyDeviceToHost));
  return SK_OK;
  SK_GUARD_END(SK_ERR_INVALID_ARGUMENT)
}
int sk_local_parameterization_compute_jacobian(const sk_local_parameterization* p, const double* x, int n, double* jacobian) {
  SK_GUARD_BEGIN
  if (!p || n < 0 || (n > 0 && (!x || !jacobian))) { set_error("sk_local_parameterization_compute_jacobian: bad arguments"); return SK_ERR_INVALID_ARGUMENT; }
  if (n == 0 || p->p.local_size == 0) return SK_OK;
  if (sk_device_count() <= 0) { set_error("no HIP device available: libskeres_amd has no CPU fallback"); return SK_ERR_NO_DEVICE; }
  const int gs = p->p.global_size, ls = p->p.local_size;
  DevBuf<double> dx, dj;
  SK_HIP_TRY(dx.upload(std::vector<double>(x, x + (size_t)n * gs), nullptr));
  SK_HIP_TRY(dj.alloc((size_t)n * gs * ls));
  hipLaunchKernelGGL(param_apply_kernel, dim3((n + 127) / 128), dim3(128), 0, nullptr, param_block_of(p->p), (const double*)dx.p, (const double*)nullptr, n, (double*)nullptr, dj.p);
  SK_HIP_TRY(hipGetLastError());
  SK_HIP_TRY(hipMemcpy(jacobian, dj.p, (size_t)n * gs * ls * sizeof(double), hipMemcpyDeviceToHost));
  return SK_OK;
  SK_GUARD_END(SK_ERR_INVALID_ARGUMENT)
}

sk_cost_function* sk_cost_function_new_autodiff(int functor_id, const double* consts, int num_consts) {
  FunctorDesc d;
  if (!functor_desc(functor_id, &d)) { set_error("unknown device functor id %d", functor_id); return nullptr; }
  if (num_consts != d.num_consts || (num_consts > 0 && !consts)) { set_error("functor %d captures %d constants, %d given", functor_id, d.num_consts, num_consts); return nullptr; }
  sk_cost_function* cf = new (std::nothrow) sk_cost_function();
  if (!cf) { set_error("out of host memory"); return nullptr; }
  cf->c.functor_id = functor_id;
  cf->c.consts.assign(consts, consts + num_consts);
  cf->c.num_residuals = d.num_residuals;
  cf->c.block_sizes.assign(d.block_sizes, d.block_sizes + d.num_blocks);
  return cf;
}

sk_cost_function* sk_cost_function_new_callback(sk_evaluate_fn fn, void* user, int num_residuals, const int* block_sizes, int num_blocks) {
  if (!fn) { set_error("null evaluate callback"); return nullptr; }
  if (num_residuals <= 0) { set_error("Nonpositive number of residuals specified: %d", num_residuals); return nullptr; }
  if (num_blocks <= 0 || !block_sizes) { set_error("a cost function needs at least one parameter block"); return nullptr; }
  for (int i = 0; i < num_blocks; ++i) if (block_sizes[i] <= 0) { set_error("Nonpositive parameter block sizes specified"); return nullptr; }
  sk_cost_function* cf = new (std::nothrow) sk_cost_function();
  if (!cf) { set_error("out of host memory"); return nullptr; }
  cf->c.functor_id = SK_FUNCTOR_HOST_CALLBACK; cf->c.callback = fn; cf->c.user = user; cf->c.num_residuals = num_residuals;
  cf->c.block_sizes.assign(block_sizes, block_sizes + num_blocks);
  return cf;
}
sk_cost_function* sk_cost_function_new_tape(int num_residuals, const int* block_sizes, int num_blocks, const int* instructions, int num_instructions,
                                            const double* tape_constants, int num_tape_constants, int num_registers, const int* output_operands,
                                            const double* captured, int num_captured) {
  SK_GUARD_BEGIN
  if (num_residuals <= 0) { set_error("Nonpositive number of residuals specified: %d", num_residuals); return nullptr; }
  if (num_blocks <= 0 || !block_sizes) { set_error("a cost function needs at least one parameter block"); return nullptr; }
  if (num_instructions < 0 || (num_instructions > 0 && !instructions) || num_tape_constants < 0 || (num_tape_constants > 0 && !tape_constants) ||
      !output_operands || num_captured < 0 || (num_captured > 0 && !captured)) { set_error("invalid argument"); return nullptr; }
  auto t = std::make_shared<Tape>();
  t->num_residuals = num_residuals; t->num_registers = num_registers; t->num_obs_consts = num_captured;
  t->block_sizes.assign(block_sizes, block_sizes + num_blocks);
  t->ins.resize((size_t)num_instructions);
  for (int i = 0; i < num_instructions; ++i) t->ins[i] = TapeIns{instructions[5 * i], instructions[5 * i + 1], instructions[5 * i + 2], instructions[5 * i + 3], instructions[5 * i + 4]};
  t->consts.assign(tape_constants, tape_constants + num_tape_constants);
  t->out.assign(output_operands, output_operands + num_residuals);
  const std::string why = tape_validate(*t);
  if (!why.empty()) { set_error("%s", why.c_str()); return nullptr; }
  sk_cost_function* cf = new (std::nothrow) sk_cost_function();
  if (!cf) { set_error("out of host memory"); return nullptr; }
  cf->c.functor_id = SK_FUNCTOR_TAPE; cf->c.num_residuals = num_residuals;
  cf->c.block_sizes = t->block_sizes;
  cf->c.consts.assign(captured, captured + num_captured);
  cf->c.tape = t;
  return cf;
  SK_GUARD_END(nullptr)
}
void sk_cost_function_free(sk_cost_function* cf) { delete cf; }
int sk_cost_function_num_residuals(const sk_cost_function* cf) { return cf->c.num_residuals; }
int sk_cost_function_num_parameter_blocks(const sk_cost_function* cf) { return (int)cf->c.block_sizes.size(); }
int sk_cost_function_parameter_block_size(const sk_cost_function* cf, int i) { return cf->c.block_sizes[i]; }

int sk_cost_function_evaluate(const sk_cost_function* cf, double const* const* parameters, double* residuals, double** jacobians) {
  SK_GUARD_BEGIN
  const CostFunction& c = cf->c;
  if (c.functor_id == SK_FUNCTOR_HOST_CALLBACK) return c.callback(c.user, parameters, residuals, jacobians) ? 1 : 0;
  if (sk_device_count() <= 0) { set_error("no HIP device available: libskeres_amd has no CPU fallback"); return -SK_ERR_NO_DEVICE; }
  const int nb = (int)c.block_sizes.size(), nres = c.num_residuals;
  std::vector<int> x_off(nb), j_off(nb);
  int nx = 0, nj = 0; unsigned long long mask = 0;
  for (int q = 0; q < nb; ++q) { x_off[q] = nx; nx += c.block_sizes[q]; j_off[q] = nj; nj += nres * c.block_sizes[q]; if (jacobians && jacobians[q]) mask |= 1ull << q; }
  std::vector<double> x(nx);
  for (int q = 0; q < nb; ++q) std::memcpy(&x[x_off[q]], parameters[q], c.block_sizes[q] * sizeof(double));
  DevBuf<double> dx, dc, dr, dj; DevBuf<int> dxo, djo, dok;
  std::vector<double> consts = c.consts; if (consts.empty()) consts.push_back(0.0);
  hipStream_t s = nullptr;
#define SK_TRYN(e) do { if ((e) != hipSuccess) { set_error("HIP error in sk_cost_function_evaluate"); return -SK_ERR_HIP; } } while (0)
  SK_TRYN(dx.upload(x, s)); SK_TRYN(dc.upload(consts, s)); SK_TRYN(dxo.upload(x_off, s)); SK_TRYN(djo.upload(j_off, s));
  SK_TRYN(dr.alloc(nres)); SK_TRYN(dj.alloc(nj)); SK_TRYN(dok.alloc(1));
  if (c.functor_id == SK_FUNCTOR_TAPE) {
    TapeDevBuffers tb;
    SK_TRYN(tb.upload(*c.tape, s));
    if (!launch_single_eval_tape(tb, dc.p, dx.p, dxo.p, dr.p, dj.p, djo.p, jacobians ? 1 : 0, mask, dok.p, s)) {
      set_error("the recorded functor needs %d registers: more than the device interpreter holds", c.tape->num_registers);
      return -SK_ERR_UNSUPPORTED;
    }
  } else {
    launch_single_eval(c.functor_id, dc.p, dx.p, dxo.p, dr.p, dj.p, djo.p, jacobians ? 1 : 0, mask, dok.p, s);
  }
  int ok = 0;
  std::vector<double> r(nres), j(nj);
  SK_TRYN(hipMemcpy(&ok, dok.p, sizeof(int), hipMemcpyDeviceToHost));
  SK_TRYN(hipMemcpy(r.data(), dr.p, nres * sizeof(double), hipMemcpyDeviceToHost));
  SK_TRYN(hipMemcpy(j.data(), dj.p, nj * sizeof(double), hipMemcpyDeviceToHost));
#undef SK_TRYN
  if (!ok) return 0;
  std::memcpy(residuals, r.data(), nres * sizeof(double));
  for (int q = 0; q < nb; ++q) if ((mask >> q) & 1ull) std::memcpy(jacobians[q], &j[j_off[q]], (size_t)nres * c.block_sizes[q] * sizeof(double));
  return 1;
  SK_GUARD_END(-SK_ERR_INVALID_ARGUMENT)
}

sk_problem* sk_problem_new(void) { return new (std::nothrow) sk_problem(); }
void sk_problem_free(sk_problem* p) { delete p; }

static int register_block(Problem& P, double* ptr, int size) {
  if (!ptr) { set_error("null parameter block pointer"); return -1; }
// ... 768 lines not shown
```

skeres_amd/csrc/dev_knobs.hpp:

```cpp
#pragma once

namespace sk {

struct DevKnobs {
  int chain_server = 1;
  int bs_resident = 1;
  const char* chain_stamps = nullptr;
  const char* bs_stamps = nullptr;
  bool debug_queues = false, debug_envelope = false, debug_segments = false, debug_chain_abort = false, debug_setup = false;
  int queue_shift = 0;
  int chain_queues = -1;
  int pair_max_trailing = 0;
  int dissect_at = -1;
  int chain_early_server = 1;
  int bs_spread = 1;
  int bs_pair = 1;
  int bulk_reserve = -1, bulk_reserve_early = -1;
  int chain_xcd_local = 0;
  int cgnr_batch = 0;
  int inner_batch = 0;
  int schedule_plain = 0;
};
const DevKnobs& dev_knobs();

}
```

Measured before the change: 260.0.

## Fuse Schur assembly launches: prologue memsets, point+kept, pair long+short, backsub

Merges several small kernel launches and memsets in the Schur assembly and back-substitution path into combined kernels. Envelope zeroing, flag clearing and the yf 0xff fill become one prologue kernel. Point-block plus kept-points, long plus short pair, and point backsub plus kept step each become one launch, partitioned by block index. Kept points are skipped in the generic point kernels via a new per-point flag. The intent is to cut launch overhead and inter-kernel gaps. The cost is some extra branching, and the fused pair kernel carries the larger shared-memory footprint for both halves.

Result: no change. 260.9 (median of 5 runs) (+0.3%).

```diff
diff --git a/skeres_amd/csrc/bal_kernels.hip b/skeres_amd/csrc/bal_kernels.hip
--- a/skeres_amd/csrc/bal_kernels.hip
+++ b/skeres_amd/csrc/bal_kernels.hip
@@ -470,8 +470,9 @@
   if (threadIdx.x == 0) out[k] = sh[0];
 }
 
-__global__ __launch_bounds__(kBlock) void bal_point_block_kernel(BalDev d) {
-  const int gid = blockIdx.x * kBlock + threadIdx.x, sub = gid % kPointLanes;
+template <bool kSkipKept>
+__device__ __forceinline__ void bal_point_block_body(const BalDev& d, int block) {
+  const int gid = block * kBlock + threadIdx.x, sub = gid % kPointLanes;
   const int p = gid / kPointLanes;
   if (p >= d.P) return;
   double t00 = 0, t10 = 0, t11 = 0, t20 = 0, t21 = 0, t22 = 0;
@@ -496,19 +497,24 @@
   const double m21 = -(l21 * m11) / l22;
   const double m20 = -(l20 * m00 + l21 * m10) / l22;
   const size_t P = d.P;
-  d.M[p] = m00; d.M[P + p] = m10; d.M[2 * P + p] = m11; d.M[3 * P + p] = m20; d.M[4 * P + p] = m21; d.M[5 * P + p] = m22;
-  const double g0 = d.gs_p[3 * (size_t)p], g1 = d.gs_p[3 * (size_t)p + 1], g2 = d.gs_p[3 * (size_t)p + 2];
-  const double u0 = m00 * g0, u1 = m10 * g0 + m11 * g1, u2 = m20 * g0 + m21 * g1 + m22 * g2;
-  d.q[p] = m00 * u0 + m10 * u1 + m20 * u2;
-  d.q[P + p] = m11 * u1 + m21 * u2;
-  d.q[2 * P + p] = m22 * u2;
+  if (!(kSkipKept && d.pt_kept && d.pt_kept[p])) {
+    d.M[p] = m00; d.M[P + p] = m10; d.M[2 * P + p] = m11; d.M[3 * P + p] = m20; d.M[4 * P + p] = m21; d.M[5 * P + p] = m22;
+    const double g0 = d.gs_p[3 * (size_t)p], g1 = d.gs_p[3 * (size_t)p + 1], g2 = d.gs_p[3 * (size_t)p + 2];
+    const double u0 = m00 * g0, u1 = m10 * g0 + m11 * g1, u2 = m20 * g0 + m21 * g1 + m22 * g2;
+    d.q[p] = m00 * u0 + m10 * u1 + m20 * u2;
+    d.q[P + p] = m11 * u1 + m21 * u2;
+    d.q[2 * P + p] = m22 * u2;
+  }
   if (!(l00 > 0.0) || !(l11 > 0.0) || !(l22 > 0.0)) *d.fail_flag = 1;
 }
-
-__global__ __launch_bounds__(kBlock) void bal_kept_points_kernel(BalDev d, int obs_blocks) {
+__global__ __launch_bounds__(kBlock) void bal_point_block_kernel(BalDev d) { bal_point_block_body<false>(d, (int)blockIdx.x); }
+
+__global__ __launch_bounds__(kBlock) void bal_kept_points_kernel(BalDev d, int point_blocks, int obs_blocks) {
+  if ((int)blockIdx.x < point_blocks) { bal_point_block_body<true>(d, (int)blockIdx.x); return; }
+  const int block = (int)blockIdx.x - point_blocks;
   const size_t N = d.N, P = d.P;
-  if ((int)blockIdx.x < obs_blocks) {
-    const int e = blockIdx.x * kBlock + threadIdx.x;
+  if (block < obs_blocks) {
+    const int e = block * kBlock + threadIdx.x;
     if (e >= d.num_kept_obs) return;
     const int o = d.kept_obs[e], k = d.kept_obs_slot[e];
     const int ic = d.kept_cam[k] / 3, t3 = 3 * (d.kept_cam[k] % 3);
@@ -531,7 +537,7 @@
     }
     return;
   }
-  const int k = (((int)blockIdx.x - obs_blocks) * kBlock + threadIdx.x) >> 6, lane = threadIdx.x & 63;
+  const int k = ((block - obs_blocks) * kBlock + threadIdx.x) >> 6, lane = threadIdx.x & 63;
   if (k >= d.num_kept) return;
   const int p = d.kept_pt[k], ic = d.kept_cam[k] / 3, t3 = 3 * (d.kept_cam[k] % 3);
   double t00 = 0, t10 = 0, t11 = 0, t20 = 0, t21 = 0, t22 = 0;
@@ -729,10 +735,11 @@
   return ((q / group) * 8 + x) * group + q % group;
 }
 
-__global__ __launch_bounds__(kBlock) void bal_pair_kernel(BalDev d, int xcd_group) {
+typedef double PairShare[7][kPairSlot];
+typedef double PairRed[7][81];
+__device__ __forceinline__ void bal_pair_short_body(const BalDev& d, int block, int xcd_group, PairShare* share) {
   const int lane = threadIdx.x & 63;
-  const int wave = (xcd_grouped_block((int)blockIdx.x, xcd_group) * kBlock + threadIdx.x) >> 6;
-  __shared__ __attribute__((aligned(16))) double share[kBlock / 64][7][kPairSlot];
+  const int wave = (xcd_grouped_block(block, xcd_group) * kBlock + threadIdx.x) >> 6;
   const int sub = lane / 9, c = lane - 9 * sub;
   const int slot = wave * 7 + sub;
   if (sub >= 7 || slot >= d.num_short_segments) return;
@@ -747,12 +754,14 @@
 #pragma unroll
   for (int k = 0; k < 9; ++k) out[k] = -acc[k];
 }
-
-__global__ __launch_bounds__(kBlock) void bal_pair_long_kernel(BalDev d, int xcd_group) {
-  __shared__ double red[kBlock / 64][7][81];
-  __shared__ __attribute__((aligned(16))) double share[kBlock / 64][7][kPairSlot];
+__global__ __launch_bounds__(kBlock, 6) void bal_pair_kernel(BalDev d, int xcd_group) {
+  __shared__ __attribute__((aligned(16))) PairShare share[kBlock / 64];
+  bal_pair_short_body(d, (int)blockIdx.x, xcd_group, share);
+}
+
+__device__ __forceinline__ void bal_pair_long_body(const BalDev& d, int block, int xcd_group, PairRed* red, PairShare* share) {
   const int lane = threadIdx.x & 63, w = threadIdx.x >> 6;
-  const int slot = (xcd_grouped_block((int)blockIdx.x, xcd_group) * kBlock + threadIdx.x) >> 6;
+  const int slot = (xcd_grouped_block(block, xcd_group) * kBlock + threadIdx.x) >> 6;
   if (slot >= d.num_long_segments) return;
   const int seg = d.long_segments[slot];
   const int sub = lane / 9, c = lane - 9 * sub;
@@ -776,6 +785,17 @@
     for (int g = 0; g < 7; ++g) s += red[w][g][e];
     blk[(size_t)(e / 9) * ld + e % 9] = -s;
   }
+}
+__global__ __launch_bounds__(kBlock) void bal_pair_long_kernel(BalDev d, int xcd_group) {
+  __shared__ PairRed red[kBlock / 64];
+  __shared__ __attribute__((aligned(16))) PairShare share[kBlock / 64];
+  bal_pair_long_body(d, (int)blockIdx.x, xcd_group, red, share);
+}
+__global__ __launch_bounds__(kBlock, 6) void bal_pair_all_kernel(BalDev d, int long_blocks, int xcd_group) {
+  __shared__ PairRed red[kBlock / 64];
+  __shared__ __attribute__((aligned(16))) PairShare share[kBlock / 64];
+  if ((int)blockIdx.x < long_blocks) bal_pair_long_body(d, (int)blockIdx.x, xcd_group, red, share);
+  else bal_pair_short_body(d, (int)blockIdx.x - long_blocks, xcd_group, share);
 }
 
 __global__ void finish_normal_matrix_kernel(double* S, int ld, int n, int npad, int rhs_row, const double* D) {
@@ -816,7 +836,8 @@
   }
 }
 
-__global__ __launch_bounds__(kBlock) void bal_point_backsub_kernel(BalDev d) {
+template <bool kSkipKept>
+__device__ __forceinline__ void bal_point_backsub_body(const BalDev& d) {
   const int gid = blockIdx.x * kBlock + threadIdx.x, sub = gid % kPointLanes;
   const int p = gid / kPointLanes;
   double acc[1] = {0.0};
@@ -829,7 +850,7 @@
     }
   }
   w0 = point_lanes_sum(w0); w1 = point_lanes_sum(w1); w2 = point_lanes_sum(w2);
-  if (p < d.P && sub == 0) {
+  if (p < d.P && sub == 0 && !(kSkipKept && d.pt_kept && d.pt_kept[p])) {
     const size_t P = d.P;
     const double t0 = d.gs_p[3 * (size_t)p] - w0, t1 = d.gs_p[3 * (size_t)p + 1] - w1, t2 = d.gs_p[3 * (size_t)p + 2] - w2;
     const double m00 = d.M[p], m10 = d.M[P + p], m11 = d.M[2 * P + p], m20 = d.M[3 * P + p], m21 = d.M[4 * P + p], m22 = d.M[5 * P + p];
@@ -849,8 +870,9 @@
   }
   block_sum<1>(acc, d.partial + d.partial_stride, d.partial_stride);
 }
-
-__global__ __launch_bounds__(kBlock) void bal_kept_step_kernel(BalDev d, int slot) {
+__global__ __launch_bounds__(kBlock) void bal_point_backsub_kernel(BalDev d) { bal_point_backsub_body<false>(d); }
+
+__device__ __forceinline__ void bal_kept_step_body(const BalDev& d, double* out) {
   double acc[1] = {0.0};
   for (int k = threadIdx.x; k < d.num_kept; k += kBlock) {
     const int p = d.kept_pt[k], ic = d.kept_cam[k] / 3, t3 = 3 * (d.kept_cam[k] % 3);
@@ -866,7 +888,12 @@
       if (home) acc[0] += df * df;
     }
   }
-  block_sum<1>(acc, d.partial + d.partial_stride + slot, d.partial_stride);
+  block_sum<1>(acc, out, d.partial_stride);
+}
+__global__ __launch_bounds__(kBlock) void bal_kept_step_kernel(BalDev d, int slot) { bal_kept_step_body(d, d.partial + d.partial_stride + slot); }
+__global__ __launch_bounds__(kBlock) void bal_point_and_kept_backsub_kernel(BalDev d, int point_blocks) {
+  if ((int)blockIdx.x < point_blocks) bal_point_backsub_body<true>(d);
+  else bal_kept_step_body(d, d.partial + d.partial_stride);
 }
 
 __global__ __launch_bounds__(kBlock) void bal_cam_step_kernel(BalDev d, int norm_lo, int norm_hi, int norm_lo2, int norm_hi2) {
@@ -925,8 +952,7 @@
   return g < 1 ? 1 : (g > cap ? cap : g);
 }
 
-__global__ __launch_bounds__(256) void zero_envelope_kernel(double* S, int ld, const int* col0) {
-  const int kb = blockIdx.y;
+__device__ __forceinline__ void zero_envelope_row(double* S, int ld, const int* col0, int kb) {
   const size_t c0 = (size_t)col0[kb] * 128, width = (size_t)(kb + 1) * 128 - c0;
   const size_t n2 = 128 * width / 2;
   for (size_t i = (size_t)blockIdx.x * 256 + threadIdx.x; i < n2; i += (size_t)gridDim.x * 256) {
@@ -934,8 +960,24 @@
     *reinterpret_cast<double2*>(S + ((size_t)kb * 128 + r) * ld + c0 + c) = make_double2(0.0, 0.0);
   }
 }
+__global__ __launch_bounds__(256) void zero_envelope_kernel(double* S, int ld, const int* col0) { zero_envelope_row(S, ld, col0, (int)blockIdx.y); }
 void launch_zero_envelope(double* S, int ld, const int* col0, int nblk, hipStream_t s) {
   if (nblk > 0) hipLaunchKernelGGL(zero_envelope_kernel, dim3(32, nblk), dim3(256), 0, s, S, ld, col0);
+}
+__global__ __launch_bounds__(256) void bal_assembly_prologue_kernel(BalPrologue p) {
+  int kb = blockIdx.y;
+#pragma unroll
+  for (int f = 0; f < 3; ++f) {
+    if (kb < p.nblk[f]) { zero_envelope_row(p.S[f], p.ld[f], p.col0[f], kb); return; }
+    kb -= p.nblk[f];
+  }
+  const long i0 = (long)blockIdx.x * 256 + threadIdx.x;
+  if (i0 < p.nflags) p.flags[i0] = 0.0;
+  unsigned long long* y = reinterpret_cast<unsigned long long*>(p.y);
+  for (long i = i0; i < p.ny; i += (long)gridDim.x * 256) y[i] = ~0ull;
+}
+void launch_bal_assembly_prologue(const BalPrologue& p, hipStream_t s) {
+  hipLaunchKernelGGL(bal_assembly_prologue_kernel, dim3(32, p.nblk[0] + p.nblk[1] + p.nblk[2] + 1), dim3(256), 0, s, p);
 }
 
 int bal_partial_blocks(int N) { return grid_for(N); }
@@ -1026,7 +1068,12 @@
 void launch_bal_kept_points(const BalDev& d, hipStream_t s) {
   if (d.num_kept <= 0) return;
   const int obs_blocks = (d.num_kept_obs + kBlock - 1) / kBlock;
-  hipLaunchKernelGGL(bal_kept_points_kernel, dim3(obs_blocks + (d.num_kept * 64 + kBlock - 1) / kBlock), dim3(kBlock), 0, s, d, obs_blocks);
+  hipLaunchKernelGGL(bal_kept_points_kernel, dim3(obs_blocks + (d.num_kept * 64 + kBlock - 1) / kBlock), dim3(kBlock), 0, s, d, 0, obs_blocks);
+}
+void launch_bal_point_and_kept(const BalDev& d, hipStream_t s) {
+  if (d.num_kept <= 0 || d.P <= 0 || !d.pt_kept) { launch_bal_point_block(d, s); launch_bal_kept_points(d, s); return; }
+  const int obs_blocks = (d.num_kept_obs + kBlock - 1) / kBlock;
+  hipLaunchKernelGGL(bal_kept_points_kernel, dim3(point_grid(d.P) + obs_blocks + (d.num_kept * 64 + kBlock - 1) / kBlock), dim3(kBlock), 0, s, d, point_grid(d.P), obs_blocks);
 }
 void launch_bal_obs_precompute(const BalDev& d, hipStream_t s) { hipLaunchKernelGGL(bal_obs_precompute_kernel, dim3(grid_for(d.N)), dim3(kBlock), 0, s, d); }
 void launch_bal_kept_sums(const BalDev& d, double* buf, int K, bool gather, hipStream_t s) {
@@ -1039,6 +1086,11 @@
 void launch_bal_pair(const BalDev& d, hipStream_t s) {
   const int group_long = dev_knobs().schedule_plain ? 0 : 8, group_short = group_long;
   auto grid = [](int blocks, int group) { return group > 0 ? (blocks + 8 * group - 1) / (8 * group) * (8 * group) : blocks; };
+  if ((dev_knobs().fused_launches & 4) && d.num_long_segments > 0 && d.num_short_segments > 0) {
+    const int gl = grid((d.num_long_segments * 64 + kBlock - 1) / kBlock, group_long), gs = grid((((d.num_short_segments + 6) / 7) * 64 + kBlock - 1) / kBlock, group_short);
+    hipLaunchKernelGGL(bal_pair_all_kernel, dim3(gl + gs), dim3(kBlock), 0, s, d, gl, group_long);
+    return;
+  }
   if (d.num_long_segments > 0)
     hipLaunchKernelGGL(bal_pair_long_kernel, dim3(grid((d.num_long_segments * 64 + kBlock - 1) / kBlock, group_long)), dim3(kBlock), 0, s, d, group_long);
   if (d.num_short_segments > 0) {
@@ -1076,8 +1128,12 @@
   const int gc = (9 * d.C + kBlock - 1) / kBlock, gp = bal_point_blocks(d.P);
   hipLaunchKernelGGL(bal_cam_step_kernel, dim3(gc), dim3(kBlock), 0, s, d, norm_lo, norm_hi, norm_lo2, norm_hi2);
   hipLaunchKernelGGL(bal_obs_backsub_kernel, dim3(grid_for(d.N)), dim3(kBlock), 0, s, d);
-  hipLaunchKernelGGL(bal_point_backsub_kernel, dim3(gp), dim3(kBlock), 0, s, d);
-  if (d.num_kept > 0) hipLaunchKernelGGL(bal_kept_step_kernel, dim3(1), dim3(kBlock), 0, s, d, gp);
+  if ((dev_knobs().fused_launches & 8) && d.num_kept > 0 && d.pt_kept) {
+    hipLaunchKernelGGL(bal_point_and_kept_backsub_kernel, dim3(gp + 1), dim3(kBlock), 0, s, d, gp);
+  } else {
+    hipLaunchKernelGGL(bal_point_backsub_kernel, dim3(gp), dim3(kBlock), 0, s, d);
+    if (d.num_kept > 0) hipLaunchKernelGGL(bal_kept_step_kernel, dim3(1), dim3(kBlock), 0, s, d, gp);
+  }
   ReduceRows rows;
   rows.n = 2;
   rows.row[0] = 0; rows.count[0] = gc; rows.out[0] = out;
diff --git a/skeres_amd/csrc/bal_kernels.hpp b/skeres_amd/csrc/bal_kernels.hpp
--- a/skeres_amd/csrc/bal_kernels.hpp
+++ b/skeres_amd/csrc/bal_kernels.hpp
@@ -31,6 +31,7 @@
   const int* kept_pt;  const int* kept_cam;
   int num_kept_obs;  const int* kept_obs;  const int* kept_obs_slot;
   const unsigned char* pseudo;
+  const unsigned char* pt_kept;
   const int* kept_home;  const int* kept_global;
   int num_dup;  const int* dup_a;  const int* dup_b;  const int* dup_cam;
   double* xc;  double* xp;
@@ -63,6 +64,9 @@
 int bal_partial_blocks(int N);
 int bal_point_blocks(int P);
 void launch_zero_envelope(double* S, int ld, const int* col0, int nblk, hipStream_t s);
+struct BalPrologue { double* S[3] = {nullptr, nullptr, nullptr}; int ld[3] = {0, 0, 0}; const int* col0[3] = {nullptr, nullptr, nullptr}; int nblk[3] = {0, 0, 0};
+                     double* flags = nullptr; int nflags = 0; double* y = nullptr; long ny = 0; };
+void launch_bal_assembly_prologue(const BalPrologue& p, hipStream_t s);
 size_t tri_packed_elems(int nblk);
 void launch_tri_pack(double* S, int ld, double* packed, int nblk, const int* col0, const long long* off, bool to_packed, hipStream_t s);
 void launch_bal_eval_jac(const BalDev& d, hipStream_t s);
@@ -84,6 +88,7 @@
 void launch_final_reduce_rows(const double* partial, int stride, const ReduceRows& rows, hipStream_t s);
 void launch_bal_point_block(const BalDev& d, hipStream_t s);
 void launch_bal_kept_points(const BalDev& d, hipStream_t s);
+void launch_bal_point_and_kept(const BalDev& d, hipStream_t s);
 void launch_bal_kept_sums(const BalDev& d, double* buf, int K, bool gather, hipStream_t s);
 void launch_bal_obs_precompute(const BalDev& d, hipStream_t s);
 void launch_bal_cam_diag(const BalDev& d, hipStream_t s);
diff --git a/skeres_amd/csrc/bal_solver.hip b/skeres_amd/csrc/bal_solver.hip
--- a/skeres_amd/csrc/bal_solver.hip
+++ b/skeres_amd/csrc/bal_solver.hip
@@ -195,6 +195,7 @@
   std::vector<int> struct_ocam_, struct_opt_;
   int struct_P_ = 0;
   DevBuf<int> b_kept_pt_, b_kept_cam_, b_kept_obs_, b_kept_obs_slot_;
+  DevBuf<unsigned char> b_pt_kept_;
   int P_own_ = 0;
   DevBuf<int> b_kept_home_, b_kept_global_;
   DevBuf<int> b_dup_a_, b_dup_b_, b_dup_cam_;
@@ -634,6 +635,9 @@
     if (segmented_) { SK_HIP_TRY(b_kept_home_.upload(ls.kept_home, s)); SK_HIP_TRY(b_kept_global_.upload(ls.kept_global, s)); }
     SK_HIP_TRY(b_kept_obs_.upload(ls.kept_obs, s)); SK_HIP_TRY(b_kept_obs_slot_.upload(ls.kept_obs_slot, s));
     num_kept_obs_ = (int)ls.kept_obs.size();
+    std::vector<unsigned char> kept(P_, 0);
+    for (int p : ls.kept_pt) kept[p] = 1;
+    SK_HIP_TRY(b_pt_kept_.upload(kept, s));
   }
   return SK_OK;
 }
@@ -694,6 +698,7 @@
   const size_t nc = 9 * (size_t)C_, nx = nc + 3 * (size_t)P_;
   d_.C = C_; d_.P = P_; d_.N = N_;
   d_.pseudo = pseudo_cams_ > 0 ? b_pseudo_.p : nullptr; d_.num_kept = pseudo_cams_ > 0 ? (int)ls.kept_pt.size() : 0; d_.kept_pt = b_kept_pt_.p; d_.kept_cam = b_kept_cam_.p;
+  d_.pt_kept = pseudo_cams_ > 0 && !ls.kept_pt.empty() ? b_pt_kept_.p : nullptr;
   d_.num_kept_obs = pseudo_cams_ > 0 ? num_kept_obs_ : 0; d_.kept_obs = b_kept_obs_.p; d_.kept_obs_slot = b_kept_obs_slot_.p;
   d_.kept_home = segmented_ && pseudo_cams_ > 0 ? b_kept_home_.p : nullptr; d_.kept_global = segmented_ && pseudo_cams_ > 0 ? b_kept_global_.p : nullptr;
   d_.num_dup = num_dup_; d_.dup_a = b_dup_a_.p; d_.dup_b = b_dup_b_.p; d_.dup_cam = b_dup_cam_.p;
@@ -1023,14 +1028,27 @@
 
 int BalSolver::enqueue_schur_assembly(const Backsolve& bs, bool graph) {
   hipStream_t s = stream_;
+  const int fused = dev_knobs().fused_launches;
   kt_.begin("memset_S", s);
-  for (int f = 0; f < 3; ++f)
-    if (fr_[f].nblk > 0) launch_zero_envelope(d_.front[f].S, (int)fr_[f].dim, (zero_by_backsolve_ && !need_full_zero_) ? b_zero_min_f_[f].p : b_zero_col0_f_[f].p, fr_[f].nblk, s);
+  if (fused & 1) {
+    BalPrologue p;
+    for (int f = 0; f < 3; ++f) {
+      if (fr_[f].nblk <= 0) continue;
+      p.S[f] = d_.front[f].S; p.ld[f] = (int)fr_[f].dim; p.nblk[f] = fr_[f].nblk;
+      p.col0[f] = (zero_by_backsolve_ && !need_full_zero_) ? b_zero_min_f_[f].p : b_zero_col0_f_[f].p;
+    }
+    p.flags = b_scal_.p + kFail; p.nflags = kInfo + 1 - kFail;
+    if (bs.resident) { p.y = b_yf_.p; p.ny = (long)(fr_[0].dim + fr_[1].dim + fr_[2].dim); }
+    launch_bal_assembly_prologue(p, s);
+  } else {
+    for (int f = 0; f < 3; ++f)
+      if (fr_[f].nblk > 0) launch_zero_envelope(d_.front[f].S, (int)fr_[f].dim, (zero_by_backsolve_ && !need_full_zero_) ? b_zero_min_f_[f].p : b_zero_col0_f_[f].p, fr_[f].nblk, s);
+  }
   kt_.end("memset_S", s);
   need_full_zero_ = !bs.zero_after;
-  SK_HIP_TRY(hipMemsetAsync(b_scal_.p + kFail, 0, (kInfo + 1 - kFail) * sizeof(double), s));
-  launch_bal_point_block(d_, s);
-  launch_bal_kept_points(d_, s);
+  if (!(fused & 1)) SK_HIP_TRY(hipMemsetAsync(b_scal_.p + kFail, 0, (kInfo + 1 - kFail) * sizeof(double), s));
+  if (fused & 2) launch_bal_point_and_kept(d_, s);
+  else { launch_bal_point_block(d_, s); launch_bal_kept_points(d_, s); }
   launch_bal_obs_precompute(d_, s);
   kt_.begin("bal_cam_diag", s); launch_bal_cam_diag(d_, s); kt_.end("bal_cam_diag", s);
   kt_.begin("bal_pair", s); launch_bal_pair(d_, s); kt_.end("bal_pair", s);
@@ -1064,7 +1082,7 @@
   double* yf[3] = {b_yf_.p + fr_[0].y_off, b_yf_.p + fr_[1].y_off, b_yf_.p + fr_[2].y_off};
   double* wf[3] = {b_wf_.p + fr_[0].y_off, b_wf_.p + fr_[1].y_off, b_wf_.p + fr_[2].y_off};
   const bool prefilled = bs.resident != 0;
-  if (prefilled) SK_HIP_TRY(hipMemsetAsync(b_yf_.p, 0xff, (fr_[0].dim + fr_[1].dim + fr_[2].dim) * sizeof(double), s));
+  if (prefilled && !(dev_knobs().fused_launches & 1)) SK_HIP_TRY(hipMemsetAsync(b_yf_.p, 0xff, (fr_[0].dim + fr_[1].dim + fr_[2].dim) * sizeof(double), s));
   if (segmented_) {
     const FrontView& L = leaf_;
     const FrontHost& R = fr_[2];
diff --git a/skeres_amd/csrc/capi.hip b/skeres_amd/csrc/capi.hip
--- a/skeres_amd/csrc/capi.hip
+++ b/skeres_amd/csrc/capi.hip
@@ -79,6 +79,7 @@
     k.pair_max_trailing = num("SK_CHAIN_PAIR_MAX_TRAILING", 0);
     k.dissect_at = num("SK_DISSECT_AT", -1);
     k.schedule_plain = num("SK_SCHEDULE_PLAIN", 0);
+    k.fused_launches = num("SK_FUSED_LAUNCHES", 15);
     k.cgnr_batch = num("SK_CGNR_BATCH", 0);
     k.inner_batch = num("SK_INNER_BATCH", 0);
     k.chain_xcd_local = num("SK_CHAIN_XCD_LOCAL", 0);
diff --git a/skeres_amd/csrc/dev_knobs.hpp b/skeres_amd/csrc/dev_knobs.hpp
--- a/skeres_amd/csrc/dev_knobs.hpp
+++ b/skeres_amd/csrc/dev_knobs.hpp
@@ -20,6 +20,7 @@
   int cgnr_batch = 0;
   int inner_batch = 0;
   int schedule_plain = 0;
+  int fused_launches = 15;
 };
 const DevKnobs& dev_knobs();
 
```
